# shurizzle/cake

Measured on AMD Instinct MI355X. Metric: decode_tokens_per_sec, higher is better.
Workload: dtype bf16; 1 GPU; model=Llama-3-8B, global_batch=1, seq_len=1097, prompt_len=32, parallelism=single, decode=greedy, repeat_penalty 1.10 last_n 128

## Files before the change

### cake_amd/csrc/engine/llama_engine.cpp

```cpp
#include "llama_engine.h"

#include <dlfcn.h>
#include <hip/hip_runtime.h>
#include <unistd.h>

#include <algorithm>
#include <chrono>
#include <cmath>
#include <cstdio>
#include <cstdlib>
#include <cstring>
#include <fstream>
#include <list>
#include <map>
#include <memory>
#include <sstream>
#include <stdexcept>
#include <string>
#include <tuple>
#include <vector>

#include "../driver/graph_loop.h"
#include "../kernels/cake_kernels.h"
#include "../runtime/json.h"
// ... 81 lines not shown
        const double factor = rs("factor", 8.0), lo = rs("low_freq_factor", 1.0),
                     hi = rs("high_freq_factor", 4.0),
                     old = rs("original_max_position_embeddings", 8192.0);
        const double lo_wl = old / lo, hi_wl = old / hi, wl = 2.0 * M_PI / f;
        const double o = wl > lo_wl ? f / factor : f;
        const double smooth = (old / wl - lo) / (hi - lo);
        const double mid = (1.0 - smooth) * o / factor + smooth * o;
        f = (wl >= hi_wl && wl <= lo_wl) ? mid : o;
      }
      out[i] = (float)f;
    }
    return out;
  }
};


std::vector<std::pair<int, int>> shard_layers(const Cfg& c, int world) {
  std::vector<std::pair<int, int>> out;
  if (world <= 1) {
    out.push_back({0, c.L});
    return out;
  }
  if (world > c.L) {
    for (int r = 0; r < world; ++r) out.push_back(r < c.L ? std::make_pair(r, r + 1)
                                                          : std::make_pair(c.L, c.L));
    return out;
  }
  const double layer_bytes = 2.0 * ((double)c.H * (c.nh + 2 * c.nkv) * c.hd +
                                    (double)c.nh * c.hd * c.H + 3.0 * c.H * c.I + 2.0 * c.H);
  const double head = 2.0 * (double)c.V * c.H / layer_bytes;
  const double total = c.L + head;
  int start = 0;
  for (int r = 0; r < world; ++r) {
    int end = r < world - 1 ? (int)std::nearbyint((r + 1) * total / world - head) : c.L;
    end = std::max(start + (c.L - start >= world - r ? 1 : 0), std::min(end, c.L - (world - 1 - r)));
    out.push_back({start, end});
    start = end;
  }
  return out;
}

std::pair<int, int> split_range(int n, int world, int rank) {
  const int q = n / world, r = n % world;
  const int a = rank * q + std::min(rank, r);
  return {a, a + q + (rank < r ? 1 : 0)};
}

bool trace_on() {
  static const bool on = [] {
    const char* v = std::getenv("CAKE_ENGINE_TRACE");
    return v && *v && std::string(v) != "0";
  }();
  return on;
}
void trace(int rank, const std::string& what) {
  if (!trace_on()) return;
  static const auto t0 = std::chrono::steady_clock::now();
  const double t = std::chrono::duration<double>(std::chrono::steady_clock::now() - t0).count();
  std::fprintf(stderr, "[engine r%d +%.3fs] %s\n", rank, t, what.c_str());
  std::fflush(stderr);
}

const char* const kNoFp8TP =
    "fp8 weights (weight_fmt 1) are not supported with tensor parallelism yet: open the "
    "tensor-parallel engine with weight_fmt 0";

const char* const kNoQHeadTP =
    "a quantised lm_head (head_fmt 1 = fp8, 2 = mxfp4) is not supported with tensor "
    "parallelism: open the tensor-parallel engine with head_fmt 0";

const char* const kNoKvTP =
    "a quantised KV cache (kv_fmt 1 = fp8, 2 = its 16-bit oracle) is not supported with tensor "
    "parallelism: open the tensor-parallel engine with kv_fmt 0";

const char* const kNoPrefillTP =
    "an fp8 MFMA prefill (prefill_fmt 1) is not supported with tensor parallelism: open the "
    "tensor-parallel engine with prefill_fmt 0";

Json msg(const char* cmd) {
  Json j = Json::object();
  j.set("cmd", Json::string(cmd));
  return j;
}

class Llama {
 public:
  Llama(const std::string& dir, const CakeEngineOpts& o, const CakePipeOpts* pp = nullptr,
        const std::vector<int>* layers = nullptr, const CakeTPOpts* tp = nullptr,
        const CakeRemoteOpts* remote = nullptr)
      : dt_(o.dtype), dev_(o.device), init_(o.init), wfmt_(CAKE_WEIGHT_FMT_OF(o.weight_fmt)),
        hfmt_(o.head_fmt), kvfmt_(o.kv_fmt), pfmt_(CAKE_PREFILL_FMT_OF(o.weight_fmt)),
        seed_(o.seed) {
    if (dt_ != 0 && dt_ != 1) throw Error("dtype must be 0 (bf16) or 1 (f16)");
    if (wfmt_ != 0 && wfmt_ != 1 && wfmt_ != 2)
      throw Error("weight_fmt must be 0 (model dtype), 1 (fp8 e4m3 projections) or 2 (mxfp4 "
                  "projections)");
    if (wfmt_ != 0 && tp) throw Error(kNoFp8TP);
    if (hfmt_ != 0 && hfmt_ != 1 && hfmt_ != 2)
      throw Error("head_fmt must be 0 (model dtype), 1 (fp8 e4m3 lm_head) or 2 (mxfp4 lm_head)");
    if (hfmt_ != 0 && tp) throw Error(kNoQHeadTP);
    if (kvfmt_ != kKv16 && kvfmt_ != kKvFp8 && kvfmt_ != kKvFp8Emu)
      throw Error("kv_fmt must be 0 (model dtype), 1 (fp8 e4m3 KV cache) or 2 (fp8 values in a "
                  "16-bit cache: the test oracle)");
    if (kvfmt_ != kKv16 && tp) throw Error(kNoKvTP);
    if (kvfmt_ != kKv16) {
      for (const char* name : {"CAKE_ATTN_OPROJ", "CAKE_ATTN_HEADS", "CAKE_MK", "CAKE_QKV_ATTN"}) {
        const char* e = std::getenv(name);
        if (e && *e && std::string(e) != "0")
          throw Error(std::string("a quantised KV cache (kv_fmt ") + std::to_string(kvfmt_) +
                      ") does not run the experimental decode path " + name + "=" + e +
                      ": unset it or open with kv_fmt 0");
      }
    }
    if (pfmt_ != 0 && pfmt_ != 1)
      throw Error("prefill_fmt must be 0 (the weights' prefill) or 1 (fp8 MFMA prefill with "
                  "per-token e4m3 activations)");
    if (pfmt_ != 0 && tp) throw Error(kNoPrefillTP);
    if (pfmt_ == 1 && wfmt_ != 1)
      throw Error("an fp8 MFMA prefill (prefill_fmt 1) runs on the resident fp8 projection codes: "
                  "open with weight_fmt 1 (fp8), not " + std::to_string(wfmt_));
    if (init_ != 0 && init_ != 1) throw Error("init must be 0 (checkpoint) or 1 (random)");
    if (tp) {
      tp_ = tp->world;
      tp_rank_ = tp->rank;
      hop_timeout_ = tp->timeout_s > 0 ? tp->timeout_s : 30.0;
      if (tp_ < 1 || tp_ > 8 || tp_rank_ < 0 || tp_rank_ >= tp_) throw Error("bad TP rank / world");
      int n = 0;
      hip_check(hipGetDeviceCount(&n), "hipGetDeviceCount");
      if (n > 0) dev_ %= n;
    }
    if (pp) {
      rank_ = pp->rank;
      world_ = pp->world;
      hop_bf16_ = pp->hop_bf16 != 0;
      hop_timeout_ = pp->hop_timeout_s > 0 ? pp->hop_timeout_s : 30.0;
      if (world_ < 1 || rank_ < 0 || rank_ >= world_) throw Error("bad rank / world");
      int n = 0;
      hip_check(hipGetDeviceCount(&n), "hipGetDeviceCount");
      if (n > 0) dev_ %= n;
    }
    hip_check(hipSetDevice(dev_), "hipSetDevice");
    hip_check(hipStreamCreateWithFlags(&st_, hipStreamNonBlocking), "hipStreamCreate");
    cfg_ = Cfg::parse(Json::parse(read_file(dir + "/config.json")));
    S_ = o.max_seq > 0 ? o.max_seq : 4096;
    k_ = std::max(1, o.steps_per_graph);
    if (cfg_.H % 8 || cfg_.hd % 2 || cfg_.nh % cfg_.nkv) throw Error("unsupported model shape");
    if (kvfmt_ != kKv16 && cfg_.hd != 64 && cfg_.hd != 128)
      throw Error("an fp8 KV cache needs a head dimension of 64 or 128");
    lc_ = cfg_;
    if (tp_ > 1) {
      if (cfg_.nh % tp_ || cfg_.nkv % tp_)
        throw Error("tensor-parallel degree must divide the query and KV heads");
      lc_.nh = cfg_.nh / tp_;
      lc_.nkv = cfg_.nkv / tp_;
      const auto ir = split_range(cfg_.I, tp_, tp_rank_);
      const auto vr = split_range(cfg_.V, tp_, tp_rank_);
      i0_ = ir.first;
      lc_.I = ir.second - ir.first;
      voff_ = vr.first;
      lc_.V = vr.second - vr.first;
      if (lc_.I % 8 || (lc_.nh * cfg_.hd) % 8) throw Error("tensor-parallel slice not 8-aligned");
    }
    if (wfmt_ == 1 && (cfg_.H % 16 || (cfg_.nh * cfg_.hd) % 16 || cfg_.I % 16))
      throw Error("fp8 weights need hidden, attention and intermediate widths divisible by 16");
    if (pfmt_ == 1 && (cfg_.H % 128 || (cfg_.nh * cfg_.hd) % 128 || cfg_.I % 128))
      throw Error("an fp8 MFMA prefill needs hidden, attention and intermediate widths divisible "
                  "by 128 (the k of one MFMA step)");
    if (wfmt_ == 2 && (cfg_.H % 32 || (cfg_.nh * cfg_.hd) % 32 || cfg_.I % 32))
      throw Error("mxfp4 weights need hidden, attention and intermediate widths divisible by 32");
    if (layers) {
      hfmt_ = 0;
      owned_ = *layers;
      std::sort(owned_.begin(), owned_.end());
      owned_.erase(std::unique(owned_.begin(), owned_.end()), owned_.end());
      if (owned_.empty() || owned_.front() < 0 || owned_.back() >= cfg_.L)
        throw Error("worker layers outside the model");
      head_ = false;
    } else {
      const bool placed = pp && pp->owners && pp->n_owners > 0;
      owner_.assign(cfg_.L, 0);
      if (placed) {
        if (pp->n_owners != cfg_.L)
          throw Error("owner map has " + std::to_string(pp->n_owners) + " entries for " +
                      std::to_string(cfg_.L) + " layers");
        for (int l = 0; l < cfg_.L; ++l) {
          if (pp->owners[l] < 0 || pp->owners[l] >= world_)
            throw Error("layer " + std::to_string(l) + " placed on rank " +
                        std::to_string(pp->owners[l]) + " outside the world of " +
                        std::to_string(world_));
          owner_[l] = pp->owners[l];
        }
      } else {
        const auto sh = shard_layers(cfg_, world_);
        for (int r = 0; r < world_; ++r)
          for (int l = sh[r].first; l < sh[r].second; ++l) owner_[l] = r;
      }
      if (remote) {
        if (remote->n_layers != cfg_.L || !remote->worker_of)
          throw Error("remote placement must name every layer (-1 = local)");
        remote_of_.assign(remote->worker_of, remote->worker_of + cfg_.L);
        for (int l = 0; l < cfg_.L; ++l)
          if (remote_of_[l] < -1 || remote_of_[l] >= remote->n_workers)
            throw Error("layer " + std::to_string(l) + " placed on an unknown worker");
        for (int w = 0; w < remote->n_workers; ++w)
          remotes_.push_back({remote->workers[w] ? remote->workers[w] : "", -1});
        remote_timeout_ = remote->timeout_s > 0 ? remote->timeout_s : 60.0;
      }
      for (int l = 0; l < cfg_.L; ++l)
        if (owner_[l] == rank_ && (remote_of_.empty() || remote_of_[l] < 0)) owned_.push_back(l);
      head_ = rank_ == 0;
      if (!head_) hfmt_ = 0;
    }
    if (hfmt_ == 1 && cfg_.H % 16) throw Error("an fp8 lm_head needs a hidden width divisible by 16");
    if (hfmt_ == 2 && cfg_.H % 32)
      throw Error("an mxfp4 lm_head needs a hidden width divisible by 32");
    lo_ = owned_.empty() ? 0 : owned_.front();
    hi_ = owned_.empty() ? 0 : owned_.back() + 1;
    local_.assign(cfg_.L, -1);
    for (size_t i = 0; i < owned_.size(); ++i) local_[owned_[i]] = (int)i;
    if (!layers) plan_walk();
    planner_.load(pkg_dir() + "/ops/gemm_tuned.json");
    load_weights(dir);
    std::fprintf(stderr,
                 "cake engine: weights %s, lm_head %s, kv cache %s%s, %lld bytes on device (rank %d, "
                 "%d layers)\n",
                 wfmt_ == 1 ? (dt_ == 0 ? "fp8 e4m3 projections (bf16 rest)"
                                        : "fp8 e4m3 projections (f16 rest)")
                 : wfmt_ == 2 ? (dt_ == 0 ? "mxfp4 projections (bf16 rest)"
                                          : "mxfp4 projections (f16 rest)")
                              : (dt_ == 0 ? "bf16" : "f16"),
                 !head_ ? "none" : hfmt_ == 1 ? "fp8 e4m3" : hfmt_ == 2 ? "mxfp4"
                                                : (dt_ == 0 ? "bf16" : "f16"),
                 kvfmt_ == kKvFp8 ? "fp8 e4m3"
                 : kvfmt_ == kKvFp8Emu ? (dt_ == 0 ? "fp8 e4m3 values in bf16 (test oracle)"
                                                   : "fp8 e4m3 values in f16 (test oracle)")
                                       : (dt_ == 0 ? "bf16" : "f16"),
                 pfmt_ == 1 ? ", prefill fp8 e4m3 activations" : "",
                 (long long)weight_bytes_, rank(), (int)owned_.size());
    alloc_state();
    warm_library();
    {
      size_t fr = 0, tot = 0;
      (void)hipMemGetInfo(&fr, &tot);
      trace(rank(), "weights + state ready (" + std::to_string(owned_.size()) + " layers), " +
                        std::to_string(fr >> 20) + " of " + std::to_string(tot >> 20) +
                        " MiB free");
    }
    if (world_ > 1) {
      connect_pipeline(pp->master_addr ? pp->master_addr : "127.0.0.1:29517",
                       pp->connect_timeout_s > 0 ? pp->connect_timeout_s : 600.0);
      trace(rank_, "pipeline connected: walk " + walk_str() + ", " +
                       std::to_string(edges_.size()) + " edges");
      selftest_pipeline();
      trace(rank_, "pipeline self-test passed");
    }
    if (tp_ > 1) {
      connect_tp(tp->master_addr ? tp->master_addr : "127.0.0.1:29517",
                 tp->connect_timeout_s > 0 ? tp->connect_timeout_s : 600.0);
      trace(rank(), "tensor-parallel channels mapped");
      selftest_tp();
      trace(rank(), "tensor-parallel self-test passed");
    }
    if (!remotes_.empty()) connect_remotes();
  }

  ~Llama() {
    (void)hipSetDevice(dev_);
    (void)hipStreamSynchronize(st_);
    if (rank_ == 0 && tp_rank_ == 0)
      for (int fd : peers_) {
        try {
          send_json(fd, msg("exit"));
        } catch (const std::exception&) {
        }
      }
    for (int fd : peers_) tcp_close(fd);
    if (ctl_fd_ >= 0) tcp_close(ctl_fd_);
    for (auto& r : remotes_)
      if (r.fd >= 0) tcp_close(r.fd);
    drop_graphs();
    for (void* p : tp_mapped_) (void)hipIpcCloseMemHandle(p);
    for (void* p : tp_owned_) (void)cake_hop_free(p);
    for (auto& kv : out_inbox_) (void)hipIpcCloseMemHandle(kv.second);
    for (auto& kv : peer_pbuf_) (void)hipIpcCloseMemHandle(kv.second);
    for (auto& kv : my_inbox_) (void)cake_hop_free(kv.second);
    if (relay_) (void)cake_hop_free(relay_);
    for (void* p : allocs_) (void)hipFree(p);
    (void)hipStreamDestroy(st_);
  }

  int rank() const { return tp_ > 1 ? tp_rank_ : rank_; }
  int world() const { return tp_ > 1 ? tp_ : world_; }
  std::pair<int, int> layer_range() const { return {lo_, hi_}; }

  const Cfg& cfg() const { return cfg_; }
  int max_seq() const { return S_; }
  int64_t weight_bytes() const { return weight_bytes_; }
  int64_t kv_bytes() const { return 2 * (int64_t)kv_elems() * kv_esize(); }

  void prefill_logits(const int32_t* prompt, int T, float* host_logits) {
    hip_check(hipSetDevice(dev_), "hipSetDevice");
    if (!head_) throw Error("prefill_logits() runs on pipeline rank 0");
    prefill(prompt, T);
    hip_check(hipMemcpyAsync(host_logits, logits_, sizeof(float) * cfg_.V, hipMemcpyDeviceToHost,
                             st_), "logits D2H");
    hip_check(hipStreamSynchronize(st_), "sync");
  }

  void forced_logits(const int32_t* prompt, int T, const int32_t* forced, int n, float* out) {
    hip_check(hipSetDevice(dev_), "hipSetDevice");
    if (!head_ || tp_rank_ != 0) throw Error("forced_logits() runs on rank 0");
    if (T <= 0 || n < 0 || T + n + 1 > S_) throw Error("prompt + forced tokens exceed max_seq");
    forced_run(prompt, T, forced, n, out);
  }

  void score(const int32_t* tokens, int n, int vchunk, float* lse, float* tgt, int32_t* top,
             float* topv) {
    hip_check(hipSetDevice(dev_), "hipSetDevice");
    if (tp_ > 1)
      throw Error("score() is not available on a tensor-parallel engine (the vocabulary is "
                  "sharded)");
    if (!head_) throw Error("score() runs on an engine that holds the head (pipeline rank 0)");
    const int V = cfg_.V;
    if (n < 2) throw Error("score() needs at least 2 tokens");
    if (n > S_) throw Error("score(): " + std::to_string(n) + " tokens exceed max_seq " +
                            std::to_string(S_));
    for (int i = 0; i < n; ++i)
      if (tokens[i] < 0 || tokens[i] >= V)
        throw Error("score(): token id " + std::to_string(tokens[i]) + " at " +
                    std::to_string(i) + " is outside [0, " + std::to_string(V) + ")");
    int Vc = vchunk;
    if (vchunk == 0) {
      const long long fit = (64LL << 20) / (4LL * n) / 256 * 256;
      Vc = (int)std::max<long long>(256, fit);
    } else if (vchunk < 0 || vchunk % 256) {
      throw Error("score(): vchunk is 0 or a positive multiple of 256, got " +
                  std::to_string(vchunk));
    }
    Vc = std::min(Vc, V);
    grow_score(n, Vc);
    prefill_body(tokens, n);
    const int H = cfg_.H;
    std::vector<int32_t> target(tokens + 1, tokens + n);
    target.push_back(-1);
    hip_check(hipMemcpyAsync(sc_target_, target.data(), sizeof(int32_t) * n,
                             hipMemcpyHostToDevice, st_), "targets H2D");
    k_check(cake_rmsnorm(dt_, hidden_, norm_, (float)cfg_.eps, n, H, x16_, st_), "rmsnorm");
    for (int v0 = 0; v0 < V; v0 += Vc) {
      const int w = std::min(Vc, V - v0);
      const void* rows;
      if (hfmt_ == 1) {
        k_check(cake_dequant_rows_fp8(dt_, head_q_ + (size_t)v0 * H, head_s_ + v0, w, H, sc_head_,
                                      st_), "dequant_rows_fp8 lm_head");
        rows = sc_head_;
      } else if (hfmt_ == 2) {
        k_check(cake_dequant_rows_mxfp4(dt_, head_q_ + (size_t)v0 * H / 2,
                                        head_e_ + (size_t)v0 * H / 32, w, H, sc_head_, st_),
                "dequant_rows_mxfp4 lm_head");
        rows = sc_head_;
      } else {
        rows = (const uint16_t*)lm_head_ + (size_t)v0 * H;
      }
      gemm(kEpiStore32, x16_, H, rows, H, nullptr, 0, sc_logits_, Vc, n, w, H, "gemm score head");
      k_check(cake_lse_rows(sc_logits_, Vc, n, w, v0, v0 == 0, sc_target_, sc_max_, sc_sum_,
                            sc_tgt_, sc_key_, st_), "lse_rows");
    }
    k_check(cake_lse_finish(sc_max_, sc_sum_, sc_key_, n, sc_lse_, sc_top_, sc_topv_, st_),
            "lse_finish");
    hip_check(hipMemcpyAsync(lse, sc_lse_, sizeof(float) * n, hipMemcpyDeviceToHost, st_), "D2H");
    hip_check(hipMemcpyAsync(tgt, sc_tgt_, sizeof(float) * n, hipMemcpyDeviceToHost, st_), "D2H");
    hip_check(hipMemcpyAsync(top, sc_top_, sizeof(int32_t) * n, hipMemcpyDeviceToHost, st_),
              "D2H");
    hip_check(hipMemcpyAsync(topv, sc_topv_, sizeof(float) * n, hipMemcpyDeviceToHost, st_),
              "D2H");
    hip_check(hipStreamSynchronize(st_), "sync");
    if (world_ > 1) sync_workers();
    check_attn_error("rank " + std::to_string(rank()));
  }

  void set_logprobs(int top_k) {
// ... 202 lines not shown
    };
    stats->p50_ms = pct(50);
    stats->p99_ms = pct(99);
  }

  void run_generation(const int32_t* prompt, int T, int max_new, const CakeEngineSampling& smp,
                      const int32_t* eos, int n_eos, cake_engine_token_cb cb, void* ctx,
                      int32_t* out, int out_cap, CakeEngineStats* stats, bool lead) {
    const auto t0 = std::chrono::steady_clock::now();
    prefill_body(prompt, T);
    std::vector<int32_t> h(prompt, prompt + T);
    hip_check(hipMemcpyAsync(hist_, h.data(), sizeof(int32_t) * T, hipMemcpyHostToDevice, st_),
              "hist H2D");
    set_i32(hist_len_, T);
    set_i32(pos_, T - 1);
    hip_check(hipMemsetAsync(slot_, 0, sizeof(unsigned long long), st_), "slot");
    Mode mode = mode_of(smp);
    if (tp_ > 1) {
      head_tp(hidden_ + (size_t)(T - 1) * cfg_.H, mode);
    } else {
      head_gemv(hidden_ + (size_t)(T - 1) * cfg_.H);
      select_tail(mode);
      logprob_record(mode);
    }
    if (mode.fused) k_check(cake_embed(dt_, embed_, tok_, 1, cfg_.H, resid_, st_), "embed");
    int32_t first = 0;
    hip_check(hipMemcpyAsync(&first, tok_, sizeof(int32_t), hipMemcpyDeviceToHost, st_), "tok");
    lp_begin(mode.logprobs >= 0, max_new);
    if (lp_on_)
      hip_check(hipMemcpyAsync(lp_host_.data(), lp_rec_ + (size_t)T * kLpRecWords,
                               kLpRecWords * 4, hipMemcpyDeviceToHost, st_), "logprob D2H");
    hip_check(hipStreamSynchronize(st_), "sync");
    if (lp_on_ && lead) lp_n_ = 1;
    const auto t1 = std::chrono::steady_clock::now();
    int n_out = 0;
    bool stop = false;
    for (int e = 0; e < n_eos && !stop; ++e)
      if (eos[e] == first) stop = true;
    if (lead) {
      out[n_out++] = first;
      const bool cb_stop = cb && cb(ctx, first) != 0;
      if (tp_ == 1) stop = stop || cb_stop;
    }
    std::vector<float> ms;
    last_mode_ = mode;
    if (remote_mode()) {
      have_graphs_ = true;
      if (!stop && max_new > 1)
        n_out += decode_eager(T, max_new - 1, mode, eos, n_eos, cb, ctx, out + n_out,
                              out_cap - n_out, &ms);
    } else {
      ensure_graphs(mode);
      if (!stop && max_new > 1)
        n_out += decode_tokens(T + 1, max_new - 1, eos, n_eos, cb, ctx,
                               lead ? out + n_out : nullptr, lead ? out_cap - n_out : 0, lead, &ms);
    }
    const auto t2 = std::chrono::steady_clock::now();
    if (stats)
      fill_stats(stats, T, n_out, std::chrono::duration<double>(t1 - t0).count(),
                 std::chrono::duration<double>(t2 - t1).count(), ms);
  }

  int read_i32(const int* p) {
    int v = 0;
    hip_check(hipMemcpyAsync(&v, p, sizeof(int), hipMemcpyDeviceToHost, st_), "i32 D2H");
    hip_check(hipStreamSynchronize(st_), "sync");
    return v;
  }

  void check_attn_error(const std::string& who) {
    unsigned int w = 0;
    hip_check(hipMemcpyAsync(&w, tickets_ + 2 * lc_.nkv, sizeof(w), hipMemcpyDeviceToHost, st_),
              "attn err D2H");
    hip_check(hipStreamSynchronize(st_), "sync");
    if (w) {
      hip_check(hipMemsetAsync(tickets_ + 2 * lc_.nkv, 0, sizeof(unsigned int), st_), "attn err");
      hip_check(hipStreamSynchronize(st_), "sync");
      throw Error(who + ": decode attention split merge timed out waiting for its partials; "
                        "the tokens of that generation are invalid");
    }
  }

 private:
  struct LayerW {
    void *ln1, *wqkv, *wo, *ln2, *wgu, *wd;
    float *sqkv = nullptr, *so = nullptr, *sgu = nullptr, *sd = nullptr;
    uint8_t *eqkv = nullptr, *eo = nullptr, *egu = nullptr, *ed = nullptr;
  };
  struct Mode {
    bool fused = true;
    bool greedy = true;
    float temperature = 0.f, top_p = 0.f, penalty = 1.f;
    int top_k = 0, last_n = 0;
    unsigned long long seed = 0;
    int logprobs = -1;
    bool operator==(const Mode& o) const {
      return std::tie(fused, greedy, temperature, top_p, penalty, top_k, last_n, seed,
                      logprobs) ==
             std::tie(o.fused, o.greedy, o.temperature, o.top_p, o.penalty, o.top_k, o.last_n,
                      o.seed, o.logprobs);
    }
  };

  int dt_, dev_, init_ = 0;
  int wfmt_ = 0;
  int hfmt_ = 0;
  int kvfmt_ = 0;
  int pfmt_ = 0;
  uint16_t *kv16_k_ = nullptr, *kv16_v_ = nullptr;
  int64_t weight_bytes_ = 0;
  uint8_t *head_q_ = nullptr, *head_e_ = nullptr;
  float* head_s_ = nullptr;
  uint16_t* w16_ = nullptr;
  bool forced_ = false;
  AoFns ao_;
  bool ao_ok_ = false, short_step_ = false;
  int heads_max_ = 0;
  float* ao_ws_ = nullptr;
  unsigned int* ao_tickets_ = nullptr;
  uint64_t seed_ = 0;
  int rank_ = 0, world_ = 1, lo_ = 0, hi_ = 0;
  bool head_ = true, hop_bf16_ = false;
  double hop_timeout_ = 30.0;
  enum StopKind { kEmbedStop, kRunStop, kHeadStop, kRemoteStop };
  struct Stop {
    StopKind kind;
    int rank;
    std::vector<int> layers;
    std::vector<int> sel;
    int remote = -1;
  };
  struct RemoteWorker {
    std::string addr;
    int fd;
  };
  std::vector<RemoteWorker> remotes_;
  std::vector<int> remote_of_;
  double remote_timeout_ = 60.0;
  std::vector<float> host_rows_;
  std::vector<Stop> walk_;
  std::vector<int> edge_in_;
  std::vector<std::pair<int, int>> edges_;
  std::vector<int> owner_;
  std::map<int, void*> my_inbox_;
  std::map<int, void*> out_inbox_;
  std::map<int, void*> peer_pbuf_;
  float* relay_ = nullptr;
  unsigned int* seq_ = nullptr;
  int* hop_err_ = nullptr;
  std::vector<int> peers_;
  struct ArChan {
    void* inbox = nullptr;
    std::vector<void*> peers;
  };

  int tp_ = 1, tp_rank_ = 0, i0_ = 0, voff_ = 0, slab_bank_ = 0;
  static constexpr int kSlabRows = 512;
  Cfg lc_;
  ArChan ch_sum_, ch_key_, ch_gat_;
  float *partial_ = nullptr, *ppart_ = nullptr, *full_logits_ = nullptr, *slab_ = nullptr;
  unsigned int* ar_seq_ = nullptr;
  int* ar_err_ = nullptr;
  std::vector<void*> peer_slab_, tp_mapped_, tp_owned_;
  int ctl_fd_ = -1;
  hipStream_t st_ = nullptr;
  Cfg cfg_;
  int S_ = 0, k_ = 1;
  GemmPlanner planner_;
  std::vector<void*> allocs_;
  void *embed_ = nullptr, *norm_ = nullptr, *lm_head_ = nullptr;
  std::vector<LayerW> layers_;
// ... 274 lines not shown
    } catch (...) {
      if (stage) (void)hipFree(stage);
      throw;
    }
    if (stage) (void)hipFree(stage);
  }


  void alloc_state() {
    const Cfg& c = lc_;
    kv_session(0);
    if (kvfmt_ == kKvFp8) {
      const size_t n = (size_t)c.nkv * S_ * c.hd;
      kv16_k_ = dalloc<uint16_t>(n);
      kv16_v_ = dalloc<uint16_t>(n);
      hip_check(hipMemset(kv16_k_, 0, n * 2), "memset");
      hip_check(hipMemset(kv16_v_, 0, n * 2), "memset");
    }
    const std::vector<float> f = c.inv_freq();
    inv_freq_ = dalloc<float>(f.size());
    hip_check(hipMemcpy(inv_freq_, f.data(), f.size() * sizeof(float), hipMemcpyHostToDevice),
              "inv_freq");
    const size_t nq = (size_t)c.nh * c.hd;
    resid_ = dalloc<float>(c.H + 4);
    hidden_ = dalloc<float>((size_t)S_ * c.H);
    q_ = dalloc<float>(nq);
    part_ = dalloc<float>(2 * (size_t)c.nh * kMaxSplit * (c.hd + 2));
    logits_ = dalloc<float>(c.V);
    attn_out_ = dalloc<uint16_t>(nq);
    act_ = dalloc<uint16_t>(c.I);
    tickets_ = dalloc<unsigned int>(2 * c.nkv + 2);
    thr_ = dalloc<unsigned int>(1);
    sel_ticket_ = dalloc<unsigned int>(1);
    pos_ = reinterpret_cast<int*>(resid_ + c.H);
    tok_ = dalloc<int>(1);
    hist_ = dalloc<int>(S_);
    hist_len_ = dalloc<int>(1);
    slot_ = dalloc<unsigned long long>(1);
    scratch_i32_ = dalloc<int>(4);
    scratch_resid_ = dalloc<float>(c.H + 4);
    zeros_ = dalloc<int32_t>(64);
    hip_check(hipMemset(tickets_, 0, sizeof(unsigned int) * (2 * c.nkv + 2)), "memset");
    hip_check(hipMemset(part_, 0, sizeof(float) * 2 * c.nh * kMaxSplit * (c.hd + 2)), "memset");
    hip_check(hipMemset(sel_ticket_, 0, sizeof(unsigned int)), "memset");
    hip_check(hipMemset(slot_, 0, sizeof(unsigned long long)), "memset");
    hip_check(hipMemset(zeros_, 0, sizeof(int32_t) * 64), "memset");
    hip_check(hipMemset(hist_, 0, sizeof(int) * S_), "memset");
    hip_check(hipMemset(resid_, 0, sizeof(float) * (c.H + 4)), "memset");
    {
      const char* e = std::getenv("CAKE_ATTN_OPROJ");
      if (e && std::string(e) == "1" && wfmt_ == 0 && kvfmt_ == kKv16) ao_ = ao_fns();
      ao_ok_ = ao_.run != nullptr && ao_.supported(c.nh, c.nkv, c.hd, c.H) != 0;
    }
    if (!ao_ok_ && kvfmt_ == kKv16) {
      const char* e = std::getenv("CAKE_ATTN_HEADS");
      int mx = 0, nw = 2, pfd = 2;
      if (e && *e) std::sscanf(e, "%d:%d:%d", &mx, &nw, &pfd);
      if (mx > 0 && cake_attn_set_heads(mx, nw) == 0 && cake_attn_set_head_prefetch(pfd) == 0)
        heads_max_ = mx;
    }
    if (ao_ok_) {
      ao_ws_ = dalloc<float>((size_t)ao_.ws_floats(c.nkv, c.H));
      const size_t tw = (size_t)ao_.ticket_words(c.nkv, c.H);
      ao_tickets_ = dalloc<unsigned int>(tw);
      hip_check(hipMemset(ao_tickets_, 0, sizeof(unsigned int) * tw), "memset");
    }
    const size_t nseq = 2 * edges_.size() + 2;
    seq_ = dalloc<unsigned int>(nseq);
    hop_err_ = dalloc<int>(4);
    hip_check(hipMemset(seq_, 0, sizeof(unsigned int) * nseq), "memset");
    hip_check(hipMemset(hop_err_, 0, sizeof(int) * 4), "memset");
    if (tp_ > 1) {
      partial_ = dalloc<float>(c.H);
      ppart_ = dalloc<float>((size_t)S_ * c.H);
      full_logits_ = dalloc<float>(cfg_.V);
      ar_seq_ = dalloc<unsigned int>(8);
      ar_err_ = dalloc<int>(4);
      hip_check(hipMemset(ar_seq_, 0, sizeof(unsigned int) * 8), "memset");
      hip_check(hipMemset(ar_err_, 0, sizeof(int) * 4), "memset");
    }
    hip_check(hipDeviceSynchronize(), "sync");
  }

  size_t kv_esize() const { return kvfmt_ == kKvFp8 ? 1 : 2; }
  size_t kv_elems() const { return owned_.size() * (size_t)lc_.nkv * S_ * lc_.hd; }
  void* kc(int l) const { return cur_.k + (size_t)l * lc_.nkv * S_ * lc_.hd * kv_esize(); }
  void* vc(int l) const { return cur_.v + (size_t)l * lc_.nkv * S_ * lc_.hd * kv_esize(); }

  static constexpr size_t kMaxSessions = 8;
  void kv_session(uint64_t id) {
    auto it = kv_.find(id);
    if (it == kv_.end()) {
      if (kv_.size() >= kMaxSessions) {
        uint64_t victim = lru_.front();
        for (uint64_t x : lru_)
          if (x != 0) { victim = x; break; }
        drop_session(victim);
      }
      const size_t n = kv_elems() * kv_esize();
      KV kv{dalloc<uint8_t>(n), dalloc<uint8_t>(n)};
      it = kv_.emplace(id, kv).first;
    }
    lru_.remove(id);
    lru_.push_back(id);
    cur_ = it->second;
  }

 public:
  void drop_session(uint64_t id) {
    auto it = kv_.find(id);
    if (it == kv_.end() || id == 0) return;
    hip_check(hipStreamSynchronize(st_), "sync");
    dfree(it->second.k);
    dfree(it->second.v);
    kv_.erase(it);
    lru_.remove(id);
    if (kv_.count(0)) cur_ = kv_[0];
  }

  void forward_host(uint64_t session, const std::vector<int>& layers, int pos0, float* h, int T) {
    hip_check(hipSetDevice(dev_), "hipSetDevice");
    const Cfg& c = lc_;
    if (T < 1 || pos0 < 0 || (int64_t)pos0 + T > S_) throw Error("positions exceed the KV cache");
    std::vector<int> sel;
    for (int l : layers) {
      if (l < 0 || l >= c.L || local_[l] < 0)
        throw Error("layer " + std::to_string(l) + " is not served here");
      sel.push_back(local_[l]);
    }
    kv_session(session);
    if (T == 1) {
      hip_check(hipMemcpyAsync(resid_, h, sizeof(float) * c.H, hipMemcpyHostToDevice, st_), "H2D");
      hip_check(hipMemcpyAsync(pos_, &pos0, sizeof(int), hipMemcpyHostToDevice, st_), "H2D");
      short_step_ = short_at(pos0);
      try {
        step_layers(&sel);
      } catch (...) {
        short_step_ = false;
        throw;
      }
      short_step_ = false;
      hip_check(hipMemcpyAsync(h, resid_, sizeof(float) * c.H, hipMemcpyDeviceToHost, st_), "D2H");
    } else {
      const size_t bytes = sizeof(float) * (size_t)T * c.H;
      hip_check(hipMemcpyAsync(hidden_, h, bytes, hipMemcpyHostToDevice, st_), "H2D");
      prefill_layers(T, pos0, &sel);
      hip_check(hipMemcpyAsync(h, hidden_, bytes, hipMemcpyDeviceToHost, st_), "D2H");
    }
    hip_check(hipStreamSynchronize(st_), "sync");
    if (kv_.count(0)) cur_ = kv_[0];
    if (T == 1) check_attn_error("worker");
  }

 private:
  float scale() const { return 1.0f / std::sqrt((float)cfg_.hd); }

  bool short_at(int pos) const { return short_len(pos + 2); }
  bool short_len(int t) const {
    if (ao_ok_) return cake_attn_splits(t) == 1;
    return heads_max_ > 0 && t <= heads_max_;
  }

  void grow_prefill(int T) {
    if (T <= pre_T_) return;
    const Cfg& c = lc_;
    for (void* p : {x16_, qkv_, att_, pact_, (void*)ptok_}) dfree(p);
// ... 322 lines not shown
        continue;
      }
      const int r = owner_.empty() ? 0 : owner_[l];
      if (walk_.back().kind != kRunStop || walk_.back().rank != r) walk_.push_back({kRunStop, r, {}, {}});
      walk_.back().layers.push_back(l);
      if (r == rank_) walk_.back().sel.push_back(local_[l]);
    }
    walk_.push_back({kHeadStop, 0, {}, {}});
    edge_in_.assign(walk_.size(), -1);
    edges_.clear();
    for (size_t i = 1; i < walk_.size(); ++i)
      if (walk_[i].rank != walk_[i - 1].rank) {
        edge_in_[i] = (int)edges_.size();
        edges_.push_back({walk_[i - 1].rank, walk_[i].rank});
      }
  }

 public:
  std::string walk_str() const {
    std::string s;
    for (const Stop& st : walk_)
      if (st.kind == kRunStop || st.kind == kRemoteStop) {
        if (!s.empty()) s += ",";
        s += (st.kind == kRemoteStop ? "w" + std::to_string(st.remote) : std::to_string(st.rank)) +
             ":" + std::to_string(st.layers.front()) + "-" + std::to_string(st.layers.back());
      }
    return s;
  }
  int n_edges() const { return (int)edges_.size(); }

 private:

  void attn(int l) {
    const Cfg& c = lc_;
    if (kvfmt_ == kKvFp8)
      k_check(cake_attn_decode_kv8(dt_, q_, kc(l), vc(l), pos_, S_, c.nh, c.nkv, c.hd, scale(),
                                   part_, tickets_, attn_out_, st_), "attn_decode_kv8");
    else if (short_step_)
      k_check(cake_attn_decode_heads(dt_, q_, kc(l), vc(l), pos_, S_, c.nh, c.nkv, c.hd,
                                     scale(), attn_out_, st_), "attn_heads");
    else
      k_check(cake_attn_decode(dt_, q_, kc(l), vc(l), pos_, S_, c.nh, c.nkv, c.hd, scale(),
                               part_, tickets_, attn_out_, st_), "attn_decode");
  }

  void step_layers(const std::vector<int>* sel = nullptr) {
    const Cfg& c = lc_;
    const int nq = c.nh * c.hd, nk = c.nkv * c.hd;
    const int nl = sel ? (int)sel->size() : (int)layers_.size();
    for (int i = 0; i < nl; ++i) {
      const int l = sel ? (*sel)[i] : i;
      const LayerW& w = layers_[l];
      if (wfmt_ == 2) {
        const uint8_t* q4 = reinterpret_cast<const uint8_t*>(w.wqkv);
        const size_t rb = (size_t)c.H / 2, re = (size_t)c.H / 32;
        k_check(cake_qkv_rope_w4_kvf(dt_, resid_, w.ln1, (float)c.eps, q4, q4 + (size_t)nq * rb,
                                     q4 + (size_t)(nq + nk) * rb, w.eqkv, w.eqkv + (size_t)nq * re,
                                     w.eqkv + (size_t)(nq + nk) * re, c.H, c.nh, c.nkv, c.hd,
                                     inv_freq_, pos_, q_, kc(l), vc(l), S_, st_, kvfmt_),
                "qkv_rope_w4");
        attn(l);
        k_check(cake_gemv_x16_w4(dt_, attn_out_, w.wo, w.eo, nq, c.H, resid_, 1, st_), "o_proj_w4");
        const uint8_t* gu4 = reinterpret_cast<const uint8_t*>(w.wgu);
        k_check(cake_swiglu_w4(dt_, resid_, w.ln2, (float)c.eps, gu4, gu4 + (size_t)c.I * rb,
                               w.egu, w.egu + (size_t)c.I * re, c.H, c.I, act_, st_), "swiglu_w4");
        k_check(cake_gemv_x16_w4(dt_, act_, w.wd, w.ed, c.I, c.H, resid_, 1, st_), "down_proj_w4");
        continue;
      }
      if (wfmt_ == 1) {
        const uint8_t* q8 = reinterpret_cast<const uint8_t*>(w.wqkv);
        k_check(cake_qkv_rope_w8_kvf(dt_, resid_, w.ln1, (float)c.eps, q8, q8 + (size_t)nq * c.H,
                                     q8 + (size_t)(nq + nk) * c.H, w.sqkv, w.sqkv + nq,
                                     w.sqkv + nq + nk, c.H, c.nh, c.nkv, c.hd, inv_freq_, pos_, q_,
                                     kc(l), vc(l), S_, st_, kvfmt_), "qkv_rope_w8");
        attn(l);
        k_check(cake_gemv_x16_w8(dt_, attn_out_, w.wo, w.so, nq, c.H, resid_, 1, st_), "o_proj_w8");
        const uint8_t* gu8 = reinterpret_cast<const uint8_t*>(w.wgu);
        k_check(cake_swiglu_w8(dt_, resid_, w.ln2, (float)c.eps, gu8, gu8 + (size_t)c.I * c.H,
                               w.sgu, w.sgu + c.I, c.H, c.I, act_, st_), "swiglu_w8");
        k_check(cake_gemv_x16_w8(dt_, act_, w.wd, w.sd, c.I, c.H, resid_, 1, st_), "down_proj_w8");
        continue;
      }
      const uint16_t* wqkv = reinterpret_cast<const uint16_t*>(w.wqkv);
      k_check(cake_qkv_rope_kvf(dt_, resid_, w.ln1, (float)c.eps, wqkv, wqkv + (size_t)nq * c.H,
                                wqkv + (size_t)(nq + nk) * c.H, c.H, c.nh, c.nkv, c.hd, inv_freq_,
                                pos_, q_, kc(l), vc(l), S_, st_, kvfmt_), "qkv_rope");
      if (kvfmt_ != kKvFp8 && short_step_ && ao_ok_) {
        k_check(ao_.run(dt_, q_, kc(l), vc(l), pos_, S_, c.nh, c.nkv, c.hd, scale(), w.wo,
                                nq, c.H, tp_ > 1 ? partial_ : resid_, tp_ > 1 ? 0 : 1, ao_ws_,
                                ao_tickets_, tickets_ + 2 * c.nkv, st_), "attn_oproj");
        if (tp_ > 1) ar_sum();
      } else {
        attn(l);
        if (tp_ > 1) {
          k_check(cake_gemv_x16(dt_, attn_out_, w.wo, nq, c.H, partial_, 0, st_), "o_proj");
          ar_sum();
        } else {
          k_check(cake_gemv_x16(dt_, attn_out_, w.wo, nq, c.H, resid_, 1, st_), "o_proj");
        }
      }
      const uint16_t* wgu = reinterpret_cast<const uint16_t*>(w.wgu);
      k_check(cake_swiglu(dt_, resid_, w.ln2, (float)c.eps, wgu, wgu + (size_t)c.I * c.H, c.H,
                          c.I, act_, st_), "swiglu");
      if (tp_ > 1) {
        k_check(cake_gemv_x16(dt_, act_, w.wd, c.I, c.H, partial_, 0, st_), "down_proj");
        ar_sum();
      } else {
        k_check(cake_gemv_x16(dt_, act_, w.wd, c.I, c.H, resid_, 1, st_), "down_proj");
      }
    }
  }

  void step_head(const Mode& m) {
    const Cfg& c = lc_;
    if (forced_) {
      head_logits(resid_);
      return;
    }
    if (tp_ > 1) {
      head_tp(resid_, m);
      return;
    }
    if (m.fused) {
      const int last_n = m.penalty != 1.f ? m.last_n : 0;
      if (hfmt_ == 1)
        k_check(cake_head_select_w8(dt_, resid_, norm_, (float)c.eps, head_q_, head_s_, c.H, c.V,
                                    logits_, hist_, hist_len_, last_n, m.penalty, slot_,
                                    sel_ticket_, tok_, pos_, S_, embed_, resid_, st_),
                "head_select_w8");
      else if (hfmt_ == 2)
        k_check(cake_head_select_w4(dt_, resid_, norm_, (float)c.eps, head_q_, head_e_, c.H, c.V,
                                    logits_, hist_, hist_len_, last_n, m.penalty, slot_,
                                    sel_ticket_, tok_, pos_, S_, embed_, resid_, st_),
                "head_select_w4");
      else
        k_check(cake_head_select(dt_, resid_, norm_, (float)c.eps, lm_head_, c.H, c.V, logits_,
                                 hist_, hist_len_, last_n, m.penalty, slot_, sel_ticket_, tok_,
                                 pos_, S_, embed_, resid_, st_),
                "head_select");
      logprob_record(m);
      return;
    }
    head_gemv(resid_);
    select_tail(m);
    logprob_record(m);
  }

  void head_gemv(const float* row) {
    const Cfg& c = lc_;
    if (hfmt_ == 1)
      k_check(cake_gemv_norm_f32_w8(dt_, row, norm_, (float)c.eps, head_q_, head_s_, c.H, c.V,
                                    logits_, st_), "lm_head_w8");
    else if (hfmt_ == 2)
      k_check(cake_gemv_norm_f32_w4(dt_, row, norm_, (float)c.eps, head_q_, head_e_, c.H, c.V,
                                    logits_, st_), "lm_head_w4");
    else
      k_check(cake_gemv_norm_f32(dt_, row, norm_, (float)c.eps, lm_head_, c.H, c.V, logits_, st_),
              "lm_head");
  }

  float* head_logits(const float* row) {
    const Cfg& c = lc_;
    head_gemv(row);
    if (tp_ == 1) return logits_;
    k_check(cake_ar_gather(logits_, voff_, c.V, full_logits_, cfg_.V, ch_gat_.peers.data(),
                           ch_gat_.inbox, ar_seq_ + 4, ar_err_ + 2, tp_rank_, tp_, hop_timeout_,
                           st_), "ar_gather");
    return full_logits_;
  }

  void forced_run(const int32_t* prompt, int T, const int32_t* forced, int n, float* out) {
    const bool lead = rank_ == 0 && tp_rank_ == 0;
    grow_prefill(T);
    if (tp_ > 1 && lead) {
      Json m = msg("forced");
      Json pr = Json::array(), fr = Json::array();
      for (int i = 0; i < T; ++i) pr.push(Json::integer(prompt[i]));
      for (int i = 0; i < n; ++i) fr.push(Json::integer(forced[i]));
      m.set("prompt", pr);
      m.set("forced", fr);
      for (int fd : peers_) send_json(fd, m);
    }
    prefill_body(prompt, T);
    const size_t V = cfg_.V;
    float* lg = head_logits(hidden_ + (size_t)(T - 1) * cfg_.H);
    if (out) hip_check(hipMemcpyAsync(out, lg, sizeof(float) * V, hipMemcpyDeviceToHost, st_), "D2H");
    hip_check(hipStreamSynchronize(st_), "sync");
    Mode m;
    m.fused = false;
    forced_ = true;
    try {
      for (int i = 0; i < n; ++i) {
        if (world_ > 1)
          for (int fd : peers_) {
            Json st = msg("fstep");
            st.set("pos", Json::integer(T + i));
            send_json(fd, st);
          }
        set_i32(tok_, forced[i]);
        set_i32(pos_, T + i);
        short_step_ = short_at(T + i);
        step_body(m);
        short_step_ = false;
        if (out)
          hip_check(hipMemcpyAsync(out + (size_t)(i + 1) * V, tp_ > 1 ? full_logits_ : logits_,
                                   sizeof(float) * V, hipMemcpyDeviceToHost, st_), "D2H");
        hip_check(hipStreamSynchronize(st_), "sync");
      }
    } catch (...) {
      forced_ = false;
      short_step_ = false;
      throw;
    }
    forced_ = false;
    if (world_ > 1) sync_workers();
    if (tp_ > 1 && lead) sync_tp_workers();
    if (lead) check_attn_error("rank " + std::to_string(rank()));
  }

  void connect_remotes() {
    for (auto& w : remotes_) {
      std::string host;
      int port = 0;
      split_host_port(w.addr, &host, &port);
      w.fd = tcp_connect(host, port, remote_timeout_);
      tcp_set_timeout(w.fd, remote_timeout_);
      Message hello;
      hello.type = MsgType::Hello;
      const std::string body = encode_body(hello);
      send_frame(w.fd, reinterpret_cast<const uint8_t*>(body.data()), (uint32_t)body.size());
      const std::string rep = recv_frame(w.fd);
      const Message info = decode_body(reinterpret_cast<const uint8_t*>(rep.data()), rep.size());
      if (info.type != MsgType::WorkerInfo)
        throw Error("worker " + w.addr + " did not answer Hello with WorkerInfo");
      trace(0, "worker " + w.addr + ": " + info.info.device + " " + info.info.dtype + " (" +
                   info.info.os + "/" + info.info.arch + "), handshake " +
                   std::to_string(info.info.latency_lo) + " ms");
    }
// ... 935 lines not shown
    const std::vector<int> ls(layers, layers + n_layers);
    return new Llama(model_dir, *opts, nullptr, &ls);
  } catch (const std::exception& e) {
    cake::put_err(err, errlen, e.what());
    return nullptr;
  }
}

CAKE_API int32_t cake_engine_forward(void* h, uint64_t session, const int32_t* layers,
                                     int32_t n_layers, int32_t pos0, float* hidden, int32_t T,
                                     char* err, int32_t errlen) {
  try {
    if (!h || !layers || !hidden) throw cake::Error("null argument");
    static_cast<Llama*>(h)->forward_host(session, std::vector<int>(layers, layers + n_layers),
                                         pos0, hidden, T);
    return 0;
  } catch (const std::exception& e) {
    cake::put_err(err, errlen, e.what());
    return 1;
  }
}

CAKE_API void cake_engine_drop_session(void* h, uint64_t session) {
  try {
    if (h) static_cast<Llama*>(h)->drop_session(session);
  } catch (const std::exception&) {
  }
}

CAKE_API void* cake_engine_open_tp(const char* model_dir, const CakeEngineOpts* opts,
                                   const CakeTPOpts* tp, char* err, int32_t errlen) {
  try {
    if (!model_dir || !opts || !tp) throw cake::Error("null argument");
    if (CAKE_WEIGHT_FMT_OF(opts->weight_fmt) != 0) throw cake::Error(cake::kNoFp8TP);
    if (CAKE_PREFILL_FMT_OF(opts->weight_fmt) != 0) throw cake::Error(cake::kNoPrefillTP);
    if (opts->head_fmt != 0) throw cake::Error(cake::kNoQHeadTP);
    if (opts->kv_fmt != 0) throw cake::Error(cake::kNoKvTP);
    return new Llama(model_dir, *opts, nullptr, nullptr, tp);
  } catch (const std::exception& e) {
    cake::put_err(err, errlen, e.what());
    return nullptr;
  }
}

CAKE_API int32_t cake_engine_serve(void* h, char* err, int32_t errlen) {
  try {
    if (!h) throw cake::Error("null engine");
    static_cast<Llama*>(h)->serve();
    return 0;
  } catch (const std::exception& e) {
    cake::put_err(err, errlen, e.what());
    return 1;
  }
}

CAKE_API int32_t cake_engine_rank_info(void* h, int32_t* o) {
  if (!h || !o) return (int32_t)hipErrorInvalidValue;
  const Llama* m = static_cast<Llama*>(h);
  const auto lr = m->layer_range();
  o[0] = m->rank();
  o[1] = m->world();
  o[2] = lr.first;
  o[3] = lr.second;
  return 0;
}

CAKE_API int32_t cake_engine_info(void* h, int32_t* o) {
  if (!h || !o) return (int32_t)hipErrorInvalidValue;
  const Llama* m = static_cast<Llama*>(h);
  const auto& c = m->cfg();
  const int32_t v[8] = {c.V, c.H, c.L, c.nh, c.nkv, c.hd, c.I, m->max_seq()};
  std::memcpy(o, v, sizeof(v));
  return 0;
}

CAKE_API int64_t cake_engine_kv_bytes(void* h) {
  return h ? static_cast<Llama*>(h)->kv_bytes() : 0;
}

CAKE_API int64_t cake_engine_weight_bytes(void* h) {
  return h ? static_cast<Llama*>(h)->weight_bytes() : 0;
}

CAKE_API int32_t cake_engine_eos(void* h, int32_t* out, int32_t cap) {
  if (!h) return 0;
  const auto& e = static_cast<Llama*>(h)->cfg().eos;
  for (int32_t i = 0; i < cap && i < (int32_t)e.size(); ++i) out[i] = e[i];
  return (int32_t)e.size();
}

CAKE_API int32_t cake_engine_generate(void* h, const int32_t* prompt, int32_t n_prompt,
                                      int32_t max_new, const CakeEngineSampling* sampling,
                                      const int32_t* eos, int32_t n_eos,
                                      cake_engine_token_cb cb, void* ctx, int32_t* out,
                                      int32_t out_cap, CakeEngineStats* stats, char* err,
                                      int32_t errlen) {
  try {
    if (!h || !prompt || !sampling || (!out && max_new > 0)) throw cake::Error("null argument");
    static_cast<Llama*>(h)->generate(prompt, n_prompt, max_new, *sampling, eos, n_eos, cb, ctx,
                                     out, out_cap, stats);
    return 0;
  } catch (const std::exception& e) {
    cake::put_err(err, errlen, e.what());
    return 1;
  }
}

CAKE_API int32_t cake_engine_continue(void* h, int32_t max_new, const int32_t* eos, int32_t n_eos,
                                      cake_engine_token_cb cb, void* ctx, int32_t* out,
                                      int32_t out_cap, CakeEngineStats* stats, char* err,
                                      int32_t errlen) {
  try {
    if (!h || (!out && max_new > 0)) throw cake::Error("null argument");
    static_cast<Llama*>(h)->continue_gen(max_new, eos, n_eos, cb, ctx, out, out_cap, stats);
    return 0;
  } catch (const std::exception& e) {
    cake::put_err(err, errlen, e.what());
    return 1;
  }
}

CAKE_API int32_t cake_engine_forced_logits(void* h, const int32_t* prompt, int32_t n_prompt,
                                           const int32_t* forced, int32_t n_forced, float* out,
                                           char* err, int32_t errlen) {
  try {
    if (!h || !prompt || (!forced && n_forced > 0) || !out) throw cake::Error("null argument");
    static_cast<Llama*>(h)->forced_logits(prompt, n_prompt, forced, n_forced, out);
    return 0;
  } catch (const std::exception& e) {
    cake::put_err(err, errlen, e.what());
    return 1;
  }
}

CAKE_API int32_t cake_engine_score(void* h, const int32_t* tokens, int32_t n, int32_t vchunk,
                                   float* lse, float* tgt, int32_t* top, float* topv, char* err,
                                   int32_t errlen) {
  try {
    if (!h || !tokens || !lse || !tgt || !top || !topv) throw cake::Error("null argument");
    static_cast<Llama*>(h)->score(tokens, n, vchunk, lse, tgt, top, topv);
    return 0;
  } catch (const std::exception& e) {
    cake::put_err(err, errlen, e.what());
    return 1;
  }
}

CAKE_API int32_t cake_engine_set_logprobs(void* h, int32_t top_k, char* err, int32_t errlen) {
  try {
    if (!h) throw cake::Error("null engine");
    static_cast<Llama*>(h)->set_logprobs(top_k);
    return 0;
  } catch (const std::exception& e) {
    cake::put_err(err, errlen, e.what());
    return 1;
  }
}

CAKE_API int32_t cake_engine_logprobs(void* h, int32_t first, int32_t count, int32_t* ids,
                                      float* logit, float* lse, int32_t* top_ids,
                                      float* top_logits, char* err, int32_t errlen) {
  try {
    if (!h || ((!ids || !logit || !lse || !top_ids || !top_logits) && count > 0))
      throw cake::Error("null argument");
    static_cast<Llama*>(h)->logprobs(first, count, ids, logit, lse, top_ids, top_logits);
    return 0;
// ... 29 lines not shown
```

### cake_amd/csrc/engine/llama_engine.h

```cpp
#pragma once
#include <stdint.h>

#ifdef __cplusplus
extern "C" {
#endif

typedef int32_t (*cake_engine_token_cb)(void* ctx, int32_t token);

#define CAKE_PREFILL_FMT_SHIFT 8
#define CAKE_PREFILL_FMT(p) ((int32_t)((uint32_t)(p) << CAKE_PREFILL_FMT_SHIFT))
#define CAKE_WEIGHT_FMT_OF(w) ((int32_t)((uint32_t)(w) & 0xffu))
#define CAKE_PREFILL_FMT_OF(w) ((int32_t)((uint32_t)(w) >> CAKE_PREFILL_FMT_SHIFT))

struct CakeEngineOpts {
  int32_t max_seq;
  int32_t dtype;
  int32_t device;
  int32_t steps_per_graph;
  int32_t init;
  int32_t weight_fmt;
  uint64_t seed;
  int32_t head_fmt;
  int32_t kv_fmt;
};

struct CakePipeOpts {
  int32_t rank, world;
  const char* master_addr;
  int32_t hop_bf16;
  double hop_timeout_s;
  double connect_timeout_s;
  const int32_t* owners;
  int32_t n_owners;
};

struct CakeTPOpts {
  int32_t rank, world;
  const char* master_addr;
  double timeout_s;
  double connect_timeout_s;
};

struct CakeRemoteOpts {
  const int32_t* worker_of;
  int32_t n_layers;
  const char* const* workers;
  int32_t n_workers;
  double timeout_s;
};

struct CakeEngineSampling {
  float temperature;
  int32_t top_k;
  float top_p;
  uint64_t seed;
  float repeat_penalty;
  int32_t repeat_last_n;
};

struct CakeEngineStats {
  int32_t n_prompt;
  int32_t n_generated;
  double prefill_s;
  double decode_s;
  double tokens_per_s;
  float p50_ms, p99_ms;
};

void* cake_engine_open(const char* model_dir, const struct CakeEngineOpts* opts, char* err,
                       int32_t errlen);
void* cake_engine_open_pp(const char* model_dir, const struct CakeEngineOpts* opts,
                          const struct CakePipeOpts* pipe, char* err, int32_t errlen);
void* cake_engine_open_tp(const char* model_dir, const struct CakeEngineOpts* opts,
                          const struct CakeTPOpts* tp, char* err, int32_t errlen);
void* cake_engine_open_remote(const char* model_dir, const struct CakeEngineOpts* opts,
                              const struct CakeRemoteOpts* remote, char* err, int32_t errlen);
int32_t cake_engine_serve(void* engine, char* err, int32_t errlen);
void* cake_engine_open_layers(const char* model_dir, const struct CakeEngineOpts* opts,
                              const int32_t* layers, int32_t n_layers, char* err,
                              int32_t errlen);
int32_t cake_engine_forward(void* engine, uint64_t session, const int32_t* layers,
                            int32_t n_layers, int32_t pos0, float* hidden, int32_t T, char* err,
                            int32_t errlen);
void cake_engine_drop_session(void* engine, uint64_t session);
int32_t cake_engine_rank_info(void* engine, int32_t* out4);
int32_t cake_engine_info(void* engine, int32_t* out8);
int32_t cake_engine_eos(void* engine, int32_t* out, int32_t cap);
int64_t cake_engine_weight_bytes(void* engine);
int64_t cake_engine_kv_bytes(void* engine);
int32_t cake_engine_generate(void* engine, const int32_t* prompt, int32_t n_prompt,
                             int32_t max_new, const struct CakeEngineSampling* sampling,
                             const int32_t* eos, int32_t n_eos, cake_engine_token_cb cb,
                             void* ctx, int32_t* out, int32_t out_cap,
                             struct CakeEngineStats* stats, char* err, int32_t errlen);
int32_t cake_engine_continue(void* engine, int32_t max_new, const int32_t* eos, int32_t n_eos,
                             cake_engine_token_cb cb, void* ctx, int32_t* out, int32_t out_cap,
                             struct CakeEngineStats* stats, char* err, int32_t errlen);
int32_t cake_engine_forced_logits(void* engine, const int32_t* prompt, int32_t n_prompt,
                                  const int32_t* forced, int32_t n_forced, float* out, char* err,
                                  int32_t errlen);
int32_t cake_engine_score(void* engine, const int32_t* tokens, int32_t n, int32_t vchunk,
                          float* lse, float* tgt, int32_t* top, float* topv, char* err,
                          int32_t errlen);
int32_t cake_engine_set_logprobs(void* engine, int32_t top_k, char* err, int32_t errlen);
int32_t cake_engine_logprobs(void* engine, int32_t first, int32_t count, int32_t* ids,
                             float* logit, float* lse, int32_t* top_ids, float* top_logits,
                             char* err, int32_t errlen);
int32_t cake_engine_walk(void* engine, char* out, int32_t cap);
int32_t cake_engine_prefill_logits(void* engine, const int32_t* prompt, int32_t n_prompt,
                                   float* out, char* err, int32_t errlen);
void cake_engine_close(void* engine);

#ifdef __cplusplus
}
#endif
```

### cake_amd/csrc/kernels/cake_kernels.h

```cpp
#pragma once

#include <stddef.h>
#include <stdint.h>

#include <hip/hip_runtime_api.h>

#define CAKE_API extern "C" __attribute__((visibility("default")))

namespace cake {

enum DType : int { kBF16 = 0, kF16 = 1, kF32 = 2 };

enum GemmEpi : int {
  kEpiStore = 0,
  kEpiResid32 = 1,
  kEpiAdd16 = 2,
  kEpiSwiglu = 3,
  kEpiGeglu = 4,
  kEpiPartial = 5,
  kEpiStore32 = 6,
  kEpiSilu = 7,
  kEpiQuickGelu = 8,
  kEpiGelu = 9,
};
// ... 48 lines not shown
                 hipStream_t st);

int cake_conv1x1_small(int dt, const void* x, const void* w, const void* bias, void* out, int N,
                       int HW, int IC, int OC, int layout, hipStream_t st);
long long cake_conv2d_workspace(int P, int OC, int splits);
int cake_conv2d_nhwc2(int dt, const void* x, const void* w, const void* bias, const float* bias2,
                      const void* resid, void* out, float* ws, const void* zeros, int N, int H,
                      int W, int IC, int OC, int KH, int KW, int stride, int pad, int up, int cfg,
                      int splits, int th, int tw, int bias2_ld, int layout, hipStream_t st);
int cake_conv2d_nhwc(int dt, const void* x, const void* w, const void* bias, const float* bias2,
                     const void* resid, void* out, float* ws, const void* zeros, int N, int H,
                     int W, int IC, int OC, int KH, int KW, int stride, int pad, int up, int cfg,
                     int splits, int th, int tw, int bias2_ld, hipStream_t st);

int cake_sum_slices(float* out, const float* src, int W, long long stride, long long n,
                    int accumulate, hipStream_t st);
int cake_stream_read(const void* p, size_t bytes, int blocks, unsigned int* sink, hipStream_t st);
int cake_cast16(int src_kind, int dt, const void* src, void* dst, size_t n, hipStream_t st);
int cake_fill_normal(int dt, void* dst, size_t n, float mean, float std, unsigned long long key,
                     hipStream_t st);
int cake_embed(int dt, const void* table, const int* tok, int T, int H, float* out,
               hipStream_t st);
void cake_rmsnorm_set_reg(int on);
int cake_rmsnorm(int dt, const float* x, const void* w, float eps, int T, int H, void* out,
                 hipStream_t st);
int cake_rope_kv(int dt, void* q, const void* k, const void* v, int ldq, int ld, int T, int nh,
                 int nkv, int hd, const float* inv_freq, int pos0, int S, void* kc, void* vc,
                 hipStream_t st);
int cake_rope_kv_kvf(int dt, void* q, const void* k, const void* v, int ldq, int ld, int T, int nh,
                     int nkv, int hd, const float* inv_freq, int pos0, int S, void* kc, void* vc,
                     hipStream_t st, int kv_fmt);
int cake_dequant_kv_fp8(int dt, const void* k8, const void* v8, int nkv, int S, int hd, int Tk,
                        void* k16, void* v16, hipStream_t st);
int cake_silu_mul(int dt, const void* g, const void* u, size_t n, void* out, hipStream_t st);
int cake_silu_mul_rows(int dt, const void* gu, size_t T, int I, void* out, hipStream_t st);
int cake_add_resid(int dt, float* resid, const void* y, size_t n, hipStream_t st);
int cake_wave_reduce_probe(const float* x, float* out, hipStream_t st);

void cake_flash_set_impl(int v);
void cake_flash_set_nw(int nw);
void cake_flash_set_pair_min(long long n);
void cake_flash_set_ksplit(int k);
int cake_flash_attn_ws(int dt, const void* q, const void* k, const void* v, void* o, int B, int H,
                       int Hkv, int N, int M, int D, const long long* strides, float scale,
                       int causal, int pos0, void* ws, long long ws_bytes, hipStream_t st);
int cake_flash_attn(int dt, const void* q, const void* k, const void* v, void* o, int B, int H,
                    int Hkv, int N, int M, int D, const long long* strides, float scale,
                    int causal, int pos0, hipStream_t st);

int cake_gemm_tile(int cfg, int* bm, int* bn);
long long cake_gemm_ws_floats(int cfg, int splits, int M, int N, int K, int gated);
int cake_gemm(int dt, int epi, int cfg, int splits, const void* a, long long lda, const void* b,
              long long ldb, void* c, long long ldc, const void* bias, void* resid, long long ldr,
              float* ws, const void* zeros, int M, int N, int K, hipStream_t st);

int cake_gemm_w8a8_num_cfgs();
int cake_gemm_w8a8_plan(int M, int Nv, int K);
int cake_gemm_w8a8(int dt, int epi, int cfg, const void* a8, long long lda, const float* sa,
                   const void* w8, long long ldb, const float* sw, void* c, long long ldc,
                   float* r32, long long ldr, int M, int N, int K, hipStream_t st);

int cake_gemv_set_tuning(int kind, int U, int prefetch, int max_blocks);
int cake_qkv_rope_kvf(int dt, const float* resid, const void* norm_w, float eps, const void* wq,
                      const void* wk, const void* wv, int K, int nh, int nkv, int hd,
                      const float* inv_freq, const int* pos, float* q_out, void* kcache,
                      void* vcache, int S, hipStream_t st, int kv_fmt);
int cake_qkv_rope(int dt, const float* resid, const void* norm_w, float eps, const void* wq,
                  const void* wk, const void* wv, int K, int nh, int nkv, int hd,
                  const float* inv_freq, const int* pos, float* q_out, void* kcache, void* vcache,
                  int S, hipStream_t st);

int cake_gemv_norm_f32(int dt, const float* resid, const void* norm_w, float eps, const void* w,
                       int K, int N, float* out, hipStream_t st);
int cake_head_select(int dt, const float* resid, const void* norm_w, float eps, const void* w,
                     int K, int N, float* out, int* hist, int* hist_len, int last_n, float penalty,
                     unsigned long long* slot, unsigned int* ticket, int* tok, int* pos,
                     int max_hist, const void* embed, float* emb_out, hipStream_t st);

int cake_swiglu(int dt, const float* resid, const void* norm_w, float eps, const void* wg,
                const void* wu, int K, int I, void* act, hipStream_t st);
int cake_gemv_x16(int dt, const void* x, const void* w, int K, int N, float* out, int accumulate,
                  hipStream_t st);

int cake_gemv_w4_set_tuning(int kind, int U, int prefetch, int max_blocks);
int cake_gemv_w4_get_tuning(int kind, int* out3);
int cake_qkv_rope_w4_kvf(int dt, const float* resid, const void* norm_w, float eps, const void* wq,
                         const void* wk, const void* wv, const void* eq, const void* ek,
                         const void* ev, int K, int nh, int nkv, int hd, const float* inv_freq,
                         const int* pos, float* q_out, void* kcache, void* vcache, int S,
                         hipStream_t st, int kv_fmt);
int cake_qkv_rope_w4(int dt, const float* resid, const void* norm_w, float eps, const void* wq,
                     const void* wk, const void* wv, const void* eq, const void* ek,
                     const void* ev, int K, int nh, int nkv, int hd, const float* inv_freq,
                     const int* pos, float* q_out, void* kcache, void* vcache, int S,
                     hipStream_t st);

int cake_gemv_norm_f32_w4(int dt, const float* resid, const void* norm_w, float eps,
                          const void* w4, const void* e8, int K, int N, float* out,
                          hipStream_t st);
int cake_head_select_w4(int dt, const float* resid, const void* norm_w, float eps, const void* w4,
                        const void* e8, int K, int N, float* out, int* hist, int* hist_len,
                        int last_n, float penalty, unsigned long long* slot, unsigned int* ticket,
                        int* tok, int* pos, int max_hist, const void* embed, float* emb_out,
                        hipStream_t st);

int cake_swiglu_w4(int dt, const float* resid, const void* norm_w, float eps, const void* wg,
                   const void* wu, const void* eg, const void* eu, int K, int I, void* act,
                   hipStream_t st);

int cake_gemv_x16_w4(int dt, const void* x, const void* w, const void* e8, int K, int N,
                     float* out, int accumulate, hipStream_t st);

int cake_gemv_w8_set_tuning(int kind, int U, int prefetch, int max_blocks);
int cake_gemv_w8_get_tuning(int kind, int* out3);
int cake_qkv_rope_w8_kvf(int dt, const float* resid, const void* norm_w, float eps, const void* wq,
                         const void* wk, const void* wv, const float* sq, const float* sk,
                         const float* sv, int K, int nh, int nkv, int hd, const float* inv_freq,
                         const int* pos, float* q_out, void* kcache, void* vcache, int S,
                         hipStream_t st, int kv_fmt);
int cake_qkv_rope_w8(int dt, const float* resid, const void* norm_w, float eps, const void* wq,
                     const void* wk, const void* wv, const float* sq, const float* sk,
                     const float* sv, int K, int nh, int nkv, int hd, const float* inv_freq,
                     const int* pos, float* q_out, void* kcache, void* vcache, int S,
                     hipStream_t st);

int cake_gemv_norm_f32_w8(int dt, const float* resid, const void* norm_w, float eps,
                          const void* w8, const float* scale, int K, int N, float* out,
                          hipStream_t st);
int cake_head_select_w8(int dt, const float* resid, const void* norm_w, float eps, const void* w8,
                        const float* scale, int K, int N, float* out, int* hist, int* hist_len,
                        int last_n, float penalty, unsigned long long* slot, unsigned int* ticket,
                        int* tok, int* pos, int max_hist, const void* embed, float* emb_out,
                        hipStream_t st);

int cake_swiglu_w8(int dt, const float* resid, const void* norm_w, float eps, const void* wg,
                   const void* wu, const float* sg, const float* su, int K, int I, void* act,
                   hipStream_t st);

int cake_gemv_x16_w8(int dt, const void* x, const void* w, const float* scale, int K, int N,
                     float* out, int accumulate, hipStream_t st);

int cake_hop_alloc(size_t bytes, void** ptr);
int cake_hop_free(void* ptr);
int cake_ipc_handle(void* ptr, void* out64);
int cake_ipc_handle_size();
int cake_ipc_open(const void* in64, void** ptr);
int cake_ipc_close(void* ptr);
int cake_hop_words(int H, int nhdr, int bf16);
int cake_hop_send(const float* src, int H, int nhdr, int bf16, void* dst_inbox, unsigned int* seq,
                  hipStream_t st);
int cake_hop_recv(const void* inbox, int H, int nhdr, int bf16, float* dst, unsigned int* seq,
                  int* err, double timeout_s, hipStream_t st);
int cake_bulk_send(const void* const* srcs, const unsigned long long* bytes,
                   const unsigned long long* offs, int nseg, void* dst_rx,
                   unsigned long long rx_bytes, unsigned int* seq, unsigned int* count,
                   hipStream_t st);
int cake_bulk_recv(const void* rx, unsigned long long bytes, void* dst, unsigned int* seq,
                   int* err, double timeout_s, hipStream_t st);

long long cake_logprob_ws_bytes(int V);
int cake_logprob_topk(const float* logits, int V, const int32_t* tok, const int32_t* hist_len,
                      int K, void* rec, int max_rec, void* ws, unsigned int* ticket,
                      int max_blocks, hipStream_t st);

int cake_quant_rows_fp8(int dt, const void* w16, int N, int K, void* w8, float* scale,
                        hipStream_t st);
int cake_dequant_rows_fp8(int dt, const void* w8, const float* scale, int N, int K, void* out16,
                          hipStream_t st);

int cake_quant_rows_mxfp4(int dt, const void* w16, int N, int K, void* w4, void* e8,
                          hipStream_t st);
int cake_dequant_rows_mxfp4(int dt, const void* w4, const void* e8, int N, int K, void* out16,
                            hipStream_t st);

int cake_sample_threshold(const float* logits, int V, float temperature, int top_k, float top_p,
                          unsigned int* thr, hipStream_t st);
int cake_select_dev(const float* logits, int V, const void* params, const int* step,
                    unsigned int* thr, unsigned long long* slot, hipStream_t st);
int cake_gumbel_argmax(const float* logits, int V, float temperature, unsigned long long seed,
                       const int* step, const unsigned int* thr, unsigned long long* slot,
                       hipStream_t st);
int cake_repeat_penalty(float* logits, const int* hist, const int* hist_len, int last_n,
                        float penalty, hipStream_t st);
int cake_argmax(const float* logits, int V, unsigned long long* slot, hipStream_t st);
int cake_select_shard(float* logits, int V, int off, const int* hist, const int* hist_len,
                      int last_n, float penalty, float temperature, unsigned long long seed,
                      unsigned long long* slot, hipStream_t st);
int cake_finalize_token(unsigned long long* slot, int* tok, int* hist, int* hist_len, int* pos,
                        int max_hist, hipStream_t st);
int cake_push_token(const int* src, int* tok, int* hist, int* hist_len, int* pos, int max_hist,
                    hipStream_t st);

int cake_lse_rows(const float* logits, long long ld, int T, int Vc, int v0, int first,
                  const int32_t* target, float* run_max, double* run_sum, float* tgt,
                  unsigned long long* key, hipStream_t st);
int cake_lse_finish(const float* run_max, const double* run_sum, const unsigned long long* key,
                    int T, float* lse, int32_t* top, float* topv, hipStream_t st);

int cake_groupnorm(int dt, const void* x, const void* gamma, const void* beta, int B, int C,
                   long long HW, int G, float eps, int silu_act, float* part, void* y,
                   hipStream_t st);
int cake_layernorm(int dt, const void* x, const void* gamma, const void* beta, long long rows,
                   int C, float eps, void* y, hipStream_t st);
int cake_geglu(int dt, const void* h, long long rows, int F, void* out, hipStream_t st);
int cake_groupnorm_nhwc_splits(int HW);
int cake_groupnorm_nhwc2(int dt, const void* x, const void* x2, int Cx, void* cat,
                         const void* gamma, const void* beta, int N, int HW, int C, int G,
                         float eps, int silu_act, double* part, unsigned int* tickets,
                         float* stats, void* y, hipStream_t st);
int cake_groupnorm_nhwc(int dt, const void* x, const void* gamma, const void* beta, int N, int HW,
                        int C, int G, float eps, int silu_act, double* part, unsigned int* tickets,
                        float* stats, void* y, hipStream_t st);

int cake_timestep_embed(int dt, const float* t_table, const int* step, int B, int dim, int flip,
                        float shift, int out16, void* out, hipStream_t st);
int cake_sched_step(int dt, float* x, const void* pred, long long n, int cfg, float guidance,
                    const void* coef, const int* step, const void* seed, void* next_in,
                    hipStream_t st);
int cake_step_advance(int* step, hipStream_t st);
int cake_scale_copy(int dt, const float* x, long long n, float scale, int dup, void* out,
                    hipStream_t st);
int cake_to_rgb8(int dt, const void* img, int B, int H, int W, int nhwc, void* out,
                 hipStream_t st);
int cake_clip_embed(int dt, const void* tok, const void* pos, const int* ids, int rows, int T,
                    int D, int V, void* out, hipStream_t st);
int cake_widen16(int dt, const void* x, long long n, float* y, hipStream_t st);

int cake_blaslt_gemm(int dt, int out, const void* a, long long lda, const void* w, long long ldw,
                     void* c, long long ldc, int M, int N, int K, void* ws, size_t ws_bytes,
                     hipStream_t st);


int cake_attn_oproj_supported(int nh, int nkv, int hd, int H);
long long cake_attn_oproj_ws_floats(int nkv, int H);
long long cake_attn_oproj_ticket_words(int nkv, int H);
int cake_attn_oproj(int dt, const float* q, const void* kc, const void* vc, const int* pos, int S,
                    int nh, int nkv, int hd, float scale, const void* wo, int ldw, int H,
                    float* out, int accumulate, float* ws, unsigned int* tickets,
                    unsigned int* err, hipStream_t st);

long long cake_mk_gstride(int H, int I, int nh, int nkv, int hd);
int cake_mk_grid();
int cake_mk_set_stamps(void* p);
int cake_mk_set_tuning(int thin, int ring, int fly, int o_all);
int cake_mk_supported(int H, int I, int nh, int nkv, int hd);
int cake_mk_decode(int dt, const void* layers, int L, int H, int I, int nh, int nkv, int hd, int S,
                   float eps, float scale, const float* inv_freq, const int* pos, float* resid,
// ... 4 lines not shown
```

### cake_amd/csrc/kernels/gemv.hip

```cpp
#include "gemv_kernel.h"

namespace cake {
GemvTune g_tune[3][kNumKinds] = {
    {{2, 4, 1024}, {2, 4, 512}, {4, 4, 1024}, {4, 4, 256}, {4, 4, 1024}},
    {{2, 4, 1024}, {2, 4, 1024}, {4, 4, 1024}, {2, 4, 1024}},
    {{2, 4, 1024}, {2, 4, 1024}, {2, 4, 1024}, {2, 4, 1024}}};
}

CAKE_API int cake_gemv_set_tuning(int kind, int U, int prefetch, int max_blocks) {
  return gemv_set_tuning<W16>(kind, U, prefetch, max_blocks);
}

CAKE_API int cake_qkv_rope_kvf(int dt, const float* resid, const void* norm_w, float eps,
                               const void* wq, const void* wk, const void* wv, int K, int nh,
                               int nkv, int hd, const float* inv_freq, const int* pos,
                               float* q_out, void* kcache, void* vcache, int S,
                               hipStream_t st, int kv_fmt) {
  return launch_qkv<W16>(dt, {resid, (const uint16_t*)norm_w, eps, {(const uint16_t*)wq},
                              {(const uint16_t*)wk}, {(const uint16_t*)wv}, K, nh, nkv, hd,
                              inv_freq, pos, q_out, (uint16_t*)kcache, (uint16_t*)vcache, S,
                              kv_fmt}, st);
}

CAKE_API int cake_qkv_rope(int dt, const float* resid, const void* norm_w, float eps,
                           const void* wq, const void* wk, const void* wv, int K, int nh,
                           int nkv, int hd, const float* inv_freq, const int* pos,
                           float* q_out, void* kcache, void* vcache, int S,
                           hipStream_t st) {
  return cake_qkv_rope_kvf(dt, resid, norm_w, eps, wq, wk, wv, K, nh, nkv, hd, inv_freq, pos,
                           q_out, kcache, vcache, S, st, 0);
}
```

### cake_amd/csrc/kernels/gemv_kernel.h

```cpp
#pragma once
#include "common.h"

namespace cake {

constexpr int kGemvThreads = 256;
constexpr int kGemvWaves = kGemvThreads / 64;
constexpr int kGemvMaxBlocks = 1024;

typedef float f32x2_t __attribute__((ext_vector_type(2)));

struct GemvTune { int U, PF, MB; };
enum GemvKind { kQkv = 0, kSwiglu = 1, kX16 = 2, kNormF32 = 3, kX16S = 4, kNumKinds = 5 };
extern GemvTune g_tune[3][kNumKinds];


template <class T>
__device__ __forceinline__ const T* pick3(const T* q, const T* k, const T* v, int kind) {
  const ptrdiff_t dk = k - q, dv = v - q;
  return q + (kind == 0 ? 0 : (kind == 1 ? dk : dv));
}

struct PlainRows {
  struct Rows { const uint4 *a, *b; };
  struct Chunk { uint4 a, b; };
  template <bool NT> static __device__ __forceinline__ Chunk load(const Rows& r, int c) {
    if constexpr (NT) return {ld_nt16(r.a + c), ld_nt16(r.b + c)};
    else return {r.a[c], r.b[c]};
  }
  template <int LOG2> static int prefetch_if_filled(int pf, int K) {
    return (K >> LOG2) >= 64 * pf ? pf : 0;
  }
};

template <int DT, bool XF32>
__device__ __forceinline__ void load_x8(const void* xs, int chunk, float* o) {
  if constexpr (XF32) {
    const float4* p = reinterpret_cast<const float4*>(xs) + chunk * 2;
    const float4 a = p[0], b = p[1];
    o[0] = a.x; o[1] = a.y; o[2] = a.z; o[3] = a.w;
    o[4] = b.x; o[5] = b.y; o[6] = b.z; o[7] = b.w;
  } else {
    unpack8<DT>(reinterpret_cast<const uint4*>(xs)[chunk], o);
  }
}

struct W16 : PlainRows {
  static constexpr int kFmt = 0, kKinds = kNumKinds, kLog2 = 3, kPad32 = 1, kPad16 = 1;
  static constexpr int kU[3] = {2, 4, 8}, kPF[2] = {8, 4};
  static constexpr bool kStrict = false, kRowScale = false;
  static __device__ __forceinline__ int perm32(int i) { return i; }
  static __device__ __forceinline__ int perm16(int i) { return i; }
  static int prefetch(int pf, int K) { return prefetch_if_filled<kLog2>(pf, K); }
  using Acc = float;
  static __device__ __forceinline__ Acc zero() { return 0.f; }
  static __device__ __forceinline__ float total(Acc a) { return a; }
  struct Mat { const uint16_t* w; };
  static __device__ __forceinline__ Mat pick(const Mat& q, const Mat& k, const Mat& v, int kind) {
    return {pick3(q.w, k.w, v.w, kind)};
  }
  static __device__ __forceinline__ Rows rows(const Mat& ma, size_t ra, const Mat& mb, size_t rb,
                                              int K) {
    return {reinterpret_cast<const uint4*>(ma.w + ra * K),
            reinterpret_cast<const uint4*>(mb.w + rb * K)};
  }
  template <int DT, bool XF32>
  static __device__ __forceinline__ void fma(const void* xs, int chunk, const Chunk& v, Acc& acc_a,
                                             Acc& acc_b) {
    float xv[8], fa[8], fb[8];
    load_x8<DT, XF32>(xs, chunk, xv);
    unpack8<DT>(v.a, fa);
    unpack8<DT>(v.b, fb);
#pragma unroll
    for (int e = 0; e < 8; ++e) {
      acc_a = fmaf(fa[e], xv[e], acc_a);
      acc_b = fmaf(fb[e], xv[e], acc_b);
    }
  }
};

template <class F>
__device__ __forceinline__ float row_scale(const typename F::Mat& m, size_t row) {
  if constexpr (F::kRowScale) return m.scale[row];
  else return 1.f;
}
template <class F>
__device__ __forceinline__ float descale(float d, bool first, float s0, const typename F::Mat& m,
                                         size_t row) {
  if constexpr (F::kRowScale) return d * (first ? s0 : m.scale[row]);
  else return d;
}


template <class F, int DT>
__device__ __forceinline__ void stage_rmsnorm(const float* __restrict__ x,
                                              const uint16_t* __restrict__ w,
                                              float eps, int K, float* xs) {
  __shared__ float red[16];
  float ss = 0.f;
  for (int i = threadIdx.x * 4; i < K; i += kGemvThreads * 4) {
    const float4 v = *reinterpret_cast<const float4*>(x + i);
    *reinterpret_cast<float4*>(xs + F::perm32(i)) = v;
    ss += v.x * v.x + v.y * v.y + v.z * v.z + v.w * v.w;
  }
  ss = block_sum(ss, red);
  const float r = rsqrtf(ss / (float)K + eps);
  for (int i = threadIdx.x * 4; i < K; i += kGemvThreads * 4) {
    float4 v = *reinterpret_cast<float4*>(xs + F::perm32(i));
    const uint2 wv = *reinterpret_cast<const uint2*>(w + i);
    v.x *= r * to_f32<DT>((uint16_t)(wv.x & 0xffff));
    v.y *= r * to_f32<DT>((uint16_t)(wv.x >> 16));
    v.z *= r * to_f32<DT>((uint16_t)(wv.y & 0xffff));
    v.w *= r * to_f32<DT>((uint16_t)(wv.y >> 16));
    *reinterpret_cast<float4*>(xs + F::perm32(i)) = v;
  }
  __syncthreads();
}

template <class F>
__device__ __forceinline__ void stage_plain16(const uint16_t* __restrict__ x, int K,
                                              uint16_t* xs) {
  for (int i = threadIdx.x * 8; i < K; i += kGemvThreads * 8)
    *reinterpret_cast<uint4*>(xs + F::perm16(i)) = *reinterpret_cast<const uint4*>(x + i);
  __syncthreads();
}

template <class F, int DT, int NX> struct NormPre {
  float4 x[NX];
  uint2 w[NX];
  __device__ __forceinline__ void load(const float* __restrict__ xg, const uint16_t* __restrict__ wg,
                                       int K) {
#pragma unroll
    for (int j = 0; j < NX; ++j) {
      const int i = (j * kGemvThreads + threadIdx.x) * 4;
      x[j] = i < K ? *reinterpret_cast<const float4*>(xg + i) : make_float4(0.f, 0.f, 0.f, 0.f);
      w[j] = i < K ? *reinterpret_cast<const uint2*>(wg + i) : make_uint2(0u, 0u);
    }
  }
  __device__ __forceinline__ void finish(float eps, int K, float* xs) {
    __shared__ float red[16];
    float ss = 0.f;
#pragma unroll
    for (int j = 0; j < NX; ++j) ss += x[j].x * x[j].x + x[j].y * x[j].y + x[j].z * x[j].z + x[j].w * x[j].w;
    ss = block_sum(ss, red);
    const float r = rsqrtf(ss / (float)K + eps);
#pragma unroll
    for (int j = 0; j < NX; ++j) {
      const int i = (j * kGemvThreads + threadIdx.x) * 4;
      float4 v = x[j];
      v.x *= r * to_f32<DT>((uint16_t)(w[j].x & 0xffff));
      v.y *= r * to_f32<DT>((uint16_t)(w[j].x >> 16));
      v.z *= r * to_f32<DT>((uint16_t)(w[j].y & 0xffff));
      v.w *= r * to_f32<DT>((uint16_t)(w[j].y >> 16));
      if (i < K) *reinterpret_cast<float4*>(xs + F::perm32(i)) = v;
    }
    __syncthreads();
  }
};

template <class F, int NX> struct Plain16Pre {
  uint4 v[NX];
  __device__ __forceinline__ void load(const uint16_t* __restrict__ xg, int K) {
#pragma unroll
    for (int j = 0; j < NX; ++j) {
      const int i = (j * kGemvThreads + threadIdx.x) * 8;
      v[j] = i < K ? *reinterpret_cast<const uint4*>(xg + i) : make_uint4(0u, 0u, 0u, 0u);
    }
  }
  __device__ __forceinline__ void finish(int K, uint16_t* xs) {
#pragma unroll
    for (int j = 0; j < NX; ++j) {
      const int i = (j * kGemvThreads + threadIdx.x) * 8;
      if (i < K) *reinterpret_cast<uint4*>(xs + F::perm16(i)) = v[j];
    }
    __syncthreads();
  }
};


template <class F, int DT, bool XF32, int U>
__device__ __forceinline__ void dot_range(const typename F::Rows& r, const void* xs, int nch,
                                          int c_start, typename F::Acc& acc_a,
                                          typename F::Acc& acc_b) {
  const int lane = threadIdx.x & 63;
  const int full = c_start + ((nch - c_start) / (64 * U)) * (64 * U);
  for (int c0 = c_start; c0 < full; c0 += 64 * U) {
    typename F::Chunk v[U];
#pragma unroll
    for (int u = 0; u < U; ++u) v[u] = F::template load<true>(r, c0 + u * 64 + lane);
#pragma unroll
    for (int u = 0; u < U; ++u) F::template fma<DT, XF32>(xs, c0 + u * 64 + lane, v[u], acc_a, acc_b);
  }
  for (int c = full + lane; c < nch; c += 64)
    F::template fma<DT, XF32>(xs, c, F::template load<false>(r, c), acc_a, acc_b);
}

template <class F, int PFC> struct Regs { typename F::Chunk c[PFC > 0 ? PFC : 1]; };

template <class F, int PFC>
__device__ __forceinline__ void prefetch_rows(const typename F::Rows& r, Regs<F, PFC>& g) {
  if constexpr (PFC > 0) {
    const int lane = threadIdx.x & 63;
#pragma unroll
    for (int c = 0; c < PFC; ++c) g.c[c] = F::template load<true>(r, c * 64 + lane);
  }
}

template <class F, int DT, bool XF32, int U, int PFC, class Map, class Epi>
__device__ __forceinline__ void run_pairs(const Map& map, const Epi& epi, const void* xs, int K,
                                          int npairs, int p0, int stride,
                                          const Regs<F, PFC>& pre) {
  const int nch = K >> F::kLog2;
  int p = p0;
  if constexpr (PFC > 0) {
    const typename F::Rows r = map(p < npairs ? p : npairs - 1);
    const int lane = threadIdx.x & 63;
    typename F::Acc aa = F::zero(), ab = F::zero();
#pragma unroll
    for (int c = 0; c < PFC; ++c) F::template fma<DT, XF32>(xs, c * 64 + lane, pre.c[c], aa, ab);
    dot_range<F, DT, XF32, U>(r, xs, nch, PFC * 64, aa, ab);
    const float sa = wave_sum(F::total(aa)), sb = wave_sum(F::total(ab));
    if (p < npairs) epi(p, sa, sb);
    p += stride;
  }
  for (; p < npairs; p += stride) {
    const typename F::Rows r = map(p);
    typename F::Acc aa = F::zero(), ab = F::zero();
    dot_range<F, DT, XF32, U>(r, xs, nch, 0, aa, ab);
    epi(p, wave_sum(F::total(aa)), wave_sum(F::total(ab)));
  }
}

template <class F> struct QkvArgs {
  const float* resid;
  const uint16_t* norm_w;
  float eps;
  typename F::Mat q, k, v;
  int K, nh, nkv, hd;
  const float* inv_freq;
  const int* pos;
  float* q_out;
  uint16_t* kcache;
  uint16_t* vcache;
  int S;
  int kv_fmt;
};

struct QkvPair {
  int kind, head, i;
  size_t ra;
};

__device__ __forceinline__ QkvPair qkv_pair(int p, int half, int nh, int nqk, int hd) {
  const int slot = p / half;
  const bool isq = slot < nh, isk = !isq && slot < nqk;
  QkvPair r;
  r.kind = isq ? 0 : (isk ? 1 : 2);
  r.head = slot - (isq ? 0 : (isk ? nh : nqk));
  r.i = p - slot * half;
  r.ra = (size_t)r.head * hd + r.i;
  return r;
}

template <class F, int DT, int U, int PFC, int NX>
__global__ __launch_bounds__(kGemvThreads) void qkv_rope_kernel(QkvArgs<F> a) {
  extern __shared__ float xs[];
  const int half = a.hd >> 1;
  const int npairs = (a.nh + 2 * a.nkv) * half;
  const int wave = threadIdx.x >> 6, lane = threadIdx.x & 63;
  const int p0 = blockIdx.x * kGemvWaves + wave;
  const int nh = a.nh, nqk = a.nh + a.nkv, hd = a.hd, K = a.K;
  auto map = [&](int p) {
    const QkvPair r = qkv_pair(p, half, nh, nqk, hd);
    const typename F::Mat m = F::pick(a.q, a.k, a.v, r.kind);
    return F::rows(m, r.ra, m, r.ra + half, K);
  };
  Regs<F, PFC> pre;
  NormPre<F, DT, NX> xp;
  const int pc = p0 < npairs ? p0 : npairs - 1;
  const typename F::Rows r0 = map(pc);
  if constexpr (NX > 0) xp.load(a.resid, a.norm_w, a.K);
  __builtin_amdgcn_sched_barrier(0);
  if (NX > 0 || (PFC > 0 && p0 < npairs)) prefetch_rows<F, PFC>(r0, pre);
  const QkvPair rc = qkv_pair(pc, half, nh, nqk, hd);
  const float f0 = a.inv_freq[rc.i];
  const typename F::Mat mc = F::pick(a.q, a.k, a.v, rc.kind);
  const float s0a = row_scale<F>(mc, rc.ra), s0b = row_scale<F>(mc, rc.ra + half);
  __builtin_amdgcn_sched_barrier(0);
  if constexpr (NX > 0) xp.finish(a.eps, a.K, xs);
  else stage_rmsnorm<F, DT>(a.resid, a.norm_w, a.eps, a.K, xs);
  const int pos = *a.pos;
  auto epi = [&](int p, float da, float db) {
    if (lane != 0) return;
    const QkvPair r = qkv_pair(p, half, nh, nqk, hd);
    const typename F::Mat m = F::pick(a.q, a.k, a.v, r.kind);
    if constexpr (F::kRowScale) {
      float sa = s0a, sb = s0b;
      if (p != p0) { sa = m.scale[r.ra]; sb = m.scale[r.ra + half]; }
      da *= sa;
      db *= sb;
    }
    float oa = da, ob = db;
    if (r.kind < 2) {
      float s, c;
      sincosf((float)pos * (p == p0 ? f0 : a.inv_freq[r.i]), &s, &c);
      oa = da * c - db * s;
      ob = da * s + db * c;
    }
    if (r.kind == 0) {
      a.q_out[r.ra] = oa;
      a.q_out[r.ra + half] = ob;
    } else {
      uint16_t* cache = r.kind == 1 ? a.kcache : a.vcache;
      const size_t off = ((size_t)r.head * a.S + pos) * a.hd + r.i;
      kv_store_pair<DT>(cache, off, half, oa, ob, a.kv_fmt);
    }
  };
  run_pairs<F, DT, true, U, PFC>(map, epi, xs, a.K, npairs, p0, gridDim.x * kGemvWaves, pre);
}

template <class F, int DT, int U, int PFC, int NX>
__global__ __launch_bounds__(kGemvThreads) void swiglu_kernel(
    const float* __restrict__ resid, const uint16_t* __restrict__ norm_w, float eps,
    const typename F::Mat wg, const typename F::Mat wu, int K, int I,
    uint16_t* __restrict__ act) {
  extern __shared__ float xs[];
  const int wave = threadIdx.x >> 6, lane = threadIdx.x & 63;
  const int j0 = blockIdx.x * kGemvWaves + wave;
  auto map = [&](int j) { return F::rows(wg, (size_t)j, wu, (size_t)j, K); };
  Regs<F, PFC> pre;
  NormPre<F, DT, NX> xp;
  const int jp = j0 < I ? j0 : I - 1;
  const typename F::Rows r0 = map(jp);
  if constexpr (NX > 0) xp.load(resid, norm_w, K);
  __builtin_amdgcn_sched_barrier(0);
  if (NX > 0 || (PFC > 0 && j0 < I)) prefetch_rows<F, PFC>(r0, pre);
  const float s0g = row_scale<F>(wg, jp), s0u = row_scale<F>(wu, jp);
  __builtin_amdgcn_sched_barrier(0);
  if constexpr (NX > 0) xp.finish(eps, K, xs);
  else stage_rmsnorm<F, DT>(resid, norm_w, eps, K, xs);
  auto epi = [&](int j, float g, float u) {
    if (lane != 0) return;
    g = descale<F>(g, j == j0, s0g, wg, j);
    u = descale<F>(u, j == j0, s0u, wu, j);
    act[j] = from_f32<DT>(silu(g) * u);
  };
  run_pairs<F, DT, true, U, PFC>(map, epi, xs, K, I, j0, gridDim.x * kGemvWaves, pre);
}

template <class F, int DT, int U, int PFC, int NX, bool ACCUM>
__global__ __launch_bounds__(kGemvThreads) void gemv_x16_kernel(
    const uint16_t* __restrict__ x, const typename F::Mat w, int K, int N,
    float* __restrict__ out) {
  extern __shared__ float smem[];
  uint16_t* xs = reinterpret_cast<uint16_t*>(smem);
  const int wave = threadIdx.x >> 6, lane = threadIdx.x & 63;
  const int npairs = (N + 1) >> 1;
  const int p0 = blockIdx.x * kGemvWaves + wave;
  auto map = [&](int p) { return F::rows(w, (size_t)(2 * p), w, (size_t)min(2 * p + 1, N - 1), K); };
  Regs<F, PFC> pre;
  Plain16Pre<F, NX> xp;
  const int pc = p0 < npairs ? p0 : npairs - 1;
  const typename F::Rows r0 = map(pc);
  if constexpr (NX > 0) xp.load(x, K);
  __builtin_amdgcn_sched_barrier(0);
  if (NX > 0 || (PFC > 0 && p0 < npairs)) prefetch_rows<F, PFC>(r0, pre);
  const float s0a = row_scale<F>(w, 2 * pc), s0b = row_scale<F>(w, min(2 * pc + 1, N - 1));
  float r0a = 0.f, r0b = 0.f;
  if constexpr (ACCUM) {
    r0a = out[2 * pc];
    r0b = out[min(2 * pc + 1, N - 1)];
  }
  __builtin_amdgcn_sched_barrier(0);
  if constexpr (NX > 0) xp.finish(K, xs);
  else stage_plain16<F>(x, K, xs);
  auto epi = [&](int p, float da, float db) {
    if (lane != 0) return;
    const int ra = 2 * p, rb = 2 * p + 1;
    da = descale<F>(da, p == p0, s0a, w, ra);
    if (ACCUM) out[ra] = da + (p == p0 ? r0a : out[ra]); else out[ra] = da;
    if (rb < N) {
      db = descale<F>(db, p == p0, s0b, w, rb);
      if (ACCUM) out[rb] = db + (p == p0 ? r0b : out[rb]); else out[rb] = db;
    }
  };
  run_pairs<F, DT, false, U, PFC>(map, epi, xs, K, npairs, p0, gridDim.x * kGemvWaves, pre);
}

struct HeadSel {
  const int* hist;
  const int* hist_len;
  int last_n;
  float penalty;
  unsigned long long* slot;
  unsigned int* ticket;
  int* tok;
  int* hist_w;
  int* hist_len_w;
  int* pos;
  int max_hist;
  const uint16_t* embed;
  float* emb_out;
  int H;
};

__device__ __forceinline__ unsigned int ordered_key(float f) {
  const unsigned int u = __float_as_uint(f);
  return (u & 0x80000000u) ? ~u : (u | 0x80000000u);
}

__device__ __forceinline__ void head_sel_window(const HeadSel& hs, int hlen, int lane, int* win) {
  const int n = min(hs.last_n, hlen), start = hlen - n;
#pragma unroll
  for (int j = 0; j < 4; ++j) win[j] = j * 64 + lane < n ? hs.hist[start + j * 64 + lane] : -1;
}

__device__ __forceinline__ void head_sel_pair(const HeadSel& hs, const int* win, int ra, int rb,
                                              int N, float& da, float& db,
                                              unsigned long long& best) {
  if (hs.penalty != 1.f) {
    const bool ia = win[0] == ra || win[1] == ra || win[2] == ra || win[3] == ra;
    const bool ib = win[0] == rb || win[1] == rb || win[2] == rb || win[3] == rb;
    if (__builtin_amdgcn_ballot_w64(ia) != 0ull) da = da >= 0.f ? da / hs.penalty : da * hs.penalty;
    if (__builtin_amdgcn_ballot_w64(ib) != 0ull) db = db >= 0.f ? db / hs.penalty : db * hs.penalty;
  }
  const unsigned long long ka =
      ((unsigned long long)ordered_key(da) << 32) | (0xffffffffu - (unsigned int)ra);
  best = ka > best ? ka : best;
  if (rb < N) {
    const unsigned long long kb =
        ((unsigned long long)ordered_key(db) << 32) | (0xffffffffu - (unsigned int)rb);
    best = kb > best ? kb : best;
  }
}

template <int DT>
__device__ __forceinline__ void head_sel_tail(const HeadSel& hs, unsigned long long best,
                                              void* lds) {
  const int wave = threadIdx.x >> 6, lane = threadIdx.x & 63;
  unsigned long long* red = reinterpret_cast<unsigned long long*>(lds);
  int& is_last = reinterpret_cast<int*>(lds)[2 * kGemvWaves];
  int& sel_tok = reinterpret_cast<int*>(lds)[2 * kGemvWaves + 1];
  __syncthreads();
  if (lane == 0) red[wave] = best;
  __syncthreads();
  if (threadIdx.x == 0) {
    unsigned long long b = red[0];
#pragma unroll
    for (int i = 1; i < kGemvWaves; ++i) b = red[i] > b ? red[i] : b;
    const unsigned long long old =
        __hip_atomic_fetch_max(hs.slot, b, __ATOMIC_RELAXED, __HIP_MEMORY_SCOPE_AGENT);
    asm volatile("s_waitcnt vmcnt(0)" ::"v"((unsigned int)old) : "memory");
    const unsigned int t =
        __hip_atomic_fetch_add(hs.ticket, 1u, __ATOMIC_RELAXED, __HIP_MEMORY_SCOPE_AGENT);
    is_last = t == gridDim.x - 1;
  }
  __syncthreads();
  if (is_last) {
    if (threadIdx.x == 0) {
      const unsigned long long key =
          __hip_atomic_fetch_max(hs.slot, 0ull, __ATOMIC_RELAXED, __HIP_MEMORY_SCOPE_AGENT);
      const int t = (int)(0xffffffffu - (unsigned int)(key & 0xffffffffull));
      *hs.tok = t;
      const int len = *hs.hist_len_w;
      if (len < hs.max_hist) { hs.hist_w[len] = t; *hs.hist_len_w = len + 1; }
      *hs.pos += 1;
      __hip_atomic_store(hs.slot, 0ull, __ATOMIC_RELAXED, __HIP_MEMORY_SCOPE_AGENT);
      __hip_atomic_store(hs.ticket, 0u, __ATOMIC_RELAXED, __HIP_MEMORY_SCOPE_AGENT);
      sel_tok = t;
    }
    if (hs.embed != nullptr) {
      __syncthreads();
      const uint16_t* row = hs.embed + (size_t)sel_tok * hs.H;
      for (int i = threadIdx.x * 8; i < hs.H; i += kGemvThreads * 8) {
        float f[8];
        unpack8<DT>(*reinterpret_cast<const uint4*>(row + i), f);
        *reinterpret_cast<float4*>(hs.emb_out + i) = make_float4(f[0], f[1], f[2], f[3]);
        *reinterpret_cast<float4*>(hs.emb_out + i + 4) = make_float4(f[4], f[5], f[6], f[7]);
      }
    }
  }
}

template <class F, int DT, int U, int PFC, int NX, bool SEL>
__global__ __launch_bounds__(kGemvThreads) void gemv_norm_f32_kernel(
    const float* __restrict__ resid, const uint16_t* __restrict__ norm_w, float eps,
    const typename F::Mat w, int K, int N, float* __restrict__ out, HeadSel hs) {
  extern __shared__ float xs[];
  const int wave = threadIdx.x >> 6, lane = threadIdx.x & 63;
  const int npairs = (N + 1) >> 1;
  const int p0 = blockIdx.x * kGemvWaves + wave;
  auto map = [&](int p) { return F::rows(w, (size_t)(2 * p), w, (size_t)min(2 * p + 1, N - 1), K); };
  int hlen = 0;
  if constexpr (SEL) hlen = hs.penalty != 1.f ? *hs.hist_len : 0;
  Regs<F, PFC> pre;
  NormPre<F, DT, NX> xp;
  const int pc = p0 < npairs ? p0 : npairs - 1;
  const typename F::Rows r0 = map(pc);
  if constexpr (NX > 0) xp.load(resid, norm_w, K);
  __builtin_amdgcn_sched_barrier(0);
  if (NX > 0 || (PFC > 0 && p0 < npairs)) prefetch_rows<F, PFC>(r0, pre);
  const float s0a = row_scale<F>(w, 2 * pc), s0b = row_scale<F>(w, min(2 * pc + 1, N - 1));
  __builtin_amdgcn_sched_barrier(0);
  if constexpr (NX > 0) xp.finish(eps, K, xs);
  else stage_rmsnorm<F, DT>(resid, norm_w, eps, K, xs);
  int win[4] = {-1, -1, -1, -1};
  if constexpr (SEL) head_sel_window(hs, hlen, lane, win);
  unsigned long long best = 0ull;
  auto epi = [&](int p, float da, float db) {
    const int ra = 2 * p, rb = 2 * p + 1;
    da = descale<F>(da, p == p0, s0a, w, ra);
    db = descale<F>(db, p == p0, s0b, w, min(rb, N - 1));
    if constexpr (SEL) head_sel_pair(hs, win, ra, rb, N, da, db, best);
    if (lane != 0) return;
    out[ra] = da;
    if (rb < N) out[rb] = db;
  };
  run_pairs<F, DT, true, U, PFC>(map, epi, xs, K, npairs, p0, gridDim.x * kGemvWaves, pre);
  if constexpr (SEL) head_sel_tail<DT>(hs, best, xs);
}

static inline int grid_for(int npairs, int max_blocks) {
  int g = (npairs + kGemvWaves - 1) / kGemvWaves;
  return g < max_blocks ? g : max_blocks;
}

}

using namespace cake;


#define DISPATCH_DT(dt, ...)                       \
  do {                                             \
    if ((dt) == kBF16) { constexpr int DT = kBF16; __VA_ARGS__; } \
    else if ((dt) == kF16) { constexpr int DT = kF16; __VA_ARGS__; } \
    else return (int)hipErrorInvalidValue;         \
  } while (0)

#define CAKE_TUNE_U(F, PFCV, ...)                                                              \
  if (t.U == F::kU[0]) { constexpr int U = F::kU[0]; constexpr int PF = PFCV; __VA_ARGS__; }      \
  else if (t.U == F::kU[1]) { constexpr int U = F::kU[1]; constexpr int PF = PFCV; __VA_ARGS__; } \
  else { constexpr int U = F::kU[2]; constexpr int PF = PFCV; __VA_ARGS__; }
#define DISPATCH_TUNE(F, t, K, ...)                                                  \
  do {                                                                               \
    const int pfc_ = F::prefetch((t).PF, K);                                         \
    if (pfc_ == F::kPF[0]) { CAKE_TUNE_U(F, F::kPF[0], __VA_ARGS__) }                \
    else if (pfc_ == F::kPF[1]) { CAKE_TUNE_U(F, F::kPF[1], __VA_ARGS__) }           \
    else { CAKE_TUNE_U(F, 0, __VA_ARGS__) }                                          \
  } while (0)
#define CAKE_NX_NORM(K, ...)                                                         \
  if constexpr (PF > 0) {                                                            \
    if ((K) <= 4096) { constexpr int NX = 4; __VA_ARGS__; }                          \
    else if ((K) <= 8192) { constexpr int NX = 8; __VA_ARGS__; }                     \
    else { constexpr int NX = 0; __VA_ARGS__; }                                      \
  } else { constexpr int NX = 0; __VA_ARGS__; }
#define CAKE_NX_X16(K, ...)                                                          \
  if constexpr (PF > 0) {                                                            \
    if ((K) <= 2048) { constexpr int NX = 1; __VA_ARGS__; }                          \
    else if ((K) <= 4096) { constexpr int NX = 2; __VA_ARGS__; }                     \
    else if ((K) <= 8192) { constexpr int NX = 4; __VA_ARGS__; }                     \
    else if ((K) <= 14336) { constexpr int NX = 7; __VA_ARGS__; }                    \
    else if ((K) <= 28672) { constexpr int NX = 14; __VA_ARGS__; }                   \
    else { constexpr int NX = 0; __VA_ARGS__; }                                      \
  } else { constexpr int NX = 0; __VA_ARGS__; }

template <class F> static inline bool bad_shape(int K, int n) {
  return K % (1 << F::kLog2) != 0 || (F::kStrict && (K < (1 << F::kLog2) || n < 1));
}
template <class F> static inline size_t x32_lds_bytes(int K) {
  return (size_t)((K + F::kPad32 - 1) / F::kPad32 * F::kPad32) * sizeof(float);
}
template <class F> static inline size_t x16_lds_bytes(int K) {
  return (size_t)((K + F::kPad16 - 1) / F::kPad16 * F::kPad16) * sizeof(uint16_t);
}

template <class F> static int gemv_set_tuning(int kind, int U, int prefetch, int max_blocks) {
  if (kind < 0 || kind >= F::kKinds || (U != F::kU[0] && U != F::kU[1] && U != F::kU[2]) ||
      max_blocks < 1 || (prefetch != 0 && prefetch != F::kPF[0] && prefetch != F::kPF[1]))
    return (int)hipErrorInvalidValue;
  g_tune[F::kFmt][kind] = GemvTune{U, prefetch, max_blocks};
  return 0;
}

template <class F> static int gemv_get_tuning(int kind, int* out3) {
  if (kind < 0 || kind >= F::kKinds || !out3) return (int)hipErrorInvalidValue;
  const GemvTune t = g_tune[F::kFmt][kind];
  out3[0] = t.U;
  out3[1] = t.PF;
  out3[2] = t.MB;
  return 0;
}

template <class F> static int launch_qkv(int dt, const QkvArgs<F>& a, hipStream_t st) {
  if (bad_shape<F>(a.K, a.nh < a.nkv ? a.nh : a.nkv) || a.hd % 2 || a.kv_fmt < 0 || a.kv_fmt > 2)
    return (int)hipErrorInvalidValue;
  const int K = a.K, npairs = (a.nh + 2 * a.nkv) * (a.hd / 2);
  const size_t lds = x32_lds_bytes<F>(K);
  const GemvTune t = g_tune[F::kFmt][kQkv];
  DISPATCH_DT(dt, DISPATCH_TUNE(F, t, K, CAKE_NX_NORM(K, hipLaunchKernelGGL((qkv_rope_kernel<F, DT, U, PF, NX>),
                                                         dim3(grid_for(npairs, t.MB)),
                                                         dim3(kGemvThreads), lds, st, a))));
  return (int)hipGetLastError();
}

template <class F>
static int launch_swiglu(int dt, const float* resid, const void* norm_w, float eps,
                         typename F::Mat wg, typename F::Mat wu, int K, int I, void* act,
                         hipStream_t st) {
  if (bad_shape<F>(K, I)) return (int)hipErrorInvalidValue;
  const size_t lds = x32_lds_bytes<F>(K);
  const GemvTune t = g_tune[F::kFmt][kSwiglu];
  const int mb = t.MB > (I + 27) / 28 ? t.MB : (I + 27) / 28;
  DISPATCH_DT(dt, DISPATCH_TUNE(F, t, K, CAKE_NX_NORM(K, hipLaunchKernelGGL((swiglu_kernel<F, DT, U, PF, NX>),
                                                         dim3(grid_for(I, mb)), dim3(kGemvThreads),
                                                         lds, st, resid, (const uint16_t*)norm_w, eps,
                                                         wg, wu, K, I, (uint16_t*)act))));
  return (int)hipGetLastError();
}

template <class F>
static int launch_x16(int dt, const void* x, typename F::Mat w, int K, int N, float* out,
                      int accumulate, hipStream_t st) {
  if (bad_shape<F>(K, N)) return (int)hipErrorInvalidValue;
  const size_t lds = x16_lds_bytes<F>(K);
  const GemvTune t = g_tune[F::kFmt][F::kKinds > kX16S && K <= 8192 ? kX16S : kX16];
  const int g = grid_for((N + 1) / 2, t.MB);
  if (accumulate) {
    DISPATCH_DT(dt, DISPATCH_TUNE(F, t, K, CAKE_NX_X16(K, hipLaunchKernelGGL((gemv_x16_kernel<F, DT, U, PF, NX, true>),
                                                          dim3(g), dim3(kGemvThreads), lds, st,
                                                          (const uint16_t*)x, w, K, N, out))));
  } else {
    DISPATCH_DT(dt, DISPATCH_TUNE(F, t, K, CAKE_NX_X16(K, hipLaunchKernelGGL((gemv_x16_kernel<F, DT, U, PF, NX, false>),
                                                          dim3(g), dim3(kGemvThreads), lds, st,
                                                          (const uint16_t*)x, w, K, N, out))));
  }
  return (int)hipGetLastError();
}

template <class F, bool SEL>
static int launch_norm_f32(int dt, const float* resid, const void* norm_w, float eps,
                           typename F::Mat w, int K, int N, float* out, const HeadSel& hs,
                           hipStream_t st) {
  if (bad_shape<F>(K, N)) return (int)hipErrorInvalidValue;
  const size_t lds = SEL && x32_lds_bytes<F>(K) < 64 ? 64 : x32_lds_bytes<F>(K);
  const GemvTune t = g_tune[F::kFmt][kNormF32];
  DISPATCH_DT(dt, DISPATCH_TUNE(F, t, K, CAKE_NX_NORM(K, hipLaunchKernelGGL((gemv_norm_f32_kernel<F, DT, U, PF, NX, SEL>),
                                                         dim3(grid_for((N + 1) / 2, t.MB)),
                                                         dim3(kGemvThreads), lds, st, resid,
                                                         (const uint16_t*)norm_w, eps, w, K, N,
                                                         out, hs))));
  return (int)hipGetLastError();
}

template <class F>
static int launch_head_select(int dt, const float* resid, const void* norm_w, float eps,
                              typename F::Mat w, int K, int N, float* out, int* hist,
                              int* hist_len, int last_n, float penalty, unsigned long long* slot,
                              unsigned int* ticket, int* tok, int* pos, int max_hist,
                              const void* embed, float* emb_out, hipStream_t st) {
  if (last_n < 0 || last_n > kHeadSelectMaxLastN || !(penalty > 0.f) || slot == nullptr ||
      ticket == nullptr || (embed != nullptr && emb_out == nullptr))
    return (int)hipErrorInvalidValue;
  const HeadSel hs{hist, hist_len, last_n, penalty, slot, ticket, tok, hist, hist_len, pos,
                   max_hist, (const uint16_t*)embed, emb_out, K};
  return launch_norm_f32<F, true>(dt, resid, norm_w, eps, w, K, N, out, hs, st);
}
```

### cake_amd/engine.py

```python
from __future__ import annotations

import ctypes as C
from dataclasses import dataclass, field
from pathlib import Path
from typing import Callable

LIB_PATH = Path(__file__).resolve().parent / "lib" / "libcake_engine.so"

TOKEN_CB = C.CFUNCTYPE(C.c_int32, C.c_void_p, C.c_int32)


class EngineOpts(C.Structure):
    _fields_ = [("max_seq", C.c_int32), ("dtype", C.c_int32), ("device", C.c_int32),
                ("steps_per_graph", C.c_int32), ("init", C.c_int32), ("weight_fmt", C.c_int32),
                ("seed", C.c_uint64), ("head_fmt", C.c_int32), ("kv_fmt", C.c_int32)]


class PipeOpts(C.Structure):
    _fields_ = [("rank", C.c_int32), ("world", C.c_int32), ("master_addr", C.c_char_p),
                ("hop_bf16", C.c_int32), ("hop_timeout_s", C.c_double),
                ("connect_timeout_s", C.c_double), ("owners", C.POINTER(C.c_int32)),
                ("n_owners", C.c_int32)]


class TPOpts(C.Structure):
    _fields_ = [("rank", C.c_int32), ("world", C.c_int32), ("master_addr", C.c_char_p),
                ("timeout_s", C.c_double), ("connect_timeout_s", C.c_double)]


class RemoteOpts(C.Structure):
    _fields_ = [("worker_of", C.POINTER(C.c_int32)), ("n_layers", C.c_int32),
                ("workers", C.POINTER(C.c_char_p)), ("n_workers", C.c_int32),
                ("timeout_s", C.c_double)]


class EngineSampling(C.Structure):
    _fields_ = [("temperature", C.c_float), ("top_k", C.c_int32), ("top_p", C.c_float),
                ("seed", C.c_uint64), ("repeat_penalty", C.c_float),
                ("repeat_last_n", C.c_int32)]


class EngineStats(C.Structure):
    _fields_ = [("n_prompt", C.c_int32), ("n_generated", C.c_int32), ("prefill_s", C.c_double),
                ("decode_s", C.c_double), ("tokens_per_s", C.c_double), ("p50_ms", C.c_float),
                ("p99_ms", C.c_float)]


WEIGHT_FORMATS = {"model": 0, "fp8": 1, "mxfp4": 2}
KV_FORMATS = {"model": 0, "fp8": 1, "fp8-emulated": 2}

PREFILL_FORMATS = {"model": 0, "fp8": 1}
PREFILL_FMT_SHIFT = 8

_lib = None


def _bind(L) -> None:
    P, I = C.c_void_p, C.c_int32
    L.cake_engine_open.argtypes = [C.c_char_p, C.POINTER(EngineOpts), C.c_char_p, I]
    L.cake_engine_open.restype = P
    L.cake_engine_open_pp.argtypes = [C.c_char_p, C.POINTER(EngineOpts), C.POINTER(PipeOpts),
                                      C.c_char_p, I]
    L.cake_engine_open_pp.restype = P
    L.cake_engine_open_tp.argtypes = [C.c_char_p, C.POINTER(EngineOpts), C.POINTER(TPOpts),
                                      C.c_char_p, I]
    L.cake_engine_open_tp.restype = P
    L.cake_engine_open_remote.argtypes = [C.c_char_p, C.POINTER(EngineOpts),
                                          C.POINTER(RemoteOpts), C.c_char_p, I]
    L.cake_engine_open_remote.restype = P
    L.cake_engine_serve.argtypes = [P, C.c_char_p, I]
    L.cake_engine_serve.restype = I
    L.cake_engine_rank_info.argtypes = [P, C.POINTER(C.c_int32)]
    L.cake_engine_rank_info.restype = I
    L.cake_engine_info.argtypes = [P, C.POINTER(C.c_int32)]
    L.cake_engine_info.restype = I
    L.cake_engine_eos.argtypes = [P, C.POINTER(C.c_int32), I]
    L.cake_engine_eos.restype = I
    L.cake_engine_weight_bytes.argtypes = [P]
    L.cake_engine_weight_bytes.restype = C.c_int64
    L.cake_engine_kv_bytes.argtypes = [P]
    L.cake_engine_kv_bytes.restype = C.c_int64
    L.cake_engine_open_layers.argtypes = [C.c_char_p, C.POINTER(EngineOpts),
                                          C.POINTER(C.c_int32), I, C.c_char_p, I]
    L.cake_engine_open_layers.restype = P
    L.cake_engine_forward.argtypes = [P, C.c_uint64, C.POINTER(C.c_int32), I, I,
                                      C.POINTER(C.c_float), I, C.c_char_p, I]
    L.cake_engine_forward.restype = I
    L.cake_engine_drop_session.argtypes = [P, C.c_uint64]
    L.cake_engine_drop_session.restype = None
    L.cake_engine_generate.argtypes = [P, C.POINTER(C.c_int32), I, I, C.POINTER(EngineSampling),
                                       C.POINTER(C.c_int32), I, TOKEN_CB, P,
                                       C.POINTER(C.c_int32), I, C.POINTER(EngineStats),
                                       C.c_char_p, I]
    L.cake_engine_generate.restype = I
    L.cake_engine_continue.argtypes = [P, I, C.POINTER(C.c_int32), I, TOKEN_CB, P,
                                       C.POINTER(C.c_int32), I, C.POINTER(EngineStats),
                                       C.c_char_p, I]
    L.cake_engine_continue.restype = I
    L.cake_engine_forced_logits.argtypes = [P, C.POINTER(C.c_int32), I, C.POINTER(C.c_int32),
                                            I, C.POINTER(C.c_float), C.c_char_p, I]
    L.cake_engine_forced_logits.restype = I
    L.cake_engine_walk.argtypes = [P, C.c_char_p, I]
    L.cake_engine_walk.restype = I
    L.cake_engine_prefill_logits.argtypes = [P, C.POINTER(C.c_int32), I,
                                             C.POINTER(C.c_float), C.c_char_p, I]
    L.cake_engine_prefill_logits.restype = I
    FP = C.POINTER(C.c_float)
    L.cake_engine_score.argtypes = [P, C.POINTER(C.c_int32), I, I, FP, FP,
                                    C.POINTER(C.c_int32), FP, C.c_char_p, I]
    L.cake_engine_score.restype = I
    IP = C.POINTER(C.c_int32)
    L.cake_engine_set_logprobs.argtypes = [P, I, C.c_char_p, I]
    L.cake_engine_set_logprobs.restype = I
    L.cake_engine_logprobs.argtypes = [P, I, I, IP, FP, FP, IP, FP, C.c_char_p, I]
    L.cake_engine_logprobs.restype = I
    L.cake_engine_close.argtypes = [P]
    L.cake_engine_close.restype = None


def lib() -> C.CDLL:
    global _lib
    if _lib is None:
        if not LIB_PATH.exists():
            raise RuntimeError(f"{LIB_PATH} missing: run `python -m cake_amd.build`")
        L = C.CDLL(str(LIB_PATH))
        _bind(L)
        _lib = L
    return _lib


@dataclass
class GenResult:
    tokens: list[int] = field(default_factory=list)
    n_prompt: int = 0
    prefill_s: float = 0.0
    decode_s: float = 0.0
    tokens_per_s: float = 0.0
    p50_ms: float = 0.0
    p99_ms: float = 0.0
    logprobs: "TokenLogprobs | None" = None


LOGPROBS_MAX_TOP = 20


@dataclass
class TokenLogprobs:
    ids: "np.ndarray"
    logit: "np.ndarray"
    lse: "np.ndarray"
    logprob: "np.ndarray"
    top_ids: "np.ndarray"
    top_logits: "np.ndarray"
    top_logprobs: "np.ndarray"


def logprob_json_lines(lp: "TokenLogprobs") -> list[str]:
    import json
    return [json.dumps({"index": i, "id": int(lp.ids[i]), "logprob": float(lp.logprob[i]),
                        "top_ids": [int(t) for t in lp.top_ids[i]],
                        "top_logprobs": [float(v) for v in lp.top_logprobs[i]]}) + "\n"
            for i in range(len(lp.ids))]
# ... 31 lines not shown

class NativeLlama:

    def __init__(self, model_dir: str | Path, *, max_seq: int = 4096, dtype: str = "bf16",
                 device: int = 0, steps_per_graph: int = 1, rank: int = 0, world: int = 1,
                 master_addr: str = "127.0.0.1:29517", hop_bf16: bool = False,
                 hop_timeout_s: float = 30.0, connect_timeout_s: float = 600.0,
                 tp: bool = False, owners: list[int] | None = None, random_init: bool = False,
                 seed: int = 0, worker_of: list[int] | None = None,
                 workers: list[str] | None = None, remote_timeout_s: float = 120.0,
                 weights: str = "model", head: str = "model", kv: str = "model",
                 layers: list[int] | None = None, prefill: str = "model"):
        if dtype not in ("bf16", "f16"):
            raise ValueError("native engine dtype: bf16 or f16")
        if weights not in WEIGHT_FORMATS:
            raise ValueError(f"native engine weights: one of {sorted(WEIGHT_FORMATS)}, "
                             f"got {weights!r}")
        if head not in WEIGHT_FORMATS:
            raise ValueError(f"native engine head: one of {sorted(WEIGHT_FORMATS)}, got {head!r}")
        if kv not in KV_FORMATS:
            raise ValueError(f"native engine kv: one of {sorted(KV_FORMATS)}, got {kv!r}")
        if prefill not in PREFILL_FORMATS:
            raise ValueError(f"native engine prefill: one of {sorted(PREFILL_FORMATS)}, "
                             f"got {prefill!r}")
        self.prefill = prefill
        self.weights = weights
        self.head = head
        self.kv = kv
        opts = EngineOpts(int(max_seq), 0 if dtype == "bf16" else 1, int(device),
                          max(1, int(steps_per_graph)), 1 if random_init else 0,
                          WEIGHT_FORMATS[weights] | PREFILL_FORMATS[prefill] << PREFILL_FMT_SHIFT,
                          int(seed) & 0xFFFFFFFFFFFFFFFF, WEIGHT_FORMATS[head], KV_FORMATS[kv])
        err = C.create_string_buffer(1024)
        self._h = None
        if world > 1 and tp:
            self._addr = master_addr.encode()
            o = TPOpts(int(rank), int(world), self._addr, float(hop_timeout_s),
                       float(connect_timeout_s))
            self._h = lib().cake_engine_open_tp(str(model_dir).encode(), C.byref(opts),
                                                C.byref(o), err, len(err))
        elif world > 1:
            self._addr = master_addr.encode()
            own = None
            if owners is not None:
                own = (C.c_int32 * len(owners))(*[int(x) for x in owners])
            self._owners = own
            pipe = PipeOpts(int(rank), int(world), self._addr, int(bool(hop_bf16)),
                            float(hop_timeout_s), float(connect_timeout_s),
                            C.cast(own, C.POINTER(C.c_int32)) if own is not None else None,
                            len(owners) if owners is not None else 0)
            self._h = lib().cake_engine_open_pp(str(model_dir).encode(), C.byref(opts),
                                                C.byref(pipe), err, len(err))
        elif layers is not None:
            ls = (C.c_int32 * len(layers))(*[int(x) for x in layers])
            self._h = lib().cake_engine_open_layers(str(model_dir).encode(), C.byref(opts), ls,
                                                    len(layers), err, len(err))
        elif workers:
            wo = (C.c_int32 * len(worker_of))(*[int(x) for x in worker_of])
            hs = (C.c_char_p * len(workers))(*[w.encode() for w in workers])
            self._remote = (wo, hs)
            ro = RemoteOpts(C.cast(wo, C.POINTER(C.c_int32)), len(worker_of),
                            C.cast(hs, C.POINTER(C.c_char_p)), len(workers),
                            float(remote_timeout_s))
            self._h = lib().cake_engine_open_remote(str(model_dir).encode(), C.byref(opts),
                                                    C.byref(ro), err, len(err))
        else:
            self._h = lib().cake_engine_open(str(model_dir).encode(), C.byref(opts), err, len(err))
        if not self._h:
            raise RuntimeError(f"native engine: {err.value.decode(errors='replace')}")
        ri = (C.c_int32 * 4)()
        lib().cake_engine_rank_info(self._h, ri)
        self.rank, self.world, self.first_layer, self.end_layer = list(ri)
        info = (C.c_int32 * 8)()
        lib().cake_engine_info(self._h, info)
        (self.vocab_size, self.hidden_size, self.num_layers, self.num_heads, self.num_kv_heads,
         self.head_dim, self.intermediate_size, self.max_seq) = list(info)
        eos = (C.c_int32 * 16)()
        n = lib().cake_engine_eos(self._h, eos, 16)
        self.eos_ids = [int(eos[i]) for i in range(min(n, 16))]

    def weight_bytes(self) -> int:
        return int(lib().cake_engine_weight_bytes(self._h))

    def kv_bytes(self) -> int:
        return int(lib().cake_engine_kv_bytes(self._h))

    def forward(self, layers: list[int], pos0: int, hidden, session: int = 1):
        import numpy as np
        if hidden.dtype != np.float32 or hidden.ndim != 2 or not hidden.flags.c_contiguous:
            raise ValueError("forward: hidden must be a C-contiguous float32 [T, H] array")
        ls = (C.c_int32 * len(layers))(*[int(x) for x in layers])
        err = C.create_string_buffer(1024)
        rc = lib().cake_engine_forward(self._h, int(session), ls, len(layers), int(pos0),
                                       hidden.ctypes.data_as(C.POINTER(C.c_float)),
                                       hidden.shape[0], err, len(err))
        if rc:
            raise RuntimeError(f"native engine: {err.value.decode(errors='replace')}")
        return hidden

    def walk(self) -> str:
        buf = C.create_string_buffer(4096)
        lib().cake_engine_walk(self._h, buf, len(buf))
        return buf.value.decode()

    def serve(self) -> None:
        err = C.create_string_buffer(1024)
        if lib().cake_engine_serve(self._h, err, len(err)):
            raise RuntimeError(f"native engine: {err.value.decode(errors='replace')}")

    def close(self) -> None:
        if getattr(self, "_h", None):
            lib().cake_engine_close(self._h)
            self._h = None

    def __del__(self):
        self.close()

    def prefill_logits(self, prompt: list[int]):
        import numpy as np
        arr = (C.c_int32 * len(prompt))(*prompt)
        out = np.empty(self.vocab_size, dtype=np.float32)
        err = C.create_string_buffer(1024)
        rc = lib().cake_engine_prefill_logits(self._h, arr, len(prompt),
                                              out.ctypes.data_as(C.POINTER(C.c_float)), err,
                                              len(err))
        if rc:
            raise RuntimeError(f"native engine: {err.value.decode(errors='replace')}")
        return out

    def score(self, tokens: list[int], *, vchunk: int = 0) -> ScoreResult:
        import numpy as np
        n = len(tokens)
        if n < 2:
            raise ValueError("score: at least 2 tokens (the first token is never scored)")
        arr = (C.c_int32 * n)(*[int(t) for t in tokens])
        lse, tgt, topv = (np.empty(n, dtype=np.float32) for _ in range(3))
        top = np.empty(n, dtype=np.int32)
        err = C.create_string_buffer(1024)
        fp = C.POINTER(C.c_float)
        rc = lib().cake_engine_score(self._h, arr, n, int(vchunk), lse.ctypes.data_as(fp),
                                     tgt.ctypes.data_as(fp),
                                     top.ctypes.data_as(C.POINTER(C.c_int32)),
                                     topv.ctypes.data_as(fp), err, len(err))
        if rc:
            raise RuntimeError(f"native engine: {err.value.decode(errors='replace')}")
        return score_result(tokens, lse, tgt, top, topv)

    def forced_logits(self, prompt: list[int], forced: list[int]):
        import numpy as np
        arr = (C.c_int32 * len(prompt))(*prompt)
        fa = (C.c_int32 * max(1, len(forced)))(*forced)
        out = np.empty((len(forced) + 1, self.vocab_size), dtype=np.float32)
        err = C.create_string_buffer(1024)
        rc = lib().cake_engine_forced_logits(self._h, arr, len(prompt), fa, len(forced),
                                             out.ctypes.data_as(C.POINTER(C.c_float)), err,
                                             len(err))
        if rc:
            raise RuntimeError(f"native engine: {err.value.decode(errors='replace')}")
        return out

    def generate(self, prompt: list[int], max_new: int, *, temperature: float = 0.0,
                 top_k: int | None = None, top_p: float | None = None, seed: int = 299792458,
                 repeat_penalty: float = 1.1, repeat_last_n: int = 128,
                 eos_ids: list[int] | None = None,
                 on_token: Callable[[int], bool | None] | None = None,
                 logprobs: int | None = None) -> GenResult:
# ... 104 lines not shown
```

### cake_amd/ops/_lib.py

```python
from __future__ import annotations

import ctypes as C
import os
import threading
from pathlib import Path

_LIB_PATH = Path(__file__).resolve().parent.parent / "lib" / "libcake_kernels.so"
_lock = threading.Lock()
_lib = None

P = C.c_void_p
I = C.c_int
F = C.c_float
D = C.c_double
Z = C.c_size_t
L = C.c_longlong
U = C.c_ulonglong

_SIGS = {
    "cake_ar_inbox_words": (L, [I, I]),
    "cake_ar_sum": (I, [P, P, I, I, P, P, P, P, I, I, D, P]),
    "cake_ar_max_key": (I, [P, P, P, P, P, I, I, D, P]),
    "cake_ar_gather": (I, [P, I, I, P, I, P, P, P, P, I, I, D, P]),
    "cake_attn_set_impl": (I, [I]),
    "cake_attn_set_stamps": (I, [P]),
    "cake_attn_set_split_cap": (I, [I]),
    "cake_attn_set_target_splits": (I, [I]),
    "cake_attn_set_prefetch": (I, [I]),
    "cake_attn_set_single_max": (I, [I]),
    "cake_attn_debug_drop_partials": (I, [I]),
    "cake_attn_splits": (I, [I]),
    "cake_attn_max_split": (I, [I]),
    "cake_attn_set_min_keys": (I, [I]),
    "cake_attn_decode": (I, [I, P, P, P, P, I, I, I, I, F, P, P, P, P]),
    "cake_attn_decode_kv8": (I, [I, P, P, P, P, I, I, I, I, F, P, P, P, P]),
    "cake_attn_set_head_prefetch": (I, [I]),
    "cake_attn_set_heads": (I, [I, I]),
    "cake_attn_heads_max": (I, []),
    "cake_attn_decode_heads": (I, [I, P, P, P, P, I, I, I, I, F, P, P]),
    "cake_attn512": (I, [I, P, P, P, P, I, I, I, L, L, L, L, L, L, L, L, F, P, P]),
    "cake_conv1x1_small": (I, [I, P, P, P, P, I, I, I, I, I, P]),
    "cake_conv2d_workspace": (L, [I, I, I]),
    "cake_conv2d_nhwc2": (I, [I, P, P, P, P, P, P, P, P, I, I, I, I, I, I, I, I, I, I, I, I, I, I,
                              I, I, P]),
    "cake_conv2d_nhwc": (I, [I, P, P, P, P, P, P, P, P, I, I, I, I, I, I, I, I, I, I, I, I, I, I,
                             I, P]),
    "cake_sum_slices": (I, [P, P, I, L, L, I, P]),
    "cake_stream_read": (I, [P, Z, I, P, P]),
    "cake_cast16": (I, [I, I, P, P, Z, P]),
    "cake_fill_normal": (I, [I, P, Z, F, F, U, P]),
    "cake_embed": (I, [I, P, P, I, I, P, P]),
    "cake_rmsnorm_set_reg": (None, [I]),
    "cake_rmsnorm": (I, [I, P, P, F, I, I, P, P]),
    "cake_rope_kv": (I, [I, P, P, P, I, I, I, I, I, I, P, I, I, P, P, P]),
    "cake_rope_kv_kvf": (I, [I, P, P, P, I, I, I, I, I, I, P, I, I, P, P, P, I]),
    "cake_dequant_kv_fp8": (I, [I, P, P, I, I, I, I, P, P, P]),
    "cake_silu_mul": (I, [I, P, P, Z, P, P]),
    "cake_silu_mul_rows": (I, [I, P, Z, I, P, P]),
    "cake_add_resid": (I, [I, P, P, Z, P]),
    "cake_wave_reduce_probe": (I, [P, P, P]),
    "cake_flash_set_impl": (None, [I]),
    "cake_flash_set_nw": (None, [I]),
    "cake_flash_set_pair_min": (None, [L]),
    "cake_flash_set_ksplit": (None, [I]),
    "cake_flash_attn_ws": (I, [I, P, P, P, P, I, I, I, I, I, I, P, F, I, I, P, L, P]),
    "cake_flash_attn": (I, [I, P, P, P, P, I, I, I, I, I, I, P, F, I, I, P]),
    "cake_gemm_tile": (I, [I, P, P]),
    "cake_gemm_ws_floats": (L, [I, I, I, I, I, I]),
    "cake_gemm": (I, [I, I, I, I, P, L, P, L, P, L, P, P, L, P, P, I, I, I, P]),
    "cake_gemm_w8a8_num_cfgs": (I, []),
    "cake_gemm_w8a8_plan": (I, [I, I, I]),
    "cake_gemm_w8a8": (I, [I, I, I, P, L, P, P, L, P, P, L, P, L, I, I, I, P]),
    "cake_gemv_set_tuning": (I, [I, I, I, I]),
    "cake_qkv_rope_kvf": (I, [I, P, P, F, P, P, P, I, I, I, I, P, P, P, P, P, I, P, I]),
    "cake_qkv_rope": (I, [I, P, P, F, P, P, P, I, I, I, I, P, P, P, P, P, I, P]),
    "cake_gemv_norm_f32": (I, [I, P, P, F, P, I, I, P, P]),
    "cake_head_select": (I, [I, P, P, F, P, I, I, P, P, P, I, F, P, P, P, P, I, P, P, P]),
    "cake_swiglu": (I, [I, P, P, F, P, P, I, I, P, P]),
    "cake_gemv_x16": (I, [I, P, P, I, I, P, I, P]),
    "cake_gemv_w4_set_tuning": (I, [I, I, I, I]),
    "cake_gemv_w4_get_tuning": (I, [I, P]),
    "cake_qkv_rope_w4_kvf": (I, [I, P, P, F, P, P, P, P, P, P, I, I, I, I, P, P, P, P, P, I, P,
                                 I]),
    "cake_qkv_rope_w4": (I, [I, P, P, F, P, P, P, P, P, P, I, I, I, I, P, P, P, P, P, I, P]),
    "cake_gemv_norm_f32_w4": (I, [I, P, P, F, P, P, I, I, P, P]),
    "cake_head_select_w4": (I, [I, P, P, F, P, P, I, I, P, P, P, I, F, P, P, P, P, I, P, P, P]),
    "cake_swiglu_w4": (I, [I, P, P, F, P, P, P, P, I, I, P, P]),
    "cake_gemv_x16_w4": (I, [I, P, P, P, I, I, P, I, P]),
    "cake_gemv_w8_set_tuning": (I, [I, I, I, I]),
    "cake_gemv_w8_get_tuning": (I, [I, P]),
    "cake_qkv_rope_w8_kvf": (I, [I, P, P, F, P, P, P, P, P, P, I, I, I, I, P, P, P, P, P, I, P,
                                 I]),
    "cake_qkv_rope_w8": (I, [I, P, P, F, P, P, P, P, P, P, I, I, I, I, P, P, P, P, P, I, P]),
    "cake_gemv_norm_f32_w8": (I, [I, P, P, F, P, P, I, I, P, P]),
    "cake_head_select_w8": (I, [I, P, P, F, P, P, I, I, P, P, P, I, F, P, P, P, P, I, P, P, P]),
    "cake_swiglu_w8": (I, [I, P, P, F, P, P, P, P, I, I, P, P]),
    "cake_gemv_x16_w8": (I, [I, P, P, P, I, I, P, I, P]),
    "cake_hop_alloc": (I, [Z, P]),
    "cake_hop_free": (I, [P]),
    "cake_ipc_handle": (I, [P, P]),
    "cake_ipc_handle_size": (I, []),
    "cake_ipc_open": (I, [P, P]),
    "cake_ipc_close": (I, [P]),
    "cake_hop_words": (I, [I, I, I]),
    "cake_hop_send": (I, [P, I, I, I, P, P, P]),
    "cake_hop_recv": (I, [P, I, I, I, P, P, P, D, P]),
    "cake_bulk_send": (I, [P, P, P, I, P, U, P, P, P]),
    "cake_bulk_recv": (I, [P, U, P, P, P, D, P]),
    "cake_logprob_ws_bytes": (L, [I]),
    "cake_logprob_topk": (I, [P, I, P, P, I, P, I, P, P, I, P]),
    "cake_quant_rows_fp8": (I, [I, P, I, I, P, P, P]),
    "cake_dequant_rows_fp8": (I, [I, P, P, I, I, P, P]),
    "cake_quant_rows_mxfp4": (I, [I, P, I, I, P, P, P]),
    "cake_dequant_rows_mxfp4": (I, [I, P, P, I, I, P, P]),
    "cake_sample_threshold": (I, [P, I, F, I, F, P, P]),
    "cake_select_dev": (I, [P, I, P, P, P, P, P]),
    "cake_gumbel_argmax": (I, [P, I, F, U, P, P, P, P]),
    "cake_repeat_penalty": (I, [P, P, P, I, F, P]),
    "cake_argmax": (I, [P, I, P, P]),
    "cake_select_shard": (I, [P, I, I, P, P, I, F, F, U, P, P]),
    "cake_finalize_token": (I, [P, P, P, P, P, I, P]),
    "cake_push_token": (I, [P, P, P, P, P, I, P]),
    "cake_lse_rows": (I, [P, L, I, I, I, I, P, P, P, P, P, P]),
    "cake_lse_finish": (I, [P, P, P, I, P, P, P, P]),
    "cake_groupnorm": (I, [I, P, P, P, I, I, L, I, F, I, P, P, P]),
    "cake_layernorm": (I, [I, P, P, P, L, I, F, P, P]),
    "cake_geglu": (I, [I, P, L, I, P, P]),
    "cake_groupnorm_nhwc_splits": (I, [I]),
    "cake_groupnorm_nhwc2": (I, [I, P, P, I, P, P, P, I, I, I, I, F, I, P, P, P, P, P]),
    "cake_groupnorm_nhwc": (I, [I, P, P, P, I, I, I, I, F, I, P, P, P, P, P]),
    "cake_timestep_embed": (I, [I, P, P, I, I, I, F, I, P, P]),
    "cake_sched_step": (I, [I, P, P, L, I, F, P, P, P, P, P]),
    "cake_step_advance": (I, [P, P]),
    "cake_scale_copy": (I, [I, P, L, F, I, P, P]),
    "cake_to_rgb8": (I, [I, P, I, I, I, I, P, P]),
    "cake_clip_embed": (I, [I, P, P, P, I, I, I, I, P, P]),
    "cake_widen16": (I, [I, P, L, P, P]),
    "cake_blaslt_gemm": (I, [I, I, P, L, P, L, P, L, I, I, I, P, Z, P]),
    "cake_graph_decode": (I, [P, P]),
    "cake_attn_oproj_supported": (I, [I, I, I, I]),
    "cake_attn_oproj_ws_floats": (L, [I, I]),
    "cake_attn_oproj_ticket_words": (L, [I, I]),
    "cake_attn_oproj": (I, [I, P, P, P, P, I, I, I, I, F, P, I, I, P, I, P, P, P, P]),
    "cake_mk_gstride": (L, [I, I, I, I, I]),
    "cake_mk_grid": (I, []),
    "cake_mk_set_stamps": (I, [P]),
    "cake_mk_set_tuning": (I, [I, I, I, I]),
    "cake_mk_supported": (I, [I, I, I, I, I]),
    "cake_mk_decode": (I, [I, P, I, I, I, I, I, I, I, F, F, P, P, P, P, P, D, P]),
}
_OPTIONAL = {"cake_attn_oproj_supported", "cake_attn_oproj_ws_floats",
             "cake_attn_oproj_ticket_words", "cake_attn_oproj",
             "cake_mk_gstride", "cake_mk_grid", "cake_mk_set_stamps", "cake_mk_set_tuning",
             "cake_mk_supported", "cake_mk_decode"}


class KernelError(RuntimeError):
    pass


def lib_path() -> Path:
    return Path(os.environ.get("CAKE_KERNEL_LIB", _LIB_PATH))


def kernels():
    global _lib
    if _lib is not None:
        return _lib
    with _lock:
        if _lib is None:
            import torch

            path = lib_path()
            if not path.exists():
                raise KernelError(
                    f"{path} not built; run `python -m cake_amd.build` (hipcc gfx950)")
            lib = C.CDLL(str(path), mode=C.RTLD_GLOBAL)
            for name, (restype, argtypes) in _SIGS.items():
                if name in _OPTIONAL and not hasattr(lib, name):
                    continue
                fn = getattr(lib, name)
                fn.argtypes = argtypes
                fn.restype = restype
            _lib = lib
    return _lib


def available() -> bool:
    try:
        kernels()
        return True
    except (KernelError, OSError):
        return False
# ... 6 lines not shown
```

### cake_amd/ops/hip.py

```python
from __future__ import annotations

import ctypes as C

import os
import threading

import torch

from ._lib import check, kernels

_DT = {torch.bfloat16: 0, torch.float16: 1}


def _dt(t: torch.Tensor) -> int:
    try:
        return _DT[t.dtype]
    except KeyError:
        raise TypeError(f"HIP kernels take bf16/f16 weights, got {t.dtype}") from None


def _stream() -> int:
    return torch.cuda.current_stream().cuda_stream


# ... 701 lines not shown
              "qkv_rope_w8_kvf")
        return
    check(kernels().cake_qkv_rope_w8(_dt(norm_w), _p(resid), _p(norm_w), float(eps), _p(wq),
                                     _p(wk), _p(wv), _p(sq), _p(sk), _p(sv), K, nh, nkv, hd,
                                     _p(inv_freq), _p(pos), _p(q_out), _p(kcache), _p(vcache), S,
                                     _stream()), "qkv_rope_w8")


def swiglu_w8(resid, norm_w, eps, wg, wu, sg, su, act):
    K = resid.numel()
    I = wg.shape[0]
    dt = norm_w.dtype
    _req(resid, "resid", dtype=torch.float32)
    _req(norm_w, "norm_w", shape=(K,))
    _req_w8(wg, sg, "wg", (I, K))
    _req_w8(wu, su, "wu", (I, K))
    _req(act, "act", dtype=dt, numel=I)
    check(kernels().cake_swiglu_w8(_dt(norm_w), _p(resid), _p(norm_w), float(eps), _p(wg), _p(wu),
                                   _p(sg), _p(su), K, I, _p(act), _stream()), "swiglu_w8")


def gemv_w8(x, w8, scale, out, accumulate: bool):
    N, K = w8.shape
    _req_w8(w8, scale, "w8", (N, K))
    _req(x, "x", numel=K)
    _req(out, "out", dtype=torch.float32, numel=N)
    check(kernels().cake_gemv_x16_w8(_dt(x), _p(x), _p(w8), _p(scale), K, N, _p(out),
                                     int(accumulate), _stream()), "gemv_x16_w8")


def norm_gemv_f32_w8(resid, norm_w, eps, w8, scale, out):
    N, K = w8.shape
    _req_w8(w8, scale, "w8", (N, K))
    _dt(norm_w)
    _req(resid, "resid", dtype=torch.float32, numel=K)
    _req(norm_w, "norm_w", shape=(K,))
    _req(out, "out", dtype=torch.float32, numel=N)
    check(kernels().cake_gemv_norm_f32_w8(_dt(norm_w), _p(resid), _p(norm_w), float(eps), _p(w8),
                                          _p(scale), K, N, _p(out), _stream()),
          "gemv_norm_f32_w8")


def _head_select_q(entry: str, qa, qb, resid, norm_w, eps, N, K, logits, hist, hist_len, last_n,
                   penalty, slot, ticket, tok, pos, embed) -> None:
    _req(resid, "resid", dtype=torch.float32, numel=K)
    _req(norm_w, "norm_w", shape=(K,))
    _req(logits, "logits", dtype=torch.float32, numel=N)
    _req(slot, "slot", dtype=torch.int64, numel=1)
    _req(ticket, "ticket", dtype=torch.int32, numel=1)
    for t, n in ((tok, "tok"), (hist, "hist"), (hist_len, "hist_len"), (pos, "pos")):
        _req(t, n, dtype=torch.int32)
    if not 0 <= int(last_n) <= HEAD_SELECT_MAX_LAST_N:
        raise ValueError(f"{entry}: last_n {last_n} > {HEAD_SELECT_MAX_LAST_N}")
    if embed is not None:
        _req(embed, "embed", dtype=norm_w.dtype)
        if embed.dim() != 2 or embed.shape[1] != K:
            raise ValueError(f"{entry}: embed {tuple(embed.shape)} does not match H={K}")
    check(getattr(kernels(), "cake_" + entry)(
        _dt(norm_w), _p(resid), _p(norm_w), float(eps), _p(qa), _p(qb), K, N, _p(logits),
        _p(hist), _p(hist_len), int(last_n), float(penalty), _p(slot), _p(ticket), _p(tok),
        _p(pos), hist.numel(), None if embed is None else _p(embed),
        None if embed is None else _p(resid), _stream()), entry)


def head_select_w8(resid, norm_w, eps, w8, scale, logits, hist, hist_len, last_n: int,
                   penalty: float, slot, ticket, tok, pos, embed=None) -> None:
    N, K = w8.shape
    _req_w8(w8, scale, "w8", (N, K))
    _head_select_q("head_select_w8", w8, scale, resid, norm_w, eps, N, K, logits, hist, hist_len,
                   last_n, penalty, slot, ticket, tok, pos, embed)


GEMV_W8_KINDS = {"qkv": 0, "swiglu": 1, "x16": 2, "head": 3}


def set_gemv_w8_tuning(kind: str, U: int = 4, prefetch: int = 4, max_blocks: int = 1024) -> None:
    check(kernels().cake_gemv_w8_set_tuning(GEMV_W8_KINDS[kind], int(U), int(prefetch),
                                            int(max_blocks)), "gemv_w8_set_tuning")


def get_gemv_w8_tuning(kind: str) -> tuple[int, int, int]:
    out = (C.c_int * 3)()
    check(kernels().cake_gemv_w8_get_tuning(GEMV_W8_KINDS[kind], out), "gemv_w8_get_tuning")
    return int(out[0]), int(out[1]), int(out[2])



def _req_w4(w4, e8, name: str, shape) -> None:
    N, K = shape
    _req(w4, name, dtype=torch.uint8, shape=(N, K // 2))
    _req(e8, name + " scales", dtype=torch.uint8, shape=(N, K // 32))


def quant_rows_mxfp4(w16, w4, e8):
    N, K = w16.shape
    _dt(w16)
    _req(w16, "w16")
    _req_w4(w4, e8, "w4", (N, K))
    check(kernels().cake_quant_rows_mxfp4(_dt(w16), _p(w16), N, K, _p(w4), _p(e8), _stream()),
          "quant_rows_mxfp4")


def dequant_rows_mxfp4(w4, e8, out16):
    N, K = out16.shape
    _req_w4(w4, e8, "w4", (N, K))
    _req(out16, "out16", shape=(N, K))
    check(kernels().cake_dequant_rows_mxfp4(_dt(out16), _p(w4), _p(e8), N, K, _p(out16),
                                            _stream()), "dequant_rows_mxfp4")


def qkv_rope_w4(resid, norm_w, eps, wq, wk, wv, eq, ek, ev, inv_freq, pos, q_out, kcache, vcache,
                kv_fmt=0):
    K = resid.numel()
    nkv, S, hd = kcache.shape
    nh = wq.shape[0] // hd
    dt = norm_w.dtype
    _req(resid, "resid", dtype=torch.float32)
    _req(norm_w, "norm_w", shape=(K,))
    _req_w4(wq, eq, "wq", (nh * hd, K))
    _req_w4(wk, ek, "wk", (nkv * hd, K))
    _req_w4(wv, ev, "wv", (nkv * hd, K))
    _req(inv_freq, "inv_freq", dtype=torch.float32, shape=(hd // 2,))
    _req(pos, "pos", dtype=torch.int32, numel=1)
    _req(q_out, "q_out", dtype=torch.float32, numel=nh * hd)
    _req(kcache, "kcache", dtype=_kv_cache_dtype(kv_fmt, dt))
    _req(vcache, "vcache", dtype=kcache.dtype, shape=kcache.shape)
    if kv_fmt != 0:
        check(kernels().cake_qkv_rope_w4_kvf(_dt(norm_w), _p(resid), _p(norm_w), float(eps),
                                             _p(wq), _p(wk), _p(wv), _p(eq), _p(ek), _p(ev), K,
                                             nh, nkv, hd, _p(inv_freq), _p(pos), _p(q_out),
                                             _p(kcache), _p(vcache), S, _stream(), int(kv_fmt)),
              "qkv_rope_w4_kvf")
        return
    check(kernels().cake_qkv_rope_w4(_dt(norm_w), _p(resid), _p(norm_w), float(eps), _p(wq),
                                     _p(wk), _p(wv), _p(eq), _p(ek), _p(ev), K, nh, nkv, hd,
                                     _p(inv_freq), _p(pos), _p(q_out), _p(kcache), _p(vcache), S,
                                     _stream()), "qkv_rope_w4")


def swiglu_w4(resid, norm_w, eps, wg, wu, eg, eu, act):
    K = resid.numel()
    I = wg.shape[0]
    dt = norm_w.dtype
    _req(resid, "resid", dtype=torch.float32)
    _req(norm_w, "norm_w", shape=(K,))
    _req_w4(wg, eg, "wg", (I, K))
    _req_w4(wu, eu, "wu", (I, K))
    _req(act, "act", dtype=dt, numel=I)
    check(kernels().cake_swiglu_w4(_dt(norm_w), _p(resid), _p(norm_w), float(eps), _p(wg), _p(wu),
                                   _p(eg), _p(eu), K, I, _p(act), _stream()), "swiglu_w4")


def gemv_w4(x, w4, e8, out, accumulate: bool):
    N = w4.shape[0]
    K = x.numel()
    _req_w4(w4, e8, "w4", (N, K))
    _req(x, "x", numel=K)
    _req(out, "out", dtype=torch.float32, numel=N)
    check(kernels().cake_gemv_x16_w4(_dt(x), _p(x), _p(w4), _p(e8), K, N, _p(out),
                                     int(accumulate), _stream()), "gemv_x16_w4")


def norm_gemv_f32_w4(resid, norm_w, eps, w4, e8, out):
    N, K = w4.shape[0], w4.shape[1] * 2
    _req_w4(w4, e8, "w4", (N, K))
    _dt(norm_w)
# ... 425 lines not shown
```

Measured before the change: 360.1 tokens/s.

## Stream decode GEMV weights from a lossless 13-bit packed copy of bf16

```diff
diff --git a/cake_amd/csrc/engine/llama_engine.cpp b/cake_amd/csrc/engine/llama_engine.cpp
--- a/cake_amd/csrc/engine/llama_engine.cpp
+++ b/cake_amd/csrc/engine/llama_engine.cpp
@@ -187,6 +187,8 @@
   j.set("cmd", Json::string(cmd));
   return j;
 }
+
+static const char* const kPack13Kinds = "gu,down,head";
 
 class Llama {
  public:
@@ -344,6 +346,7 @@
                  (long long)weight_bytes_, rank(), (int)owned_.size());
     alloc_state();
     warm_library();
+    pack13_all();
     {
       size_t fr = 0, tot = 0;
       (void)hipMemGetInfo(&fr, &tot);
@@ -401,6 +404,7 @@
   const Cfg& cfg() const { return cfg_; }
   int max_seq() const { return S_; }
   int64_t weight_bytes() const { return weight_bytes_; }
+  int64_t packed_bytes() const { return packed_bytes_; }
   int64_t kv_bytes() const { return 2 * (int64_t)kv_elems() * kv_esize(); }
 
   void prefill_logits(const int32_t* prompt, int T, float* host_logits) {
@@ -769,11 +773,23 @@
   }
 
  private:
+  struct P13Mat {
+    uint8_t* planes = nullptr;
+    int* hdr = nullptr;
+    uint16_t* raw = nullptr;
+    const uint8_t* p(size_t r0, size_t K) const { return planes + r0 * (K / 8 * 13); }
+    const int* h(size_t r0) const { return hdr + r0; }
+  };
   struct LayerW {
     void *ln1, *wqkv, *wo, *ln2, *wgu, *wd;
     float *sqkv = nullptr, *so = nullptr, *sgu = nullptr, *sd = nullptr;
     uint8_t *eqkv = nullptr, *eo = nullptr, *egu = nullptr, *ed = nullptr;
+    P13Mat pqkv, po, pgu, pd;
   };
+  P13Mat phead_;
+  int64_t packed_bytes_ = 0;
+  int packed_mats_ = 0, packed_raw_rows_ = 0;
+  bool pack_full_ = false;
   struct Mode {
     bool fused = true;
     bool greedy = true;
@@ -1214,6 +1230,73 @@
     hip_check(hipDeviceSynchronize(), "sync");
   }
 
+  void pack13_one(int kind, const void* rows16, size_t N, size_t K, int hd, bool required,
+                  P13Mat& out) {
+    constexpr size_t kReserve = (size_t)4 << 30;
+    if (pack_full_ || K % 2048 != 0) return;
+    const int nraw = cake_pack13_rows(kind, rows16, (int)N, (int)K, hd, nullptr, nullptr, nullptr,
+                                      0, st_);
+    k_check(nraw < 0 ? -nraw : 0, "pack13_rows (count)");
+    const size_t planes = N * (K / 8 * 13), hdrs = (N * 4 + 15) / 16 * 16;
+    const size_t bytes = (size_t)cake_pack13_bytes((int)N, (int)K, nraw);
+    size_t fr = 0, tot = 0;
+    hip_check(hipMemGetInfo(&fr, &tot), "hipMemGetInfo");
+    if (fr < bytes + kReserve) {
+      if (required)
+        throw Error("CAKE_PACK16=1: the packed copy of a [" + std::to_string(N) + ", " +
+                    std::to_string(K) + "] matrix (" + std::to_string(bytes >> 20) +
+                    " MiB) does not fit above the 4 GiB reserve (" + std::to_string(fr >> 20) +
+                    " MiB free)");
+      pack_full_ = true;
+      return;
+    }
+    uint8_t* blk = dalloc<uint8_t>(bytes);
+    P13Mat m;
+    m.planes = blk;
+    m.hdr = reinterpret_cast<int*>(blk + planes);
+    m.raw = nraw ? reinterpret_cast<uint16_t*>(blk + planes + hdrs) : nullptr;
+    const int got = cake_pack13_rows(kind, rows16, (int)N, (int)K, hd, m.planes, m.hdr, m.raw,
+                                     nraw, st_);
+    k_check(got < 0 ? -got : (got == nraw ? 0 : (int)hipErrorUnknown), "pack13_rows");
+    out = m;
+    packed_bytes_ += (int64_t)bytes;
+    packed_raw_rows_ += nraw;
+    ++packed_mats_;
+  }
+
+  void pack13_all() {
+    const char* e = std::getenv("CAKE_PACK16");
+    const std::string mode = e ? e : "";
+    if (mode == "0") return;
+    const bool required = mode == "1";
+    if (!mode.empty() && !required) throw Error("CAKE_PACK16 must be 0, 1 or unset, not " + mode);
+    if (dt_ != 0 || tp_ > 1) {
+      if (required)
+        throw Error("CAKE_PACK16=1: the 13-bit packing is of bf16 weights without tensor "
+                    "parallelism; unset it (or 0) for f16 and tensor-parallel engines");
+      return;
+    }
+    const char* ke = std::getenv("CAKE_PACK16_KINDS");
+    const std::string kinds = "," + std::string(ke && *ke ? ke : kPack13Kinds) + ",";
+    auto on = [&](const char* k) { return kinds.find("," + std::string(k) + ",") != std::string::npos; };
+    const Cfg& c = lc_;
+    const size_t H = c.H, nq = (size_t)c.nh * c.hd, nk = (size_t)c.nkv * c.hd, I = c.I;
+    if (wfmt_ == 0)
+      for (LayerW& w : layers_) {
+        if (on("qkv")) pack13_one(1, w.wqkv, nq + 2 * nk, H, c.hd, required, w.pqkv);
+        if (on("o")) pack13_one(0, w.wo, H, nq, 0, required, w.po);
+        if (on("gu")) pack13_one(2, w.wgu, 2 * I, H, 0, required, w.pgu);
+        if (on("down")) pack13_one(0, w.wd, H, I, 0, required, w.pd);
+      }
+    if (head_ && hfmt_ == 0 && lm_head_ && on("head"))
+      pack13_one(0, lm_head_, (size_t)c.V, H, 0, required, phead_);
+    std::fprintf(stderr,
+                 "cake engine: decode streams %d matrices packed to 13 bits (%d raw rows), "
+                 "%.2f GiB beside the 16-bit weights%s (rank %d)\n",
+                 packed_mats_, packed_raw_rows_, (double)packed_bytes_ / (double)(1 << 30),
+                 pack_full_ ? "; the rest stay 16-bit: HBM reserve reached" : "", rank());
+  }
+
   size_t kv_esize() const { return kvfmt_ == kKvFp8 ? 1 : 2; }
   size_t kv_elems() const { return owned_.size() * (size_t)lc_.nkv * S_ * lc_.hd; }
   void* kc(int l) const { return cur_.k + (size_t)l * lc_.nkv * S_ * lc_.hd * kv_esize(); }
@@ -1702,9 +1785,15 @@
         continue;
       }
       const uint16_t* wqkv = reinterpret_cast<const uint16_t*>(w.wqkv);
-      k_check(cake_qkv_rope_kvf(dt_, resid_, w.ln1, (float)c.eps, wqkv, wqkv + (size_t)nq * c.H,
-                                wqkv + (size_t)(nq + nk) * c.H, c.H, c.nh, c.nkv, c.hd, inv_freq_,
-                                pos_, q_, kc(l), vc(l), S_, st_, kvfmt_), "qkv_rope");
+      if (const P13Mat& m = w.pqkv; m.planes)
+        k_check(cake_qkv_rope_p13_kvf(dt_, resid_, w.ln1, (float)c.eps, m.p(0, c.H), m.p(nq, c.H),
+                                      m.p(nq + nk, c.H), m.h(0), m.h(nq), m.h(nq + nk), m.raw,
+                                      m.raw, m.raw, c.H, c.nh, c.nkv, c.hd, inv_freq_, pos_, q_,
+                                      kc(l), vc(l), S_, st_, kvfmt_), "qkv_rope_p13");
+      else
+        k_check(cake_qkv_rope_kvf(dt_, resid_, w.ln1, (float)c.eps, wqkv, wqkv + (size_t)nq * c.H,
+                                  wqkv + (size_t)(nq + nk) * c.H, c.H, c.nh, c.nkv, c.hd, inv_freq_,
+                                  pos_, q_, kc(l), vc(l), S_, st_, kvfmt_), "qkv_rope");
       if (kvfmt_ != kKvFp8 && short_step_ && ao_ok_) {
         k_check(ao_.run(dt_, q_, kc(l), vc(l), pos_, S_, c.nh, c.nkv, c.hd, scale(), w.wo,
                                 nq, c.H, tp_ > 1 ? partial_ : resid_, tp_ > 1 ? 0 : 1, ao_ws_,
@@ -1715,16 +1804,27 @@
         if (tp_ > 1) {
           k_check(cake_gemv_x16(dt_, attn_out_, w.wo, nq, c.H, partial_, 0, st_), "o_proj");
           ar_sum();
+        } else if (w.po.planes) {
+          k_check(cake_gemv_x16_p13(dt_, attn_out_, w.po.planes, w.po.hdr, w.po.raw, nq, c.H,
+                                    resid_, 1, st_), "o_proj_p13");
         } else {
           k_check(cake_gemv_x16(dt_, attn_out_, w.wo, nq, c.H, resid_, 1, st_), "o_proj");
         }
       }
       const uint16_t* wgu = reinterpret_cast<const uint16_t*>(w.wgu);
-      k_check(cake_swiglu(dt_, resid_, w.ln2, (float)c.eps, wgu, wgu + (size_t)c.I * c.H, c.H,
-                          c.I, act_, st_), "swiglu");
+      if (const P13Mat& m = w.pgu; m.planes)
+        k_check(cake_swiglu_p13(dt_, resid_, w.ln2, (float)c.eps, m.p(0, c.H), m.p(c.I, c.H),
+                                m.h(0), m.h(c.I), m.raw, m.raw, c.H, c.I, act_, st_),
+                "swiglu_p13");
+      else
+        k_check(cake_swiglu(dt_, resid_, w.ln2, (float)c.eps, wgu, wgu + (size_t)c.I * c.H, c.H,
+                            c.I, act_, st_), "swiglu");
       if (tp_ > 1) {
         k_check(cake_gemv_x16(dt_, act_, w.wd, c.I, c.H, partial_, 0, st_), "down_proj");
         ar_sum();
+      } else if (w.pd.planes) {
+        k_check(cake_gemv_x16_p13(dt_, act_, w.pd.planes, w.pd.hdr, w.pd.raw, c.I, c.H, resid_, 1,
+                                  st_), "down_proj_p13");
       } else {
         k_check(cake_gemv_x16(dt_, act_, w.wd, c.I, c.H, resid_, 1, st_), "down_proj");
       }
@@ -1753,6 +1853,12 @@
                                     logits_, hist_, hist_len_, last_n, m.penalty, slot_,
                                     sel_ticket_, tok_, pos_, S_, embed_, resid_, st_),
                 "head_select_w4");
+      else if (phead_.planes)
+        k_check(cake_head_select_p13(dt_, resid_, norm_, (float)c.eps, phead_.planes, phead_.hdr,
+                                     phead_.raw, c.H, c.V, logits_, hist_, hist_len_, last_n,
+                                     m.penalty, slot_, sel_ticket_, tok_, pos_, S_, embed_, resid_,
+                                     st_),
+                "head_select_p13");
       else
         k_check(cake_head_select(dt_, resid_, norm_, (float)c.eps, lm_head_, c.H, c.V, logits_,
                                  hist_, hist_len_, last_n, m.penalty, slot_, sel_ticket_, tok_,
@@ -1774,6 +1880,9 @@
     else if (hfmt_ == 2)
       k_check(cake_gemv_norm_f32_w4(dt_, row, norm_, (float)c.eps, head_q_, head_e_, c.H, c.V,
                                     logits_, st_), "lm_head_w4");
+    else if (phead_.planes)
+      k_check(cake_gemv_norm_f32_p13(dt_, row, norm_, (float)c.eps, phead_.planes, phead_.hdr,
+                                     phead_.raw, c.H, c.V, logits_, st_), "lm_head_p13");
     else
       k_check(cake_gemv_norm_f32(dt_, row, norm_, (float)c.eps, lm_head_, c.H, c.V, logits_, st_),
               "lm_head");
@@ -2875,6 +2984,10 @@
   return h ? static_cast<Llama*>(h)->weight_bytes() : 0;
 }
 
+CAKE_API int64_t cake_engine_packed_bytes(void* h) {
+  return h ? static_cast<Llama*>(h)->packed_bytes() : 0;
+}
+
 CAKE_API int32_t cake_engine_eos(void* h, int32_t* out, int32_t cap) {
   if (!h) return 0;
   const auto& e = static_cast<Llama*>(h)->cfg().eos;
diff --git a/cake_amd/csrc/engine/llama_engine.h b/cake_amd/csrc/engine/llama_engine.h
--- a/cake_amd/csrc/engine/llama_engine.h
+++ b/cake_amd/csrc/engine/llama_engine.h
@@ -87,6 +87,7 @@
 int32_t cake_engine_info(void* engine, int32_t* out8);
 int32_t cake_engine_eos(void* engine, int32_t* out, int32_t cap);
 int64_t cake_engine_weight_bytes(void* engine);
+int64_t cake_engine_packed_bytes(void* engine);
 int64_t cake_engine_kv_bytes(void* engine);
 int32_t cake_engine_generate(void* engine, const int32_t* prompt, int32_t n_prompt,
                              int32_t max_new, const struct CakeEngineSampling* sampling,
diff --git a/cake_amd/csrc/kernels/cake_kernels.h b/cake_amd/csrc/kernels/cake_kernels.h
--- a/cake_amd/csrc/kernels/cake_kernels.h
+++ b/cake_amd/csrc/kernels/cake_kernels.h
@@ -154,6 +154,30 @@
 int cake_gemv_x16(int dt, const void* x, const void* w, int K, int N, float* out, int accumulate,
                   hipStream_t st);
 
+int cake_gemv_p13_set_tuning(int kind, int U, int prefetch, int max_blocks);
+int cake_gemv_p13_get_tuning(int kind, int* out3);
+int cake_qkv_rope_p13_kvf(int dt, const float* resid, const void* norm_w, float eps,
+                          const void* pq, const void* pk, const void* pv, const int* hq,
+                          const int* hk, const int* hv, const void* rq, const void* rk,
+                          const void* rv, int K, int nh, int nkv, int hd, const float* inv_freq,
+                          const int* pos, float* q_out, void* kcache, void* vcache, int S,
+                          hipStream_t st, int kv_fmt);
+
+int cake_gemv_norm_f32_p13(int dt, const float* resid, const void* norm_w, float eps,
+                           const void* planes, const int* hdr, const void* raw, int K, int N,
+                           float* out, hipStream_t st);
+int cake_head_select_p13(int dt, const float* resid, const void* norm_w, float eps,
+                         const void* planes, const int* hdr, const void* raw, int K, int N,
+                         float* out, int* hist, int* hist_len, int last_n, float penalty,
+                         unsigned long long* slot, unsigned int* ticket, int* tok, int* pos,
+                         int max_hist, const void* embed, float* emb_out, hipStream_t st);
+
+int cake_swiglu_p13(int dt, const float* resid, const void* norm_w, float eps, const void* pg,
+                    const void* pu, const int* hg, const int* hu, const void* rg, const void* ru,
+                    int K, int I, void* act, hipStream_t st);
+int cake_gemv_x16_p13(int dt, const void* x, const void* planes, const int* hdr, const void* raw,
+                      int K, int N, float* out, int accumulate, hipStream_t st);
+
 int cake_gemv_w4_set_tuning(int kind, int U, int prefetch, int max_blocks);
 int cake_gemv_w4_get_tuning(int kind, int* out3);
 int cake_qkv_rope_w4_kvf(int dt, const float* resid, const void* norm_w, float eps, const void* wq,
@@ -235,6 +259,12 @@
                       int K, void* rec, int max_rec, void* ws, unsigned int* ticket,
                       int max_blocks, hipStream_t st);
 
+long long cake_pack13_bytes(int N, int K, int nraw);
+int cake_pack13_rows(int kind, const void* rows16, int N, int K, int hd, void* planes, int* hdr,
+                     void* raw, int raw_cap, hipStream_t st);
+int cake_unpack13_rows(const void* planes, const int* hdr, const void* raw, int N, int K,
+                       void* out16, hipStream_t st);
+
 int cake_quant_rows_fp8(int dt, const void* w16, int N, int K, void* w8, float* scale,
                         hipStream_t st);
 int cake_dequant_rows_fp8(int dt, const void* w8, const float* scale, int N, int K, void* out16,
diff --git a/cake_amd/csrc/kernels/gemv.hip b/cake_amd/csrc/kernels/gemv.hip
--- a/cake_amd/csrc/kernels/gemv.hip
+++ b/cake_amd/csrc/kernels/gemv.hip
@@ -1,10 +1,11 @@
 #include "gemv_kernel.h"
 
 namespace cake {
-GemvTune g_tune[3][kNumKinds] = {
+GemvTune g_tune[4][kNumKinds] = {
     {{2, 4, 1024}, {2, 4, 512}, {4, 4, 1024}, {4, 4, 256}, {4, 4, 1024}},
     {{2, 4, 1024}, {2, 4, 1024}, {4, 4, 1024}, {2, 4, 1024}},
-    {{2, 4, 1024}, {2, 4, 1024}, {2, 4, 1024}, {2, 4, 1024}}};
+    {{2, 4, 1024}, {2, 4, 1024}, {2, 4, 1024}, {2, 4, 1024}},
+    {{1, 1, 1024}, {1, 1, 512}, {1, 1, 1024}, {1, 1, 512}, {1, 1, 1024}}};
 }
 
 CAKE_API int cake_gemv_set_tuning(int kind, int U, int prefetch, int max_blocks) {
diff --git a/cake_amd/csrc/kernels/gemv_kernel.h b/cake_amd/csrc/kernels/gemv_kernel.h
--- a/cake_amd/csrc/kernels/gemv_kernel.h
+++ b/cake_amd/csrc/kernels/gemv_kernel.h
@@ -1,4 +1,6 @@
 #pragma once
+#include <type_traits>
+
 #include "common.h"
 
 namespace cake {
@@ -11,7 +13,7 @@
 
 struct GemvTune { int U, PF, MB; };
 enum GemvKind { kQkv = 0, kSwiglu = 1, kX16 = 2, kNormF32 = 3, kX16S = 4, kNumKinds = 5 };
-extern GemvTune g_tune[3][kNumKinds];
+extern GemvTune g_tune[4][kNumKinds];
 
 
 template <class T>
@@ -78,6 +80,19 @@
   }
 };
 
+template <class F, class = void> struct HasRawRows : std::false_type {};
+template <class F>
+struct HasRawRows<F, std::void_t<decltype(F::kRawRows)>> : std::bool_constant<F::kRawRows> {};
+
+template <class F, class = void> struct Bf16Only : std::false_type {};
+template <class F>
+struct Bf16Only<F, std::void_t<decltype(F::kBf16Only)>> : std::bool_constant<F::kBf16Only> {};
+
+template <class F, int U, class = void> struct X16Waves : std::integral_constant<int, 1> {};
+template <class F, int U>
+struct X16Waves<F, U, std::void_t<decltype(F::x16_waves(U))>>
+    : std::integral_constant<int, F::x16_waves(U)> {};
+
 template <class F>
 __device__ __forceinline__ float row_scale(const typename F::Mat& m, size_t row) {
   if constexpr (F::kRowScale) return m.scale[row];
@@ -194,7 +209,13 @@
     F::template fma<DT, XF32>(xs, c, F::template load<false>(r, c), acc_a, acc_b);
 }
 
-template <class F, int PFC> struct Regs { typename F::Chunk c[PFC > 0 ? PFC : 1]; };
+template <class F, int PFC, bool RAW = HasRawRows<F>::value> struct Regs {
+  typename F::Chunk c[PFC > 0 ? PFC : 1];
+};
+template <class F, int PFC> struct Regs<F, PFC, true> {
+  typename F::Chunk c[PFC > 0 ? PFC : 1];
+  typename F::Rows r;
+};
 
 template <class F, int PFC>
 __device__ __forceinline__ void prefetch_rows(const typename F::Rows& r, Regs<F, PFC>& g) {
@@ -205,10 +226,66 @@
   }
 }
 
+template <class F, int PFC>
+__device__ __forceinline__ void keep_rows(const typename F::Rows& r, Regs<F, PFC>& g) {
+  if constexpr (HasRawRows<F>::value) g.r = r;
+}
+
+template <class F, int DT, bool XF32, int U, int PFC, class Map, class Epi>
+__device__ __forceinline__ void run_pairs_raw(const Map& map, const Epi& epi, const void* xs, int K,
+                                              int npairs, int p0, int stride,
+                                              const Regs<F, PFC>& pre) {
+  const int nch = K >> F::kLog2;
+  auto raw_dots = [&](const typename F::Rows& r, float& aa, float& ab) {
+    dot_range<W16, DT, XF32, 4>(F::raw_rows(r, K), xs, K >> W16::kLog2, 0, aa, ab);
+  };
+  auto clamped = [&](int q) { return map(q < npairs ? q : npairs - 1); };
+  int p = p0;
+  typename F::Rows rn;
+  if constexpr (PFC > 0) {
+    const typename F::Rows r = pre.r;
+    rn = clamped(p + stride);
+    const int lane = threadIdx.x & 63;
+    if (F::is_raw(r)) {
+      float aa = 0.f, ab = 0.f;
+      raw_dots(r, aa, ab);
+      const float sa = wave_sum(aa), sb = wave_sum(ab);
+      if (p < npairs) epi(p, sa, sb);
+    } else {
+      typename F::Acc aa = F::zero(), ab = F::zero();
+#pragma unroll
+      for (int c = 0; c < PFC; ++c) F::template fma<DT, XF32>(xs, c * 64 + lane, pre.c[c], aa, ab);
+      dot_range<F, DT, XF32, U>(r, xs, nch, PFC * 64, aa, ab);
+      const float sa = wave_sum(F::total(aa)), sb = wave_sum(F::total(ab));
+      if (p < npairs) epi(p, sa, sb);
+    }
+    p += stride;
+  } else {
+    rn = clamped(p);
+  }
+  for (; p < npairs; p += stride) {
+    const typename F::Rows r = rn;
+    rn = clamped(p + stride);
+    if (F::is_raw(r)) {
+      float aa = 0.f, ab = 0.f;
+      raw_dots(r, aa, ab);
+      epi(p, wave_sum(aa), wave_sum(ab));
+      continue;
+    }
+    typename F::Acc aa = F::zero(), ab = F::zero();
+    dot_range<F, DT, XF32, U>(r, xs, nch, 0, aa, ab);
+    epi(p, wave_sum(F::total(aa)), wave_sum(F::total(ab)));
+  }
+}
+
 template <class F, int DT, bool XF32, int U, int PFC, class Map, class Epi>
 __device__ __forceinline__ void run_pairs(const Map& map, const Epi& epi, const void* xs, int K,
                                           int npairs, int p0, int stride,
                                           const Regs<F, PFC>& pre) {
+  if constexpr (HasRawRows<F>::value) {
+    run_pairs_raw<F, DT, XF32, U, PFC>(map, epi, xs, K, npairs, p0, stride, pre);
+    return;
+  }
   const int nch = K >> F::kLog2;
   int p = p0;
   if constexpr (PFC > 0) {
@@ -278,6 +355,7 @@
   NormPre<F, DT, NX> xp;
   const int pc = p0 < npairs ? p0 : npairs - 1;
   const typename F::Rows r0 = map(pc);
+  keep_rows<F, PFC>(r0, pre);
   if constexpr (NX > 0) xp.load(a.resid, a.norm_w, a.K);
   __builtin_amdgcn_sched_barrier(0);
   if (NX > 0 || (PFC > 0 && p0 < npairs)) prefetch_rows<F, PFC>(r0, pre);
@@ -331,6 +409,7 @@
   NormPre<F, DT, NX> xp;
   const int jp = j0 < I ? j0 : I - 1;
   const typename F::Rows r0 = map(jp);
+  keep_rows<F, PFC>(r0, pre);
   if constexpr (NX > 0) xp.load(resid, norm_w, K);
   __builtin_amdgcn_sched_barrier(0);
   if (NX > 0 || (PFC > 0 && j0 < I)) prefetch_rows<F, PFC>(r0, pre);
@@ -348,7 +427,8 @@
 }
 
 template <class F, int DT, int U, int PFC, int NX, bool ACCUM>
-__global__ __launch_bounds__(kGemvThreads) void gemv_x16_kernel(
+__global__ __launch_bounds__(kGemvThreads) __attribute__((amdgpu_waves_per_eu(X16Waves<F, U>::value)))
+void gemv_x16_kernel(
     const uint16_t* __restrict__ x, const typename F::Mat w, int K, int N,
     float* __restrict__ out) {
   extern __shared__ float smem[];
@@ -361,6 +441,7 @@
   Plain16Pre<F, NX> xp;
   const int pc = p0 < npairs ? p0 : npairs - 1;
   const typename F::Rows r0 = map(pc);
+  keep_rows<F, PFC>(r0, pre);
   if constexpr (NX > 0) xp.load(x, K);
   __builtin_amdgcn_sched_barrier(0);
   if (NX > 0 || (PFC > 0 && p0 < npairs)) prefetch_rows<F, PFC>(r0, pre);
@@ -496,6 +577,7 @@
   NormPre<F, DT, NX> xp;
   const int pc = p0 < npairs ? p0 : npairs - 1;
   const typename F::Rows r0 = map(pc);
+  keep_rows<F, PFC>(r0, pre);
   if constexpr (NX > 0) xp.load(resid, norm_w, K);
   __builtin_amdgcn_sched_barrier(0);
   if (NX > 0 || (PFC > 0 && p0 < npairs)) prefetch_rows<F, PFC>(r0, pre);
@@ -534,6 +616,13 @@
     if ((dt) == kBF16) { constexpr int DT = kBF16; __VA_ARGS__; } \
     else if ((dt) == kF16) { constexpr int DT = kF16; __VA_ARGS__; } \
     else return (int)hipErrorInvalidValue;         \
+  } while (0)
+#define DISPATCH_DT_F(F, dt, ...)                  \
+  do {                                             \
+    if constexpr (Bf16Only<F>::value) {            \
+      if ((dt) == kBF16) { constexpr int DT = kBF16; __VA_ARGS__; } \
+      else return (int)hipErrorInvalidValue;       \
+    } else DISPATCH_DT(dt, __VA_ARGS__);           \
   } while (0)
 
 #define CAKE_TUNE_U(F, PFCV, ...)                                                              \
@@ -596,7 +685,7 @@
   const int K = a.K, npairs = (a.nh + 2 * a.nkv) * (a.hd / 2);
   const size_t lds = x32_lds_bytes<F>(K);
   const GemvTune t = g_tune[F::kFmt][kQkv];
-  DISPATCH_DT(dt, DISPATCH_TUNE(F, t, K, CAKE_NX_NORM(K, hipLaunchKernelGGL((qkv_rope_kernel<F, DT, U, PF, NX>),
+  DISPATCH_DT_F(F, dt, DISPATCH_TUNE(F, t, K, CAKE_NX_NORM(K, hipLaunchKernelGGL((qkv_rope_kernel<F, DT, U, PF, NX>),
                                                          dim3(grid_for(npairs, t.MB)),
                                                          dim3(kGemvThreads), lds, st, a))));
   return (int)hipGetLastError();
@@ -610,7 +699,7 @@
   const size_t lds = x32_lds_bytes<F>(K);
   const GemvTune t = g_tune[F::kFmt][kSwiglu];
   const int mb = t.MB > (I + 27) / 28 ? t.MB : (I + 27) / 28;
-  DISPATCH_DT(dt, DISPATCH_TUNE(F, t, K, CAKE_NX_NORM(K, hipLaunchKernelGGL((swiglu_kernel<F, DT, U, PF, NX>),
+  DISPATCH_DT_F(F, dt, DISPATCH_TUNE(F, t, K, CAKE_NX_NORM(K, hipLaunchKernelGGL((swiglu_kernel<F, DT, U, PF, NX>),
                                                          dim3(grid_for(I, mb)), dim3(kGemvThreads),
                                                          lds, st, resid, (const uint16_t*)norm_w, eps,
                                                          wg, wu, K, I, (uint16_t*)act))));
@@ -625,11 +714,11 @@
   const GemvTune t = g_tune[F::kFmt][F::kKinds > kX16S && K <= 8192 ? kX16S : kX16];
   const int g = grid_for((N + 1) / 2, t.MB);
   if (accumulate) {
-    DISPATCH_DT(dt, DISPATCH_TUNE(F, t, K, CAKE_NX_X16(K, hipLaunchKernelGGL((gemv_x16_kernel<F, DT, U, PF, NX, true>),
+    DISPATCH_DT_F(F, dt, DISPATCH_TUNE(F, t, K, CAKE_NX_X16(K, hipLaunchKernelGGL((gemv_x16_kernel<F, DT, U, PF, NX, true>),
                                                           dim3(g), dim3(kGemvThreads), lds, st,
                                                           (const uint16_t*)x, w, K, N, out))));
   } else {
-    DISPATCH_DT(dt, DISPATCH_TUNE(F, t, K, CAKE_NX_X16(K, hipLaunchKernelGGL((gemv_x16_kernel<F, DT, U, PF, NX, false>),
+    DISPATCH_DT_F(F, dt, DISPATCH_TUNE(F, t, K, CAKE_NX_X16(K, hipLaunchKernelGGL((gemv_x16_kernel<F, DT, U, PF, NX, false>),
                                                           dim3(g), dim3(kGemvThreads), lds, st,
                                                           (const uint16_t*)x, w, K, N, out))));
   }
@@ -643,7 +732,7 @@
   if (bad_shape<F>(K, N)) return (int)hipErrorInvalidValue;
   const size_t lds = SEL && x32_lds_bytes<F>(K) < 64 ? 64 : x32_lds_bytes<F>(K);
   const GemvTune t = g_tune[F::kFmt][kNormF32];
-  DISPATCH_DT(dt, DISPATCH_TUNE(F, t, K, CAKE_NX_NORM(K, hipLaunchKernelGGL((gemv_norm_f32_kernel<F, DT, U, PF, NX, SEL>),
+  DISPATCH_DT_F(F, dt, DISPATCH_TUNE(F, t, K, CAKE_NX_NORM(K, hipLaunchKernelGGL((gemv_norm_f32_kernel<F, DT, U, PF, NX, SEL>),
                                                          dim3(grid_for((N + 1) / 2, t.MB)),
                                                          dim3(kGemvThreads), lds, st, resid,
                                                          (const uint16_t*)norm_w, eps, w, K, N,
diff --git a/cake_amd/csrc/kernels/gemv_p13.hip b/cake_amd/csrc/kernels/gemv_p13.hip
--- /dev/null
+++ b/cake_amd/csrc/kernels/gemv_p13.hip
@@ -0,0 +1,23 @@
+#include "gemv_p13_kernel.h"
+
+CAKE_API int cake_gemv_p13_set_tuning(int kind, int U, int prefetch, int max_blocks) {
+  return gemv_set_tuning<P13>(kind, U, prefetch, max_blocks);
+}
+
+CAKE_API int cake_gemv_p13_get_tuning(int kind, int* out3) { return gemv_get_tuning<P13>(kind, out3); }
+
+CAKE_API int cake_qkv_rope_p13_kvf(int dt, const float* resid, const void* norm_w, float eps,
+                                   const void* pq, const void* pk, const void* pv, const int* hq,
+                                   const int* hk, const int* hv, const void* rq, const void* rk,
+                                   const void* rv, int K, int nh, int nkv, int hd,
+                                   const float* inv_freq, const int* pos, float* q_out,
+                                   void* kcache, void* vcache, int S, hipStream_t st, int kv_fmt) {
+  if (p13_bad(dt, K, pq, hq) || p13_bad(dt, K, pk, hk) || p13_bad(dt, K, pv, hv))
+    return (int)hipErrorInvalidValue;
+  return launch_qkv<P13>(dt, {resid, (const uint16_t*)norm_w, eps,
+                              {(const uint8_t*)pq, hq, (const uint16_t*)rq},
+                              {(const uint8_t*)pk, hk, (const uint16_t*)rk},
+                              {(const uint8_t*)pv, hv, (const uint16_t*)rv}, K, nh, nkv, hd,
+                              inv_freq, pos, q_out, (uint16_t*)kcache, (uint16_t*)vcache, S,
+                              kv_fmt}, st);
+}
diff --git a/cake_amd/csrc/kernels/gemv_p13_head.hip b/cake_amd/csrc/kernels/gemv_p13_head.hip
--- /dev/null
+++ b/cake_amd/csrc/kernels/gemv_p13_head.hip
@@ -0,0 +1,23 @@
+#include "gemv_p13_kernel.h"
+
+CAKE_API int cake_gemv_norm_f32_p13(int dt, const float* resid, const void* norm_w, float eps,
+                                    const void* planes, const int* hdr, const void* raw, int K,
+                                    int N, float* out, hipStream_t st) {
+  if (p13_bad(dt, K, planes, hdr)) return (int)hipErrorInvalidValue;
+  return launch_norm_f32<P13, false>(dt, resid, norm_w, eps,
+                                     {(const uint8_t*)planes, hdr, (const uint16_t*)raw}, K, N,
+                                     out, HeadSel{}, st);
+}
+
+CAKE_API int cake_head_select_p13(int dt, const float* resid, const void* norm_w, float eps,
+                                  const void* planes, const int* hdr, const void* raw, int K,
+                                  int N, float* out, int* hist, int* hist_len, int last_n,
+                                  float penalty, unsigned long long* slot, unsigned int* ticket,
+                                  int* tok, int* pos, int max_hist, const void* embed,
+                                  float* emb_out, hipStream_t st) {
+  if (p13_bad(dt, K, planes, hdr)) return (int)hipErrorInvalidValue;
+  return launch_head_select<P13>(dt, resid, norm_w, eps,
+                                 {(const uint8_t*)planes, hdr, (const uint16_t*)raw}, K, N, out,
+                                 hist, hist_len, last_n, penalty, slot, ticket, tok, pos,
+                                 max_hist, embed, emb_out, st);
+}
diff --git a/cake_amd/csrc/kernels/gemv_p13_kernel.h b/cake_amd/csrc/kernels/gemv_p13_kernel.h
--- /dev/null
+++ b/cake_amd/csrc/kernels/gemv_p13_kernel.h
@@ -0,0 +1,151 @@
+#pragma once
+#include "gemv_kernel.h"
+
+namespace cake {
+
+constexpr int kP13Tile = 2048;
+constexpr int kP13TileBytes = 3328;
+enum PackKind { kPackAdjacent = 0, kPackHeadHalves = 1, kPackGateUp = 2 };
+
+__host__ __device__ inline int p13_partner(int kind, int r, int N, int hd) {
+  if (kind == kPackHeadHalves) return r % hd < hd / 2 ? r + hd / 2 : r - hd / 2;
+  if (kind == kPackGateUp) return r < N / 2 ? r + N / 2 : r - N / 2;
+  return (r ^ 1) < N ? (r ^ 1) : r;
+}
+
+__device__ __forceinline__ uint32_t p13_base4(int hdr) {
+  return (uint32_t)(hdr & 0x7f) * 0x01010101u;
+}
+
+__device__ __forceinline__ void p13_high(uint32_t code, uint32_t sgn, int j, uint32_t base4,
+                                         uint32_t& hia, uint32_t& hib) {
+  const uint32_t ca = code & 0x0f0f0f0fu, cb = (code >> 4) & 0x0f0f0f0fu;
+  const uint32_t ta = (ca + 0x7f7f7f7fu) & 0x80808080u, tb = (cb + 0x7f7f7f7fu) & 0x80808080u;
+  const uint32_t ha = ca + ((ta - (ta >> 7)) & base4), hb = cb + ((tb - (tb >> 7)) & base4);
+  const uint32_t sa = sgn << (7 - 2 * j), sb = sgn << (6 - 2 * j);
+  hia = (ha & 0x7f7f7f7fu) | (sa & 0x80808080u);
+  hib = (hb & 0x7f7f7f7fu) | (sb & 0x80808080u);
+}
+
+__device__ __forceinline__ uint4 p13_decode8(uint32_t lo0, uint32_t lo1, uint32_t code,
+                                             uint32_t sgn, int j, uint32_t base4) {
+  uint32_t hia, hib;
+  p13_high(code, sgn, j, base4, hia, hib);
+  uint4 o;
+  o.x = __builtin_amdgcn_perm(hia, lo0, 0x05010400u);
+  o.y = __builtin_amdgcn_perm(hia, lo0, 0x07030602u);
+  o.z = __builtin_amdgcn_perm(hib, lo1, 0x05010400u);
+  o.w = __builtin_amdgcn_perm(hib, lo1, 0x07030602u);
+  return o;
+}
+
+__device__ __forceinline__ void p13_decode8f(uint32_t lo0, uint32_t lo1, uint32_t code,
+                                             uint32_t sgn, int j, uint32_t base4, float* o) {
+  uint32_t hia, hib;
+  p13_high(code, sgn, j, base4, hia, hib);
+  o[0] = __uint_as_float(__builtin_amdgcn_perm(hia, lo0, 0x04000c0cu));
+  o[1] = __uint_as_float(__builtin_amdgcn_perm(hia, lo0, 0x05010c0cu));
+  o[2] = __uint_as_float(__builtin_amdgcn_perm(hia, lo0, 0x06020c0cu));
+  o[3] = __uint_as_float(__builtin_amdgcn_perm(hia, lo0, 0x07030c0cu));
+  o[4] = __uint_as_float(__builtin_amdgcn_perm(hib, lo1, 0x04000c0cu));
+  o[5] = __uint_as_float(__builtin_amdgcn_perm(hib, lo1, 0x05010c0cu));
+  o[6] = __uint_as_float(__builtin_amdgcn_perm(hib, lo1, 0x06020c0cu));
+  o[7] = __uint_as_float(__builtin_amdgcn_perm(hib, lo1, 0x07030c0cu));
+}
+
+__device__ __forceinline__ uint32_t ld_nt4(const uint32_t* p) { return __builtin_nontemporal_load(p); }
+
+struct P13 {
+  static constexpr int kFmt = 3, kKinds = kNumKinds, kLog2 = 5, kPad32 = 1, kPad16 = 1;
+  static constexpr int kU[3] = {1, 2, 3}, kPF[2] = {2, 1};
+  static constexpr bool kStrict = true, kRowScale = false, kRawRows = true, kBf16Only = true;
+  static constexpr int x16_waves(int U) { return U == 1 ? 3 : 1; }
+  static __device__ __forceinline__ int perm32(int i) { return i; }
+  static __device__ __forceinline__ int perm16(int i) { return i; }
+  static int prefetch(int pf, int K) { return PlainRows::prefetch_if_filled<kLog2>(pf, K); }
+  using Acc = float;
+  static __device__ __forceinline__ Acc zero() { return 0.f; }
+  static __device__ __forceinline__ float total(Acc a) { return a; }
+  struct Mat {
+    const uint8_t* planes;
+    const int* hdr;
+    const uint16_t* raw;
+  };
+  static __device__ __forceinline__ Mat pick(const Mat& q, const Mat& k, const Mat& v, int kind) {
+    return {pick3(q.planes, k.planes, v.planes, kind), pick3(q.hdr, k.hdr, v.hdr, kind),
+            pick3(q.raw, k.raw, v.raw, kind)};
+  }
+  struct Rows {
+    const uint8_t *a, *b;
+    int ha, hb;
+    const uint16_t *rawa, *rawb;
+  };
+  static __device__ __forceinline__ Rows rows(const Mat& ma, size_t ra, const Mat& mb, size_t rb,
+                                              int K) {
+    const size_t rowb = (size_t)(K / kP13Tile) * kP13TileBytes;
+    return {ma.planes + ra * rowb, mb.planes + rb * rowb, ma.hdr[ra], mb.hdr[rb], ma.raw, mb.raw};
+  }
+  static __device__ __forceinline__ bool is_raw(const Rows& r) {
+    return (__builtin_amdgcn_readfirstlane(r.ha | r.hb) >> 8) != 0;
+  }
+  static __device__ __forceinline__ PlainRows::Rows raw_rows(const Rows& r, int K) {
+    const int sa = __builtin_amdgcn_readfirstlane(r.ha) >> 8;
+    const int sb = __builtin_amdgcn_readfirstlane(r.hb) >> 8;
+    return {reinterpret_cast<const uint4*>(r.rawa + (size_t)(sa - 1) * K),
+            reinterpret_cast<const uint4*>(r.rawb + (size_t)(sb - 1) * K)};
+  }
+  struct Chunk {
+    uint4 la0, la1, ca, lb0, lb1, cb;
+    uint32_t sa, sb;
+    int ha, hb;
+  };
+  template <bool NT> static __device__ __forceinline__ Chunk load(const Rows& r, int c) {
+    const size_t t = (size_t)(c >> 6) * kP13TileBytes;
+    const int l = c & 63;
+    const uint4* pa = reinterpret_cast<const uint4*>(r.a + t) + l;
+    const uint4* pb = reinterpret_cast<const uint4*>(r.b + t) + l;
+    const uint32_t* qa = reinterpret_cast<const uint32_t*>(r.a + t + 3072) + l;
+    const uint32_t* qb = reinterpret_cast<const uint32_t*>(r.b + t + 3072) + l;
+    Chunk v;
+    if constexpr (NT) {
+      v.la0 = ld_nt16(pa); v.la1 = ld_nt16(pa + 64); v.ca = ld_nt16(pa + 128); v.sa = ld_nt4(qa);
+      v.lb0 = ld_nt16(pb); v.lb1 = ld_nt16(pb + 64); v.cb = ld_nt16(pb + 128); v.sb = ld_nt4(qb);
+    } else {
+      v.la0 = pa[0]; v.la1 = pa[64]; v.ca = pa[128]; v.sa = *qa;
+      v.lb0 = pb[0]; v.lb1 = pb[64]; v.cb = pb[128]; v.sb = *qb;
+    }
+    v.ha = r.ha;
+    v.hb = r.hb;
+    return v;
+  }
+  template <int DT, bool XF32>
+  static __device__ __forceinline__ void fma(const void* xs, int chunk, const Chunk& v, Acc& acc_a,
+                                             Acc& acc_b) {
+    if constexpr (DT == kBF16) {
+      const int c16 = ((chunk >> 6) << 8) + (chunk & 63);
+      const uint32_t la[8] = {v.la0.x, v.la0.y, v.la0.z, v.la0.w, v.la1.x, v.la1.y, v.la1.z, v.la1.w};
+      const uint32_t lb[8] = {v.lb0.x, v.lb0.y, v.lb0.z, v.lb0.w, v.lb1.x, v.lb1.y, v.lb1.z, v.lb1.w};
+      const uint32_t ca[4] = {v.ca.x, v.ca.y, v.ca.z, v.ca.w};
+      const uint32_t cb[4] = {v.cb.x, v.cb.y, v.cb.z, v.cb.w};
+      const uint32_t base_a = p13_base4(v.ha), base_b = p13_base4(v.hb);
+#pragma unroll
+      for (int j = 0; j < 4; ++j) {
+        float xv[8], fa[8], fb[8];
+        load_x8<DT, XF32>(xs, c16 + j * 64, xv);
+        p13_decode8f(la[2 * j], la[2 * j + 1], ca[j], v.sa, j, base_a, fa);
+        p13_decode8f(lb[2 * j], lb[2 * j + 1], cb[j], v.sb, j, base_b, fb);
+#pragma unroll
+        for (int e = 0; e < 8; ++e) {
+          acc_a = fmaf(fa[e], xv[e], acc_a);
+          acc_b = fmaf(fb[e], xv[e], acc_b);
+        }
+      }
+    }
+  }
+};
+
+static inline bool p13_bad(int dt, int K, const void* planes, const void* hdr) {
+  return dt != kBF16 || K < kP13Tile || K % kP13Tile != 0 || planes == nullptr || hdr == nullptr;
+}
+
+}
diff --git a/cake_amd/csrc/kernels/gemv_p13_mlp.hip b/cake_amd/csrc/kernels/gemv_p13_mlp.hip
--- /dev/null
+++ b/cake_amd/csrc/kernels/gemv_p13_mlp.hip
@@ -0,0 +1,18 @@
+#include "gemv_p13_kernel.h"
+
+CAKE_API int cake_swiglu_p13(int dt, const float* resid, const void* norm_w, float eps,
+                             const void* pg, const void* pu, const int* hg, const int* hu,
+                             const void* rg, const void* ru, int K, int I, void* act,
+                             hipStream_t st) {
+  if (p13_bad(dt, K, pg, hg) || p13_bad(dt, K, pu, hu)) return (int)hipErrorInvalidValue;
+  return launch_swiglu<P13>(dt, resid, norm_w, eps, {(const uint8_t*)pg, hg, (const uint16_t*)rg},
+                            {(const uint8_t*)pu, hu, (const uint16_t*)ru}, K, I, act, st);
+}
+
+CAKE_API int cake_gemv_x16_p13(int dt, const void* x, const void* planes, const int* hdr,
+                               const void* raw, int K, int N, float* out, int accumulate,
+                               hipStream_t st) {
+  if (p13_bad(dt, K, planes, hdr)) return (int)hipErrorInvalidValue;
+  return launch_x16<P13>(dt, x, {(const uint8_t*)planes, hdr, (const uint16_t*)raw}, K, N, out,
+                         accumulate, st);
+}
diff --git a/cake_amd/csrc/kernels/pack13.hip b/cake_amd/csrc/kernels/pack13.hip
--- /dev/null
+++ b/cake_amd/csrc/kernels/pack13.hip
@@ -0,0 +1,205 @@
+#include "gemv_p13_kernel.h"
+
+namespace cake {
+
+constexpr int kPackThreads = 256;
+
+__global__ __launch_bounds__(kPackThreads) void p13_scan_kernel(const uint16_t* __restrict__ w,
+                                                                int K, int* __restrict__ tmp) {
+  __shared__ int smax[kPackThreads / 64], smin[kPackThreads / 64];
+  const uint4* p = reinterpret_cast<const uint4*>(w + (size_t)blockIdx.x * K);
+  int hmax = 0, hmin = 128;
+  for (int c = threadIdx.x; c < K / 8; c += kPackThreads) {
+    const uint4 v = p[c];
+    const uint32_t d[4] = {v.x, v.y, v.z, v.w};
+#pragma unroll
+    for (int e = 0; e < 8; ++e) {
+      const int h = (int)((d[e >> 1] >> (16 * (e & 1) + 8)) & 0x7f);
+      hmax = max(hmax, h);
+      hmin = h ? min(hmin, h) : hmin;
+    }
+  }
+#pragma unroll
+  for (int o = 32; o > 0; o >>= 1) {
+    hmax = max(hmax, __shfl_xor(hmax, o));
+    hmin = min(hmin, __shfl_xor(hmin, o));
+  }
+  if ((threadIdx.x & 63) == 0) {
+    smax[threadIdx.x >> 6] = hmax;
+    smin[threadIdx.x >> 6] = hmin;
+  }
+  __syncthreads();
+  if (threadIdx.x == 0) {
+    for (int i = 1; i < kPackThreads / 64; ++i) {
+      hmax = max(hmax, smax[i]);
+      hmin = min(hmin, smin[i]);
+    }
+    const int unrep = hmin != 128 && hmin <= hmax - 15;
+    tmp[blockIdx.x] = hmax | (unrep << 8);
+  }
+}
+
+__global__ __launch_bounds__(1024) void p13_assign_kernel(const int* __restrict__ tmp, int kind,
+                                                          int N, int hd, int* __restrict__ hdr,
+                                                          int* __restrict__ count) {
+  __shared__ int scan[1024];
+  int running = 0;
+  for (int r0 = 0; r0 < N; r0 += 1024) {
+    const int r = r0 + (int)threadIdx.x;
+    int f = 0, top = 0;
+    if (r < N) {
+      const int t = tmp[r];
+      top = t & 0xff;
+      f = ((t | tmp[p13_partner(kind, r, N, hd)]) >> 8) & 1;
+    }
+    scan[threadIdx.x] = f;
+    __syncthreads();
+    for (int o = 1; o < 1024; o <<= 1) {
+      const int add = (int)threadIdx.x >= o ? scan[threadIdx.x - o] : 0;
+      __syncthreads();
+      scan[threadIdx.x] += add;
+      __syncthreads();
+    }
+    if (r < N && hdr != nullptr) {
+      const int slot = f ? running + scan[threadIdx.x] - 1 : -1;
+      hdr[r] = ((slot + 1) << 8) | ((top - 15) & 0xff);
+    }
+    running += scan[1023];
+    __syncthreads();
+  }
+  if (threadIdx.x == 0) *count = running;
+}
+
+__global__ __launch_bounds__(kPackThreads) void p13_write_kernel(
+    const uint16_t* __restrict__ w, size_t nlanes, int tiles, int K, const int* __restrict__ hdr,
+    uint8_t* __restrict__ planes, uint16_t* __restrict__ raw) {
+  for (size_t idx = (size_t)blockIdx.x * kPackThreads + threadIdx.x; idx < nlanes;
+       idx += (size_t)gridDim.x * kPackThreads) {
+    const int l = (int)(idx & 63);
+    const size_t rt = idx >> 6, row = rt / tiles, t = rt % tiles;
+    const int h = hdr[row], slot = (h >> 8) - 1, base = (int)(int8_t)(h & 0xff);
+    const uint4* src = reinterpret_cast<const uint4*>(w + row * K + t * kP13Tile);
+    uint32_t lo[8] = {0, 0, 0, 0, 0, 0, 0, 0}, code[4] = {0, 0, 0, 0}, sgn = 0;
+    if (slot >= 0) {
+      uint4* dst = reinterpret_cast<uint4*>(raw + (size_t)slot * K + t * kP13Tile);
+#pragma unroll
+      for (int j = 0; j < 4; ++j) dst[j * 64 + l] = src[j * 64 + l];
+    } else {
+#pragma unroll
+      for (int j = 0; j < 4; ++j) {
+        const uint4 v = src[j * 64 + l];
+        const uint32_t d[4] = {v.x, v.y, v.z, v.w};
+#pragma unroll
+        for (int e = 0; e < 8; ++e) {
+          const uint32_t x = (d[e >> 1] >> (16 * (e & 1))) & 0xffffu;
+          const int h7 = (int)((x >> 8) & 0x7f);
+          const uint32_t cd = h7 ? (uint32_t)(h7 - base) : 0u;
+          lo[2 * j + (e >> 2)] |= (x & 0xffu) << (8 * (e & 3));
+          code[j] |= cd << (4 * (e < 4 ? 2 * e : 2 * (e - 4) + 1));
+          sgn |= (x >> 15) << (8 * (e & 3) + 2 * j + (e >> 2));
+        }
+      }
+    }
+    uint8_t* tp = planes + rt * kP13TileBytes;
+    reinterpret_cast<uint4*>(tp)[l] = make_uint4(lo[0], lo[1], lo[2], lo[3]);
+    reinterpret_cast<uint4*>(tp + 1024)[l] = make_uint4(lo[4], lo[5], lo[6], lo[7]);
+    reinterpret_cast<uint4*>(tp + 2048)[l] = make_uint4(code[0], code[1], code[2], code[3]);
+    reinterpret_cast<uint32_t*>(tp + 3072)[l] = sgn;
+  }
+}
+
+__global__ __launch_bounds__(kPackThreads) void p13_unpack_kernel(
+    const uint8_t* __restrict__ planes, const int* __restrict__ hdr,
+    const uint16_t* __restrict__ raw, size_t nlanes, int tiles, int K, uint16_t* __restrict__ out) {
+  for (size_t idx = (size_t)blockIdx.x * kPackThreads + threadIdx.x; idx < nlanes;
+       idx += (size_t)gridDim.x * kPackThreads) {
+    const int l = (int)(idx & 63);
+    const size_t rt = idx >> 6, row = rt / tiles, t = rt % tiles;
+    const int h = hdr[row], slot = (h >> 8) - 1;
+    uint4* dst = reinterpret_cast<uint4*>(out + row * K + t * kP13Tile);
+    if (slot >= 0) {
+      const uint4* src = reinterpret_cast<const uint4*>(raw + (size_t)slot * K + t * kP13Tile);
+#pragma unroll
+      for (int j = 0; j < 4; ++j) dst[j * 64 + l] = src[j * 64 + l];
+      continue;
+    }
+    const uint8_t* tp = planes + rt * kP13TileBytes;
+    const uint4 l0 = reinterpret_cast<const uint4*>(tp)[l];
+    const uint4 l1 = reinterpret_cast<const uint4*>(tp + 1024)[l];
+    const uint4 cv = reinterpret_cast<const uint4*>(tp + 2048)[l];
+    const uint32_t sgn = reinterpret_cast<const uint32_t*>(tp + 3072)[l];
+    const uint32_t lo[8] = {l0.x, l0.y, l0.z, l0.w, l1.x, l1.y, l1.z, l1.w};
+    const uint32_t code[4] = {cv.x, cv.y, cv.z, cv.w};
+    const uint32_t base4 = p13_base4(h);
+#pragma unroll
+    for (int j = 0; j < 4; ++j)
+      dst[j * 64 + l] = p13_decode8(lo[2 * j], lo[2 * j + 1], code[j], sgn, j, base4);
+  }
+}
+
+static inline int pack_grid(size_t nlanes) {
+  const size_t want = (nlanes + kPackThreads - 1) / kPackThreads;
+  return (int)(want < 16384 ? want : 16384);
+}
+
+static inline bool pack_bad_shape(int kind, int N, int K, int hd) {
+  if (N < 1 || K < kP13Tile || K % kP13Tile) return true;
+  if (kind == kPackHeadHalves) return hd < 2 || hd % 2 || N % hd;
+  if (kind == kPackGateUp) return N % 2 != 0;
+  return kind != kPackAdjacent;
+}
+
+}
+
+using namespace cake;
+
+CAKE_API long long cake_pack13_bytes(int N, int K, int nraw) {
+  if (N < 1 || K < kP13Tile || K % kP13Tile || nraw < 0) return -1;
+  return (long long)N * (K / kP13Tile) * kP13TileBytes + ((long long)N * 4 + 15) / 16 * 16 +
+         (long long)nraw * K * 2;
+}
+
+CAKE_API int cake_pack13_rows(int kind, const void* rows16, int N, int K, int hd, void* planes,
+                              int* hdr, void* raw, int raw_cap, hipStream_t st) {
+  const bool count_only = planes == nullptr && hdr == nullptr && raw == nullptr;
+  if (rows16 == nullptr || pack_bad_shape(kind, N, K, hd) || raw_cap < 0 ||
+      (!count_only && (planes == nullptr || hdr == nullptr)))
+    return -(int)hipErrorInvalidValue;
+  int* tmp = nullptr;
+  hipError_t e = hipMalloc(&tmp, sizeof(int) * ((size_t)N + 1));
+  if (e != hipSuccess) return -(int)e;
+  const uint16_t* w = (const uint16_t*)rows16;
+  int count = 0;
+  hipLaunchKernelGGL(p13_scan_kernel, dim3(N), dim3(kPackThreads), 0, st, w, K, tmp);
+  hipLaunchKernelGGL(p13_assign_kernel, dim3(1), dim3(1024), 0, st, tmp, kind, N, hd, hdr, tmp + N);
+  e = hipGetLastError();
+  if (e == hipSuccess) e = hipMemcpyAsync(&count, tmp + N, sizeof(int), hipMemcpyDeviceToHost, st);
+  if (e == hipSuccess) e = hipStreamSynchronize(st);
+  if (e == hipSuccess && !count_only) {
+    if (count > raw_cap || (count > 0 && raw == nullptr)) {
+      e = hipErrorInvalidValue;
+    } else {
+      const int tiles = K / kP13Tile;
+      const size_t nlanes = (size_t)N * tiles * 64;
+      hipLaunchKernelGGL(p13_write_kernel, dim3(pack_grid(nlanes)), dim3(kPackThreads), 0, st, w,
+                         nlanes, tiles, K, hdr, (uint8_t*)planes, (uint16_t*)raw);
+      e = hipGetLastError();
+      if (e == hipSuccess) e = hipStreamSynchronize(st);
+    }
+  }
+  (void)hipFree(tmp);
+  return e == hipSuccess ? count : -(int)e;
+}
+
+CAKE_API int cake_unpack13_rows(const void* planes, const int* hdr, const void* raw, int N, int K,
+                                void* out16, hipStream_t st) {
+  if (N < 1 || K < kP13Tile || K % kP13Tile || planes == nullptr || hdr == nullptr ||
+      out16 == nullptr)
+    return (int)hipErrorInvalidValue;
+  const int tiles = K / kP13Tile;
+  const size_t nlanes = (size_t)N * tiles * 64;
+  hipLaunchKernelGGL(p13_unpack_kernel, dim3(pack_grid(nlanes)), dim3(kPackThreads), 0, st,
+                     (const uint8_t*)planes, hdr, (const uint16_t*)raw, nlanes, tiles, K,
+                     (uint16_t*)out16);
+  return (int)hipGetLastError();
+}
diff --git a/cake_amd/engine.py b/cake_amd/engine.py
--- a/cake_amd/engine.py
+++ b/cake_amd/engine.py
@@ -78,6 +78,8 @@
     L.cake_engine_eos.restype = I
     L.cake_engine_weight_bytes.argtypes = [P]
     L.cake_engine_weight_bytes.restype = C.c_int64
+    L.cake_engine_packed_bytes.argtypes = [P]
+    L.cake_engine_packed_bytes.restype = C.c_int64
     L.cake_engine_kv_bytes.argtypes = [P]
     L.cake_engine_kv_bytes.restype = C.c_int64
     L.cake_engine_open_layers.argtypes = [C.c_char_p, C.POINTER(EngineOpts),
@@ -275,6 +277,9 @@
     def weight_bytes(self) -> int:
         return int(lib().cake_engine_weight_bytes(self._h))
 
+    def packed_bytes(self) -> int:
+        return int(lib().cake_engine_packed_bytes(self._h))
+
     def kv_bytes(self) -> int:
         return int(lib().cake_engine_kv_bytes(self._h))
 
diff --git a/cake_amd/ops/_lib.py b/cake_amd/ops/_lib.py
--- a/cake_amd/ops/_lib.py
+++ b/cake_amd/ops/_lib.py
@@ -78,6 +78,15 @@
     "cake_head_select": (I, [I, P, P, F, P, I, I, P, P, P, I, F, P, P, P, P, I, P, P, P]),
     "cake_swiglu": (I, [I, P, P, F, P, P, I, I, P, P]),
     "cake_gemv_x16": (I, [I, P, P, I, I, P, I, P]),
+    "cake_gemv_p13_set_tuning": (I, [I, I, I, I]),
+    "cake_gemv_p13_get_tuning": (I, [I, P]),
+    "cake_qkv_rope_p13_kvf": (I, [I, P, P, F, P, P, P, P, P, P, P, P, P, I, I, I, I, P, P, P, P,
+                                  P, I, P, I]),
+    "cake_gemv_norm_f32_p13": (I, [I, P, P, F, P, P, P, I, I, P, P]),
+    "cake_head_select_p13": (I, [I, P, P, F, P, P, P, I, I, P, P, P, I, F, P, P, P, P, I, P, P,
+                                 P]),
+    "cake_swiglu_p13": (I, [I, P, P, F, P, P, P, P, P, P, I, I, P, P]),
+    "cake_gemv_x16_p13": (I, [I, P, P, P, P, I, I, P, I, P]),
     "cake_gemv_w4_set_tuning": (I, [I, I, I, I]),
     "cake_gemv_w4_get_tuning": (I, [I, P]),
     "cake_qkv_rope_w4_kvf": (I, [I, P, P, F, P, P, P, P, P, P, I, I, I, I, P, P, P, P, P, I, P,
@@ -109,6 +118,9 @@
     "cake_bulk_recv": (I, [P, U, P, P, P, D, P]),
     "cake_logprob_ws_bytes": (L, [I]),
     "cake_logprob_topk": (I, [P, I, P, P, I, P, I, P, P, I, P]),
+    "cake_pack13_bytes": (L, [I, I, I]),
+    "cake_pack13_rows": (I, [I, P, I, I, I, P, P, P, I, P]),
+    "cake_unpack13_rows": (I, [P, P, P, I, I, P, P]),
     "cake_quant_rows_fp8": (I, [I, P, I, I, P, P, P]),
     "cake_dequant_rows_fp8": (I, [I, P, P, I, I, P, P]),
     "cake_quant_rows_mxfp4": (I, [I, P, I, I, P, P, P]),
diff --git a/cake_amd/ops/hip.py b/cake_amd/ops/hip.py
--- a/cake_amd/ops/hip.py
+++ b/cake_amd/ops/hip.py
@@ -807,6 +807,163 @@
 def get_gemv_w8_tuning(kind: str) -> tuple[int, int, int]:
     out = (C.c_int * 3)()
     check(kernels().cake_gemv_w8_get_tuning(GEMV_W8_KINDS[kind], out), "gemv_w8_get_tuning")
+    return int(out[0]), int(out[1]), int(out[2])
+
+
+
+PACK13_TILE, PACK13_TILE_BYTES = 2048, 3328
+PACK13_KINDS = {"adjacent": 0, "head_halves": 1, "gate_up": 2}
+
+
+def pack13_bytes(N: int, K: int, nraw: int) -> int:
+    return int(kernels().cake_pack13_bytes(int(N), int(K), int(nraw)))
+
+
+class Packed13:
+
+    def __init__(self, planes, hdr, raw, K: int):
+        self.planes, self.hdr, self.raw, self.K = planes, hdr, raw, int(K)
+
+    @property
+    def N(self) -> int:
+        return self.hdr.numel()
+
+    @property
+    def nraw(self) -> int:
+        return 0 if self.raw is None else self.raw.shape[0]
+
+    def rows(self, lo: int, hi: int) -> "Packed13":
+        return Packed13(self.planes[lo:hi], self.hdr[lo:hi], self.raw, self.K)
+
+    def args(self):
+        return _p(self.planes), _p(self.hdr), _p(self.raw)
+
+
+def _req_p13(m: Packed13, name: str, N: int, K: int) -> None:
+    _req(m.planes, name + " planes", dtype=torch.uint8, numel=N * (K // 8) * 13)
+    _req(m.hdr, name + " hdr", dtype=torch.int32, shape=(N,))
+    if m.raw is not None:
+        _req(m.raw, name + " raw", dtype=torch.bfloat16)
+    if m.K != K:
+        raise ValueError(f"{name}: packed with K = {m.K}, not {K}")
+
+
+def pack13_rows(w16, kind: str = "adjacent", hd: int = 0) -> Packed13:
+    N, K = w16.shape
+    _req(w16, "w16")
+    k, st = PACK13_KINDS[kind], _stream()
+    nraw = kernels().cake_pack13_rows(k, _p(w16), N, K, int(hd), None, None, None, 0, st)
+    check(-nraw if nraw < 0 else 0, "pack13_rows")
+    planes = torch.zeros((N, K // PACK13_TILE * PACK13_TILE_BYTES), dtype=torch.uint8,
+                         device=w16.device)
+    hdr = torch.zeros(N, dtype=torch.int32, device=w16.device)
+    raw = torch.zeros((nraw, K), dtype=w16.dtype, device=w16.device) if nraw else None
+    got = kernels().cake_pack13_rows(k, _p(w16), N, K, int(hd), _p(planes), _p(hdr), _p(raw),
+                                     nraw, st)
+    check(-got if got < 0 else 0, "pack13_rows")
+    assert got == nraw, (got, nraw)
+    return Packed13(planes, hdr, raw, K)
+
+
+def unpack13_rows(m: Packed13, out16) -> None:
+    N, K = out16.shape
+    _req_p13(m, "m", N, K)
+    _req(out16, "out16", dtype=torch.bfloat16)
+    check(kernels().cake_unpack13_rows(*m.args(), N, K, _p(out16), _stream()), "unpack13_rows")
+
+
+def qkv_rope_p13(resid, norm_w, eps, mq: Packed13, mk: Packed13, mv: Packed13, inv_freq, pos,
+                 q_out, kcache, vcache, kv_fmt=0):
+    K = resid.numel()
+    nkv, S, hd = kcache.shape
+    nh = mq.N // hd
+    _req(resid, "resid", dtype=torch.float32)
+    _req(norm_w, "norm_w", shape=(K,))
+    _req_p13(mq, "wq", nh * hd, K)
+    _req_p13(mk, "wk", nkv * hd, K)
+    _req_p13(mv, "wv", nkv * hd, K)
+    _req(inv_freq, "inv_freq", dtype=torch.float32, shape=(hd // 2,))
+    _req(pos, "pos", dtype=torch.int32, numel=1)
+    _req(q_out, "q_out", dtype=torch.float32, numel=nh * hd)
+    _req(kcache, "kcache", dtype=_kv_cache_dtype(kv_fmt, norm_w.dtype))
+    _req(vcache, "vcache", dtype=kcache.dtype, shape=kcache.shape)
+    (pq, hq, rq), (pk, hk, rk), (pv, hv, rv) = mq.args(), mk.args(), mv.args()
+    check(kernels().cake_qkv_rope_p13_kvf(_dt(norm_w), _p(resid), _p(norm_w), float(eps), pq, pk,
+                                          pv, hq, hk, hv, rq, rk, rv, K, nh, nkv, hd,
+                                          _p(inv_freq), _p(pos), _p(q_out), _p(kcache),
+                                          _p(vcache), S, _stream(), int(kv_fmt)),
+          "qkv_rope_p13_kvf")
+
+
+def swiglu_p13(resid, norm_w, eps, mg: Packed13, mu: Packed13, act):
+    K = resid.numel()
+    I = mg.N
+    _req(resid, "resid", dtype=torch.float32)
+    _req(norm_w, "norm_w", shape=(K,))
+    _req_p13(mg, "wg", I, K)
+    _req_p13(mu, "wu", I, K)
+    _req(act, "act", dtype=norm_w.dtype, numel=I)
+    (pg, hg, rg), (pu, hu, ru) = mg.args(), mu.args()
+    check(kernels().cake_swiglu_p13(_dt(norm_w), _p(resid), _p(norm_w), float(eps), pg, pu, hg,
+                                    hu, rg, ru, K, I, _p(act), _stream()), "swiglu_p13")
+
+
+def gemv_p13(x, m: Packed13, out, accumulate: bool):
+    N, K = m.N, x.numel()
+    _req_p13(m, "w", N, K)
+    _req(x, "x", numel=K)
+    _req(out, "out", dtype=torch.float32, numel=N)
+    check(kernels().cake_gemv_x16_p13(_dt(x), _p(x), *m.args(), K, N, _p(out), int(accumulate),
+                                      _stream()), "gemv_x16_p13")
+
+
+def norm_gemv_f32_p13(resid, norm_w, eps, m: Packed13, out):
+    N, K = m.N, resid.numel()
+    _req_p13(m, "w", N, K)
+    _req(resid, "resid", dtype=torch.float32, numel=K)
+    _req(norm_w, "norm_w", shape=(K,))
+    _req(out, "out", dtype=torch.float32, numel=N)
+    check(kernels().cake_gemv_norm_f32_p13(_dt(norm_w), _p(resid), _p(norm_w), float(eps),
+                                           *m.args(), K, N, _p(out), _stream()),
+          "gemv_norm_f32_p13")
+
+
+def head_select_p13(resid, norm_w, eps, m: Packed13, logits, hist, hist_len, last_n: int,
+                    penalty: float, slot, ticket, tok, pos, embed=None) -> None:
+    N, K = m.N, resid.numel()
+    _req_p13(m, "w", N, K)
+    _req(resid, "resid", dtype=torch.float32, numel=K)
+    _req(norm_w, "norm_w", shape=(K,))
+    _req(logits, "logits", dtype=torch.float32, numel=N)
+    _req(slot, "slot", dtype=torch.int64, numel=1)
+    _req(ticket, "ticket", dtype=torch.int32, numel=1)
+    for t, n in ((tok, "tok"), (hist, "hist"), (hist_len, "hist_len"), (pos, "pos")):
+        _req(t, n, dtype=torch.int32)
+    if not 0 <= int(last_n) <= HEAD_SELECT_MAX_LAST_N:
+        raise ValueError(f"head_select_p13: last_n {last_n} > {HEAD_SELECT_MAX_LAST_N}")
+    if embed is not None:
+        _req(embed, "embed", dtype=norm_w.dtype)
+        if embed.dim() != 2 or embed.shape[1] != K:
+            raise ValueError(f"head_select_p13: embed {tuple(embed.shape)} does not match H={K}")
+    check(kernels().cake_head_select_p13(
+        _dt(norm_w), _p(resid), _p(norm_w), float(eps), *m.args(), K, N, _p(logits), _p(hist),
+        _p(hist_len), int(last_n), float(penalty), _p(slot), _p(ticket), _p(tok), _p(pos),
+        hist.numel(), None if embed is None else _p(embed),
+        None if embed is None else _p(resid), _stream()), "head_select_p13")
+
+
+GEMV_P13_KINDS = {"qkv": 0, "swiglu": 1, "x16": 2, "head": 3, "x16s": 4}
+GEMV_P13_U, GEMV_P13_PF = (1, 2, 3), (0, 1, 2)
+
+
+def set_gemv_p13_tuning(kind: str, U: int = 1, prefetch: int = 1, max_blocks: int = 1024) -> None:
+    check(kernels().cake_gemv_p13_set_tuning(GEMV_P13_KINDS[kind], int(U), int(prefetch),
+                                             int(max_blocks)), "gemv_p13_set_tuning")
+
+
+def get_gemv_p13_tuning(kind: str) -> tuple[int, int, int]:
+    out = (C.c_int * 3)()
+    check(kernels().cake_gemv_p13_get_tuning(GEMV_P13_KINDS[kind], out), "gemv_p13_get_tuning")
     return int(out[0]), int(out[1]), int(out[2])
 
 
```

New measurement: 391.7 tokens/s (median of 6 runs). +8.8%, better.
